# vt-asaplab/vPIN

Hardware: AMD Instinct MI355X
Metric: R1CS constraints/sec, whole Spartan SNARK (sat proof + SPARK evaluation proof; vPIN point-mult + point-add instances) (higher is better)
Workload: dtype u256 (integers mod q and mod p = 2^255-19, 32-bit limbs); 1 GPU; vPIN LeNet trace (layers L1..L7): 12 SNARKs per step; inputs=resident in HBM, parallelism=one trace per rank x 1 rank(s), no collective; 4 stream(s) per rank, table_slot_bytes=128

## Files before the change

vpin_amd/csrc/capi.hip:

```cpp
#include <chrono>
#include <csignal>
#include <execinfo.h>
#include <fcntl.h>
#include <unistd.h>
#include <cstdio>
#include <cstdlib>
#include <cstring>
#include <thread>

#include "ctx.h"

namespace vpin {

static thread_local std::string g_last_error;

void set_last_error(const char* what, hipError_t e) {
  g_last_error = std::string(what) + ": " + hipGetErrorString(e);
}

void set_last_error_text(const char* text) { g_last_error = text; }

static hipEvent_t get_event(vpin_ctx* c) {
  if (!c->free_events.empty()) {
    hipEvent_t e = c->free_events.back();
// ... 209 lines not shown
void ctx_leave_alt(vpin_ctx* c) { if (c && c->stream_alt) ctx_switch_stream(c, c->stream_main, c->cus_main, false); }

ProfScope::ProfScope(vpin_ctx* c, int kclass, double bytes, int also, double units) : ctx(c) {
  if (!c->prof) return;
  ProfRec r;
  r.kclass = kclass;
  r.also = also;
  r.units = units;
  r.bytes = bytes;
  r.start = get_event(c);
  r.stop = get_event(c);
  (void)hipEventRecord(r.start, c->stream);
  c->recs.push_back(r);
  rec = (int)c->recs.size() - 1;
}

ProfScope::~ProfScope() {
  if (rec >= 0) (void)hipEventRecord(ctx->recs[rec].stop, ctx->stream);
}

}

using namespace vpin;

extern "C" {

const char* vpin_strerror(int code) {
  switch (code) {
    case VPIN_OK: return "ok";
    case VPIN_EINVAL: return "invalid argument";
    case VPIN_ENODEV: return "no usable HIP device (this library has no CPU fallback)";
    case VPIN_ENOMEM: return "out of memory";
    case VPIN_EHIP: return "HIP runtime error";
    case VPIN_ESHAPE: return "operand shapes do not match";
    case VPIN_EVERIFY: return "proof rejected by the verifier";
    case VPIN_ECOMM: return "a peer rank failed or timed out";
    default: return "unknown error";
  }
}

const char* vpin_last_error(void) { return g_last_error.c_str(); }

int vpin_abi_version(void) { return 11; }

static int ctx_create(int device, int priority, const uint32_t* cu_mask, uint32_t n_words, vpin_ctx** out);

int vpin_ctx_create(int device, vpin_ctx** out) { return ctx_create(device, 0, nullptr, 0, out); }
int vpin_ctx_create_prio(int device, int priority, vpin_ctx** out) { return ctx_create(device, priority, nullptr, 0, out); }
int vpin_ctx_create_cumask(int device, const uint32_t* cu_mask, uint32_t n_words, vpin_ctx** out) {
  if (!cu_mask || n_words == 0) return VPIN_EINVAL;
  return ctx_create(device, 0, cu_mask, n_words, out);
}

static int ctx_create(int device, int priority, const uint32_t* cu_mask, uint32_t n_words, vpin_ctx** out) {
  if (!out) return VPIN_EINVAL;
  setenv("KMP_BLOCKTIME", "0", 0);
  setenv("OMP_WAIT_POLICY", "PASSIVE", 0);
  setenv("KMP_AFFINITY", "disabled", 0);
  *out = nullptr;
  int n = 0;
  if (hipGetDeviceCount(&n) != hipSuccess || n <= 0) return VPIN_ENODEV;
  if (device < 0 || device >= n) return VPIN_EINVAL;
  VPIN_HIP_TRY(hipSetDevice(device));
  vpin_ctx* c = new (std::nothrow) vpin_ctx();
  if (!c) return VPIN_ENOMEM;
  c->device = device;
  hipDeviceProp_t prop;
  if (hipGetDeviceProperties(&prop, device) == hipSuccess) c->num_cus = prop.multiProcessorCount;
  int lo = 0, hi = 0;
  (void)hipDeviceGetStreamPriorityRange(&lo, &hi);
  int prio = priority < 0 ? hi : priority > 0 ? lo : 0;
  hipError_t e;
  if (cu_mask) {
    int enabled = 0;
    for (uint32_t w = 0; w < n_words; w++) {
      uint32_t bits = cu_mask[w];
      if ((w + 1) * 32 > (uint32_t)c->num_cus) bits &= (w * 32 >= (uint32_t)c->num_cus) ? 0u : ((1u << (c->num_cus - w * 32)) - 1u);
      enabled += __builtin_popcount(bits);
    }
    if (enabled == 0) { delete c; return VPIN_EINVAL; }
    e = hipExtStreamCreateWithCUMask(&c->stream, n_words, cu_mask);
    c->num_cus = enabled;
    c->cu_masked = true;
  } else {
    e = hipStreamCreateWithPriority(&c->stream, hipStreamNonBlocking, prio);
  }
  if (e != hipSuccess) { set_last_error("hipStreamCreate", e); delete c; return VPIN_EHIP; }
  c->stream_main = c->stream;
  c->cus_main = c->num_cus;
  c->partials_cap = (size_t)18 * 4096 * 3;
  if (hipMalloc(&c->d_partials, c->partials_cap * sizeof(fq)) != hipSuccess ||
      hipMalloc(&c->d_out, 8 * sizeof(fq)) != hipSuccess ||
      hipHostMalloc(&c->h_out, 8 * sizeof(fq), hipHostMallocDefault) != hipSuccess) {
    vpin_ctx_destroy(c);
    return VPIN_ENOMEM;
  }
  ctx_register(c);
  *out = c;
  return VPIN_OK;
}

void vpin_ctx_destroy(vpin_ctx* c) {
  if (!c) return;
  (void)hipSetDevice(c->device);
  if (c->stream) (void)hipStreamSynchronize(c->stream);
  ctx_leave_alt(c);
  if (c->prover_cache_free) c->prover_cache_free(c);
  if (c->spark_cache_free) c->spark_cache_free(c);
  if (c->verify_cache_free) c->verify_cache_free(c);
  if (c->h_spark) (void)hipHostFree(c->h_spark);
  if (c->d_spark_cnt) (void)hipFree(c->d_spark_cnt);
  if (c->d_add_count) (void)hipFree(c->d_add_count);
  ctx_unregister(c);
  ctx_wait_unpinned(c);
  dev_pool_release(c);
  if (!c->pool_sizes.empty()) {
    fprintf(stderr, "vpin_ctx_destroy: %zu device block(s) still referenced by live handles are released with the context; "
                    "free tables / instances / decommitments before the context\n", c->pool_sizes.size());
    for (auto& kv : c->pool_sizes) (void)hipFree(kv.first);
    c->pool_sizes.clear();
  }
  for (auto& r : c->recs) { (void)hipEventDestroy(r.start); (void)hipEventDestroy(r.stop); }
  for (auto e : c->free_events) (void)hipEventDestroy(e);
  if (c->d_partials) (void)hipFree(c->d_partials);
  if (c->d_out) (void)hipFree(c->d_out);
  if (c->h_out) (void)hipHostFree(c->h_out);
  if (c->h_bullet) (void)hipHostFree(c->h_bullet);
  if (c->stream_alt) { (void)hipStreamSynchronize(c->stream_alt); (void)hipStreamDestroy(c->stream_alt); }
  if (c->stream_switch_ev) (void)hipEventDestroy(c->stream_switch_ev);
  if (c->stream_main) (void)hipStreamDestroy(c->stream_main);
  delete c;
}

void* vpin_ctx_stream(vpin_ctx* c) { return c ? (void*)c->stream : nullptr; }

int vpin_ctx_set_cumask_after_phase1(vpin_ctx* c, const uint32_t* cu_mask, uint32_t n_words) {
  if (!c || c->cu_masked || c->stream != c->stream_main) return VPIN_EINVAL;
  (void)hipSetDevice(c->device);
  if (c->stream_alt) {
    VPIN_HIP_TRY(hipStreamSynchronize(c->stream_alt));
    (void)hipStreamDestroy(c->stream_alt);
    c->stream_alt = nullptr;
    c->cus_alt = 0;
  }
  if (!cu_mask || n_words == 0) return VPIN_OK;
  int enabled = 0;
  for (uint32_t w = 0; w < n_words; w++) {
    uint32_t bits = cu_mask[w];
    if ((w + 1) * 32 > (uint32_t)c->cus_main) bits &= (w * 32 >= (uint32_t)c->cus_main) ? 0u : ((1u << (c->cus_main - w * 32)) - 1u);
    enabled += __builtin_popcount(bits);
  }
  if (enabled == 0) return VPIN_EINVAL;
  if (!c->stream_switch_ev) VPIN_HIP_TRY(hipEventCreateWithFlags(&c->stream_switch_ev, hipEventDisableTiming));
  VPIN_HIP_TRY(hipExtStreamCreateWithCUMask(&c->stream_alt, n_words, cu_mask));
  c->cus_alt = enabled;
  return VPIN_OK;
}

int vpin_ctx_set_progress_flag(vpin_ctx* c, int* flag) {
  if (!c) return VPIN_EINVAL;
  c->progress_flag = flag;
  return VPIN_OK;
}

unsigned long long vpin_ctx_strip_rows_taken(vpin_ctx* c) { return c ? c->strip_rows_taken : 0ull; }
unsigned long long vpin_ctx_row_table_rows(vpin_ctx* c) { return c ? c->row_table_rows : 0ull; }
// ... 329 lines not shown
```

vpin_amd/csrc/ctx.h:

```cpp
#pragma once
#include <hip/hip_runtime.h>

#include <atomic>
#include <chrono>
#include <cstdio>
#include <cstdlib>
#include <map>
#include <mutex>
#include <string>
#include <unordered_map>
#include <vector>

#include "../../include/vpin_hip.h"
#include "fq_dev.h"

namespace vpin {

void set_last_error(const char* what, hipError_t e);

#define VPIN_HIP_TRY(expr)                         \
  do {                                             \
    hipError_t e_ = (expr);                        \
    if (e_ != hipSuccess) {                        \
      ::vpin::set_last_error(#expr, e_);           \
      return VPIN_EHIP;                            \
    }                                              \
  } while (0)

struct ProfRec {
  int kclass;
  double bytes;
  hipEvent_t start, stop;
  int also = -1;
  double units = 0.0;
};

}

struct vpin_ctx;

struct vpin_table {
  vpin::fq* d = nullptr;
  size_t len = 0;
  size_t cap = 0;
  bool owned = true;
  vpin_ctx* owner = nullptr;
};

struct vpin_gens;

struct vpin_ctx {
  int device = 0;
  hipStream_t stream = nullptr;
  int num_cus = 256;
  bool cu_masked = false;
  hipStream_t stream_main = nullptr, stream_alt = nullptr;
  hipEvent_t stream_switch_ev = nullptr;
  int cus_main = 256, cus_alt = 0;
  vpin::fq* d_partials = nullptr;
  size_t partials_cap = 0;
  vpin::fq* d_out = nullptr;
  vpin::fq* h_out = nullptr;
  bool prof = false;
  bool prof_count_adds = false;
  unsigned long long* d_add_count = nullptr;
  std::vector<vpin::ProfRec> recs;
  std::vector<hipEvent_t> free_events;
  vpin_kstat stats[VPIN_K_COUNT] = {};
  std::mutex pool_mu;
  std::atomic<int> pins{0};
  std::map<size_t, std::vector<void*>> pool_free_lists;
  std::unordered_map<void*, size_t> pool_sizes;
  void* prover_cache = nullptr;
  void (*prover_cache_free)(vpin_ctx*) = nullptr;
  void* spark_cache = nullptr;
  void (*spark_cache_free)(vpin_ctx*) = nullptr;
  void* verify_cache = nullptr;
  void (*verify_cache_free)(vpin_ctx*) = nullptr;
  vpin::fq* h_spark = nullptr;
  uint32_t* d_spark_cnt = nullptr;
  uint32_t spark_seq = 0;
  int round_split = 0, round_split_grid = 0, round_split_ncirc = 0;
  int round_group_ndotp = 0;
  uint32_t tail_seq = 0;
  std::atomic<int> tail_rounds{0};
  vpin::fq tail_sums[3 * 18];
  vpin::fq tail_final[6 * 18];
  unsigned long long pip_row_chunks = 0;
  unsigned long long row_table_rows = 0;
  unsigned long long strip_rows_taken = 0;
  unsigned long long rlc_shared_sums = 0;
  size_t rlc_shared_cap = 0;
  bool pool_poison = false;
  uint32_t pool_poison_word = 0;
  unsigned long long pool_poison_blocks = 0, pool_poison_bytes = 0;
  unsigned long long witness_redo_ops = 0;
  bool low_memory = false;
  bool shared_device = false;
  int expected_proofs = 0;
  double gens_scalars_per_proof = 0.0;
  void* h_bullet = nullptr;
  uint32_t bullet_seq = 0;
  std::atomic<vpin_comm*> comm_pub{nullptr};
  vpin_comm* comm = nullptr;
  volatile int* progress_flag = nullptr;
};

namespace vpin {

struct ProfScope {
  vpin_ctx* ctx;
  int rec = -1;
  ProfScope(vpin_ctx* c, int kclass, double bytes, int also = -1, double units = 0.0);
  ~ProfScope();
};

void ctx_enter_alt(vpin_ctx* c);
void ctx_leave_alt(vpin_ctx* c);
struct AltStreamGuard {
  vpin_ctx* c;
  explicit AltStreamGuard(vpin_ctx* ctx) : c(ctx) {}
  ~AltStreamGuard() { ctx_leave_alt(c); }
};

int dev_alloc(vpin_ctx* c, size_t bytes, void** out);
hipError_t driver_malloc(void** p, size_t bytes);
void note_driver_alloc(size_t bytes);
void dev_free(vpin_ctx* c, void* p);
int live_ctx_count();
double host_cpu_quota();
void dev_free_owned(vpin_ctx* owner, vpin_ctx* fallback, void* p);
void dev_pool_release(vpin_ctx* c);
void dev_release_block(vpin_ctx* c, void* p);

struct DevBuf {
  vpin_ctx* c;
  void* p = nullptr;
  explicit DevBuf(vpin_ctx* ctx) : c(ctx) {}
// ... 87 lines not shown
```

vpin_amd/csrc/host/prover_common.h:

```cpp
#pragma once
#include <omp.h>

#include <chrono>
#include <cstdlib>
#include <cstring>
#include <map>
#include <memory>
#include <mutex>
#include <string>
#include <vector>

#include "../ctx.h"
#include "../comm.h"
#include "curve.h"
#include "transcript.h"

extern "C" {
size_t vpin_gens_msm_parts_count(size_t ncols);
int vpin_gens_msm_parts(vpin_ctx* ctx, const vpin_gens* g, const uint8_t* scalars_mont, size_t rows, size_t ncols,
                        uint8_t* parts_xyzt);
int vpin_poly_bound(vpin_ctx* c, const vpin_table* Z, const uint8_t* Lvec, size_t L_size, uint8_t* out_LZ);
int vpin_gens_map_stream(vpin_ctx* ctx, const uint8_t* stream64, size_t nb, uint8_t* out_xyzt);
void vpin_r1cs_dims(const vpin_r1cs_dev* d, size_t* num_cons, size_t* num_vars, size_t* num_inputs);
}

namespace vpin_prover {

#if defined(__clang__)
#pragma clang diagnostic push
#pragma clang diagnostic ignored "-Wunused-function"
#endif


using namespace vpin_host;
using Clock = std::chrono::steady_clock;
static double secs(Clock::time_point a, Clock::time_point b) { return std::chrono::duration<double>(b - a).count(); }

static int host_threads() {
  static const int fixed = [] {
    setenv("KMP_BLOCKTIME", "0", 0);
    setenv("OMP_WAIT_POLICY", "PASSIVE", 0);
    const char* e = getenv("VPIN_HOST_THREADS");
    int want = e ? atoi(e) : 0;
    const int hw = omp_get_num_procs();
    return want > hw ? hw : want;
  }();
  if (fixed >= 1) return fixed;
  const int ctxs = vpin::live_ctx_count();
  int n = (int)(vpin::host_cpu_quota() / (2.0 * (double)(ctxs > 0 ? ctxs : 1)));
  return n < 1 ? 1 : n > 8 ? 8 : n;
}

static size_t log2z(size_t n) { size_t l = 0; while (((size_t)1 << l) < n) l++; return l; }
static const uint8_t* B(const Fq* p) { return reinterpret_cast<const uint8_t*>(p); }
static uint8_t* B(Fq* p) { return reinterpret_cast<uint8_t*>(p); }

struct CG { uint8_t b[32]; };
static CG compress(const Point& p) { CG c; p.compress(c.b); return c; }


struct Mcg {
  int n;
  const FixedBase* G[4];
  const FixedBase* h;
};

inline void derive_gens(std::vector<Point>& g, size_t nb, const char* label, vpin_ctx* dev = nullptr) {
  static std::mutex mu;
  static std::map<std::string, std::shared_ptr<const std::vector<Point>>> cache;
  std::shared_ptr<const std::vector<Point>> have;
  {
    std::lock_guard<std::mutex> lock(mu);
    auto it = cache.find(label);
    if (it != cache.end()) have = it->second;
  }
  if (have && have->size() >= nb) {
    g.assign(have->begin(), have->begin() + (long)nb);
    return;
  }
  uint8_t bc[32];
  Point::basepoint().compress(bc);
  Shake256 sh;
  sh.absorb(reinterpret_cast<const uint8_t*>(label), strlen(label));
  sh.absorb(bc, 32);
  sh.finalize();
  std::vector<uint8_t> stream(64 * nb);
  sh.squeeze(stream.data(), stream.size());
  auto fresh = std::make_shared<std::vector<Point>>(nb);
// ... 310 lines not shown
  };
  size_t n = R;
  static const bool fine = getenv("VPIN_SPARK_TRACE") && atoi(getenv("VPIN_SPARK_TRACE")) >= 3;
  double tb[6] = {0, 0, 0, 0, 0, 0};
  const bool fused = vpin::bullet_fused(bs);
  auto sum_side = [&](int row, size_t nn) {
    const uint8_t* ptrs[256];
    const size_t cnt = vpin::bullet_part_ptrs(c, bs, nn, row, ptrs);
    Point acc = Point::identity();
    for (size_t k = 0; k < cnt; k++) acc = acc + Point::from_xyzt(ptrs[k]);
    return acc;
  };
  Fq u_prev = Fq::zero(), u_inv_prev = Fq::zero();
  for (size_t round = 0; round < lgR; round++) {
    n /= 2;
    Fq cLR[2];
    auto t0 = Clock::now();
    if (fused) rc = vpin::bullet_step(c, pc.dev, bs, n, round ? B(&u_prev) : nullptr, round ? B(&u_inv_prev) : nullptr, B(cLR));
    else rc = vpin::bullet_round_begin(c, pc.dev, bs, n, parts.data(), B(cLR));
    if (rc) return rc;
    auto t1 = Clock::now();
    Point qh[2] = {Point::identity(), Point::identity()};
    pc.fb_gR.mul_acc(qh[0], cLR[0] * r_); pc.fb_h.mul_acc(qh[0], bv1[round]);
    pc.fb_gR.mul_acc(qh[1], cLR[1] * r_); pc.fb_h.mul_acc(qh[1], bv2[round]);
    auto t2 = Clock::now();
    if ((rc = vpin::bullet_round_end(c))) return rc;
    auto t3 = Clock::now();
    Point lr[2] = {(fused ? sum_side(0, n) : sum_parts(parts.data())) + qh[0],
                   (fused ? sum_side(1, n) : sum_parts(parts.data() + np * 128)) + qh[1]};
    auto t4 = Clock::now();
    out.Lvec[round] = compress(lr[0]);
    out.Rvec[round] = compress(lr[1]);
    tr.append_point("L", out.Lvec[round].b);
    tr.append_point("R", out.Rvec[round].b);
    Fq u = tr.challenge_scalar("u"), u_inv = u.invert();
    auto t5 = Clock::now();
    if (fused) { u_prev = u; u_inv_prev = u_inv; }
    else if ((rc = vpin::bullet_fold(c, bs, n, B(&u), B(&u_inv)))) return rc;
    blind_fin = blind_fin + bv1[round] * u * u + bv2[round] * u_inv * u_inv;
    if (fine) {
      auto t6 = Clock::now();
      tb[0] += secs(t0, t1); tb[1] += secs(t1, t2); tb[2] += secs(t2, t3); tb[3] += secs(t3, t4); tb[4] += secs(t4, t5); tb[5] += secs(t5, t6);
    }
  }
  if (fine)
    fprintf(stderr, "[dplog] R=%zu, %zu rounds, us per round: rows+inner products %.1f | host Q,H terms %.1f | wait for the MSM %.1f | "
            "sum %zu parts x2 %.1f | compress x2 + transcript + invert %.1f | fold launch %.1f\n", R, lgR, tb[0] / lgR * 1e6,
            tb[1] / lgR * 1e6, tb[2] / lgR * 1e6, np, tb[3] / lgR * 1e6, tb[4] / lgR * 1e6, tb[5] / lgR * 1e6);
  Fq xa[2];
  if (fused) rc = vpin::bullet_finish_fused(c, pc.dev, bs, B(&u_prev), B(&u_inv_prev), B(xa));
  else rc = vpin::bullet_finish(c, pc.dev, bs, B(xa), parts.data());
  if (rc) return rc;
  const Fq x_hat = xa[0], a_hat = xa[1], y_hat = x_hat * a_hat;
  Point g_hat = fused ? sum_side(0, 0) : sum_parts(parts.data());
  {
    Point p = g_hat.mul(d_);
    pc.fb_h.mul_acc(p, r_delta);
    out.delta = compress(p);
    tr.append_point("delta", out.delta.b);
    Point q = pc.fb_gR.mul(d_ * r_);
    pc.fb_h.mul_acc(q, r_beta);
    out.beta = compress(q);
    tr.append_point("beta", out.beta.b);
  }
  Fq c_ = tr.challenge_scalar("c");
  out.z1 = d_ + c_ * y_hat;
  out.z2 = a_hat * (c_ * blind_fin + r_beta) + r_delta;
  bs_guard.done = true;
  return VPIN_OK;
}

struct TableGuard {
  vpin_ctx* c;
  std::vector<vpin_table*> t;
  explicit TableGuard(vpin_ctx* c_) : c(c_) {}
  ~TableGuard() { for (auto* p : t) vpin_table_free(c, p); }
  vpin_table* add(vpin_table* p) { t.push_back(p); return p; }
};

#if defined(__clang__)
#pragma clang diagnostic pop
#endif

int sat_prove_core(vpin_ctx* c, const vpin_r1cs_dev* dinst, size_t nv, size_t ncons, size_t ni,
                   const vpin_table* d_para, const vpin_table* d_input, const vpin_table* d_vars, const uint8_t* inputs,
                   const uint8_t seed_commit64[64], const uint8_t seed_proof64[64], uint8_t* proof_out, size_t proof_cap,
                   size_t* proof_len, uint8_t* comm_para_out, uint8_t* comm_input_out, uint8_t inst_evals_out[96],
                   uint8_t* rx_out, uint8_t* ry_out, vpin_host::Transcript* tr_out, vpin_host::Transcript* tape_out);

}
```

vpin_amd/csrc/prover.cpp:

```cpp
#include "host/proof_sizes.h"
#include "host/prover_common.h"

namespace {

using namespace vpin_host;
using namespace vpin_prover;


struct SatGens {
  size_t ell = 0, L = 0, R = 0, nb = 0;
  std::vector<Point> g;
  FixedBase fb[5];
  const vpin_gens* dev = nullptr;
  PcGens pc;
  Mcg gens_1, gens_3, gens_4;
};

struct ProverCache {
  std::map<size_t, std::unique_ptr<SatGens>> by_nv;
};

static void cache_free(vpin_ctx* c) {
  auto* pc = static_cast<ProverCache*>(c->prover_cache);
  if (!pc) return;
// ... 369 lines not shown
  if (rc) return rc;
  struct Guard { vpin_ctx* c; vpin::BulletState* s; ~Guard() { (void)hipStreamSynchronize(c->stream); vpin::bullet_free(c, s); } } guard{c, bs};
  const bool fused = !classic && vpin::bullet_fused(bs);
  if (!classic && !fused) return VPIN_ESHAPE;
  const size_t lgR = log2z(R), np = vpin_gens_msm_parts_count(R);
  auto sum_side = [&](int row, size_t nn) {
    const uint8_t* ptrs[256];
    const size_t cnt = vpin::bullet_part_ptrs(c, bs, nn, row, ptrs);
    Point acc = Point::identity();
    for (size_t k = 0; k < cnt; k++) acc = acc + Point::from_xyzt(ptrs[k]);
    return acc;
  };
  std::vector<uint8_t> parts(2 * np * 128);
  const Fq* u = reinterpret_cast<const Fq*>(u_mont);
  Fq u_prev = Fq::zero(), ui_prev = Fq::zero();
  size_t n = R;
  for (size_t k = 0; k < lgR; k++) {
    n /= 2;
    if (fused) rc = vpin::bullet_step(c, g, bs, n, k ? B(&u_prev) : nullptr, k ? B(&ui_prev) : nullptr, cLR_out + 64 * k);
    else rc = vpin::bullet_round_begin(c, g, bs, n, parts.data(), cLR_out + 64 * k);
    if (rc) return rc;
    if ((rc = vpin::bullet_round_end(c))) return rc;
    for (int row = 0; row < 2; row++) {
      Point acc = Point::identity();
      if (fused) acc = sum_side(row, n);
      else
        for (size_t p = 0; p < np; p++) acc = acc + Point::from_xyzt(parts.data() + ((size_t)row * np + p) * 128);
      acc.compress(LR_out + 64 * k + 32 * row);
    }
    u_prev = u[k];
    ui_prev = u[k].invert();
    if (!fused && (rc = vpin::bullet_fold(c, bs, n, B(&u_prev), B(&ui_prev)))) return rc;
  }
  Point ghat = Point::identity();
  if (fused) {
    if ((rc = vpin::bullet_finish_fused(c, g, bs, B(&u_prev), B(&ui_prev), xhat_ahat_out))) return rc;
    ghat = sum_side(0, 0);
  } else {
    if ((rc = vpin::bullet_finish(c, g, bs, xhat_ahat_out, parts.data()))) return rc;
    for (size_t p = 0; p < np; p++) ghat = ghat + Point::from_xyzt(parts.data() + p * 128);
  }
  ghat.compress(ghat_out);
  return VPIN_OK;
}

void vpin_sat_last_timings(double out[8]) { memcpy(out, g_timings, sizeof g_timings); }

size_t vpin_sat_proof_max_bytes(size_t num_cons, size_t num_vars) { return vpin_sizes::sat_proof_max_bytes(num_cons, num_vars); }

}

namespace vpin_prover {

static int dist_fingerprint_check(vpin_ctx* c, size_t nv, size_t ncons, size_t ni, const uint8_t seed_commit64[64],
                                  const uint8_t seed_proof64[64]) {
  vpin_comm* cm = c->comm;
  auto fnv = [](const uint8_t* p, size_t n) { uint64_t h = 0xcbf29ce484222325ull; for (size_t i = 0; i < n; i++) { h ^= p[i]; h *= 0x100000001b3ull; } return h; };
  auto env_num = [](const char* name, long dflt) { const char* e = getenv(name); return e ? atol(e) : dflt; };
  uint64_t fp[9] = {
      (uint64_t)nv, (uint64_t)ncons, (uint64_t)ni, fnv(seed_commit64, 64), fnv(seed_proof64, 64),
      (uint64_t)(getenv("VPIN_DIST_NO_SAT_SPLIT") != nullptr), (uint64_t)(getenv("VPIN_DIST_BY_CIRCUIT") != nullptr),
      (uint64_t)env_num("VPIN_SPARK_TAIL_PAIRS", 1024), (uint64_t)(getenv("VPIN_BULLET_CLASSIC") != nullptr)};
  std::vector<uint64_t> all((size_t)cm->world * 9);
  int rc = vpin::comm_allgather_ctx(c, fp, all.data(), sizeof fp, "fingerprint");
  if (rc) return rc;
  static const char* what[9] = {"num_vars", "num_cons", "num_inputs", "seed_commit", "seed_proof", "VPIN_DIST_NO_SAT_SPLIT",
                                "VPIN_DIST_BY_CIRCUIT", "VPIN_SPARK_TAIL_PAIRS", "VPIN_BULLET_CLASSIC"};
  for (int r = 0; r < cm->world; r++)
    for (int k = 0; k < 9; k++)
      if (all[(size_t)r * 9 + k] != fp[k]) {
        char msg[200];
        snprintf(msg, sizeof msg, "collective proof: rank %d and rank %d differ in %s (%llu vs %llu)", cm->rank, r, what[k],
                 (unsigned long long)fp[k], (unsigned long long)all[(size_t)r * 9 + k]);
        vpin::set_last_error(msg, hipErrorUnknown);
        return VPIN_ECOMM;
      }
  return VPIN_OK;
}

int sat_prove_core(vpin_ctx* c, const vpin_r1cs_dev* dinst, size_t nv, size_t ncons, size_t ni,
                   const vpin_table* d_para, const vpin_table* d_input, const vpin_table* d_vars, const uint8_t* inputs,
                   const uint8_t seed_commit64[64], const uint8_t seed_proof64[64], uint8_t* proof_out, size_t proof_cap,
                   size_t* proof_len, uint8_t* comm_para_out, uint8_t* comm_input_out, uint8_t inst_evals_out[96],
                   uint8_t* rx_out, uint8_t* ry_out, vpin_host::Transcript* tr_out, vpin_host::Transcript* tape_out) {
  auto t_begin = Clock::now();
  memset(g_timings, 0, sizeof g_timings);
  (void)hipSetDevice(c->device);

  SatGens* sg = nullptr;
  auto t0 = Clock::now();
  int rc = get_gens(c, nv, &sg);
  if (rc) return rc;
  g_timings[5] = secs(t0, Clock::now());
  const size_t L = sg->L, R = sg->R;
  TableGuard tg(c);

  t0 = Clock::now();
  vpin_comm* cm = (c->comm && c->comm->world > 1) ? c->comm : nullptr;
  if (cm && (rc = dist_fingerprint_check(c, nv, ncons, ni, seed_commit64, seed_proof64))) return rc;
  const size_t nrows = cm ? vpin::comm_strided_count(L, cm->rank, cm->world) : L;
  vpin::CommitPairState* cps = nullptr;
  if (nrows && (rc = vpin::commit_pair_begin(c, sg->dev, d_para, d_input, L, &cps, cm ? (size_t)cm->rank : 0, nrows, cm ? (size_t)cm->world : 1)))
    return rc;
  const uint8_t two = 2;
  Transcript tape1 = make_tape(&two, 1, seed_commit64);
  std::vector<Fq> blind_para = tape1.challenge_vector("poly_blinds", L);
  std::vector<Fq> blind_input = tape1.challenge_vector("poly_blinds", L);
  std::vector<Fq> blind_vars(L);
  for (size_t i = 0; i < L; i++) blind_vars[i] = blind_para[i] + blind_input[i];
  std::vector<CG> comm_vars(L);
  if (!cm) {
    rc = vpin::commit_pair_finish(c, sg->dev, cps, B(blind_para.data()), B(blind_input.data()), R + 1, comm_para_out,
                                  comm_input_out, comm_vars[0].b);
    if (rc) return rc;
  } else {
    const size_t pmax = vpin::comm_block_max(L, cm->world);
    std::vector<uint8_t> mine(3 * pmax * 32, 0), all((size_t)cm->world * 3 * pmax * 32);
    if (nrows) {
      std::vector<Fq> bp(nrows), bi(nrows);
      for (size_t k = 0; k < nrows; k++) { bp[k] = blind_para[cm->rank + k * cm->world]; bi[k] = blind_input[cm->rank + k * cm->world]; }
      if ((rc = vpin::commit_pair_finish(c, sg->dev, cps, B(bp.data()), B(bi.data()), R + 1, mine.data(), mine.data() + pmax * 32,
                                         mine.data() + 2 * pmax * 32)))
        return rc;
    }
    if ((rc = vpin::comm_allgather_ctx(c, mine.data(), all.data(), mine.size(), "witness_commit"))) return rc;
    for (int r = 0; r < cm->world; r++) {
      const size_t n = vpin::comm_strided_count(L, r, cm->world);
      const uint8_t* blk = all.data() + (size_t)r * 3 * pmax * 32;
      for (size_t k = 0; k < n; k++) {
        const size_t row = (size_t)r + k * (size_t)cm->world;
        memcpy(comm_para_out + row * 32, blk + k * 32, 32);
        memcpy(comm_input_out + row * 32, blk + pmax * 32 + k * 32, 32);
        memcpy(comm_vars[row].b, blk + 2 * pmax * 32 + k * 32, 32);
      }
    }
  }
  g_timings[0] = secs(t0, Clock::now());

  Transcript tr("snark_example");
  Transcript tape = make_tape(reinterpret_cast<const uint8_t*>("proof"), 5, seed_proof64);
  tr.append_protocol_name("Spartan SNARK proof");
  tr.append_protocol_name("R1CS proof");
  tr.append_message("poly_commitment", "poly_commitment_begin");
  for (size_t i = 0; i < L; i++) tr.append_point("poly_commitment_share", comm_vars[i].b);
  tr.append_message("poly_commitment", "poly_commitment_end");

  t0 = Clock::now();
  const size_t zl = 2 * nv;
  vpin_table* d_z = nullptr;
  if ((rc = vpin_r1cs_build_z(c, dinst, d_vars, inputs, &d_z))) return rc;
  tg.add(d_z);
  const int nrx = (int)log2z(ncons), nry = (int)log2z(zl);
  std::vector<Fq> tau = tr.challenge_vector("challenge_tau", nrx);
  int lw = 0;
  if (cm && (cm->world & (cm->world - 1)) == 0) {
    const int l = (int)log2z((size_t)cm->world);
    static const bool off = getenv("VPIN_DIST_NO_SAT_SPLIT") != nullptr;
    if (!off && nrx - l >= 12 && nry - l >= 12) lw = l;
  }
  const size_t wstep = (size_t)1 << lw, wrank = lw ? (size_t)cm->rank : 0;
  vpin_table* d_pyr = nullptr;
  if ((rc = vpin_eq_suffix_tables(c, B(tau.data()), nrx - lw, &d_pyr))) return rc;
  tg.add(d_pyr);
  const Fq one = Fq::one();
  vpin_table* d_abc[3] = {nullptr, nullptr, nullptr};
  auto t_spmv = Clock::now();
  if (lw) rc = vpin::r1cs_multiply_vec_strided(c, dinst, d_z, wrank, wstep, &d_abc[0], &d_abc[1], &d_abc[2]);
// ... 8 lines not shown
  rc = zk_sumcheck(c, 4, tabs1, Fq::zero(), Fq::zero(), nrx, sg->gens_1, sg->gens_4, tr, tape, sc1, rx, claims1, blind_post1,
                   &tau, d_pyr, lw);
  if (rc) return rc;
  if ((rc = vpin::comm_mark(c, "sat_phase1_rest"))) return rc;
  vpin::ctx_enter_alt(c);
  if (c->progress_flag) *c->progress_flag = 1;
  g_timings[1] = secs(t0, Clock::now());

  const Fq tau_claim = claims1[0], Az_claim = claims1[1], Bz_claim = claims1[2], Cz_claim = claims1[3];
  Fq Az_blind = tape.challenge_scalar("Az_blind"), Bz_blind = tape.challenge_scalar("Bz_blind"),
     Cz_blind = tape.challenge_scalar("Cz_blind"), prod_blind = tape.challenge_scalar("prod_Az_Bz_blind");
  KnowProof pok_Cz;
  CG comm_Cz = knowledge_prove(pok_Cz, sg->gens_1, tr, tape, Cz_claim, Cz_blind);
  ProdProof pprod;
  CG comm_Az, comm_Bz, comm_prod;
  product_prove(pprod, sg->gens_1, tr, tape, Az_claim, Az_blind, Bz_claim, Bz_blind, Az_claim * Bz_claim, prod_blind, comm_Az,
                comm_Bz, comm_prod);
  tr.append_point("comm_Az_claim", comm_Az.b);
  tr.append_point("comm_Bz_claim", comm_Bz.b);
  tr.append_point("comm_Cz_claim", comm_Cz.b);
  tr.append_point("comm_prod_Az_Bz_claims", comm_prod.b);
  Fq blind_expected1 = tau_claim * (prod_blind - Cz_blind);
  Fq claim_post1 = (Az_claim * Bz_claim - Cz_claim) * tau_claim;
  EqProof eq1;
  equality_prove(eq1, sg->gens_1, tr, tape, claim_post1, blind_expected1, claim_post1, blind_post1);

  t0 = Clock::now();
  Fq r_A = tr.challenge_scalar("challenege_Az"), r_B = tr.challenge_scalar("challenege_Bz"),
     r_C = tr.challenge_scalar("challenege_Cz");
  Fq claim2 = r_A * Az_claim + r_B * Bz_claim + r_C * Cz_claim;
  Fq blind_claim2 = r_A * Az_blind + r_B * Bz_blind + r_C * Cz_blind;
  vpin_table *d_eq_rx = nullptr, *d_eabc = nullptr;
  if ((rc = vpin_eq_table(c, B(rx.data()), nrx, &d_eq_rx))) return rc;
  tg.add(d_eq_rx);
  t_spmv = Clock::now();
  {
    Fq rabc[3] = {r_A, r_B, r_C};
    if (lw) rc = vpin::r1cs_eval_table_strided(c, dinst, d_eq_rx, B(rabc), wrank, wstep, &d_eabc);
    else rc = vpin_r1cs_eval_table(c, dinst, d_eq_rx, B(rabc), &d_eabc);
    if (rc) return rc;
    tg.add(d_eabc);
  }
  g_timings[6] += secs(t_spmv, Clock::now());
  Fq claims2[2], blind_post2;
  vpin_table* d_z2 = d_z;
  if (lw) {
    if ((rc = vpin::table_take_strided(c, d_z, wrank, wstep, &d_z2))) return rc;
    tg.add(d_z2);
  }
  vpin_table* tabs2[2] = {d_z2, d_eabc};
  rc = zk_sumcheck(c, 2, tabs2, claim2, blind_claim2, nry, sg->gens_1, sg->gens_3, tr, tape, sc2, ry, claims2, blind_post2, nullptr,
                   nullptr, lw);
  if (rc) return rc;
  if ((rc = vpin::comm_mark(c, "sat_phase2_rest"))) return rc;
  g_timings[2] = secs(t0, Clock::now());

  t0 = Clock::now();
  const size_t left = sg->ell / 2, right = sg->ell - left;
  std::vector<Fq> Lv(L), Rv(R), LZ(R);
  host_eq(ry.data() + 1, left, Lv.data());
  host_eq(ry.data() + 1 + left, right, Rv.data());
  if (cm) rc = vpin::poly_bound_dist(c, d_vars, B(Lv.data()), L, B(LZ.data()));
  else rc = vpin_poly_bound(c, d_vars, B(Lv.data()), L, B(LZ.data()));
  if (rc) return rc;
  Fq eval_vars_at_ry = Fq::zero();
  for (size_t i = 0; i < R; i++) eval_vars_at_ry = eval_vars_at_ry + LZ[i] * Rv[i];
  Fq blind_eval = tape.challenge_scalar("blind_eval");
  tr.append_protocol_name("polynomial evaluation proof");
  Fq LZ_blind = Fq::zero();
  for (size_t i = 0; i < L; i++) LZ_blind = LZ_blind + blind_vars[i] * Lv[i];

  DpLog pe;
  if ((rc = dplog_prove(c, sg->pc, tr, tape, LZ, LZ_blind, Rv, eval_vars_at_ry, blind_eval, pe))) return rc;
  g_timings[3] = secs(t0, Clock::now());

  Fq blind_eval_Z = (one - ry[0]) * blind_eval;
  Fq blind_expected2 = claims2[1] * blind_eval_Z;
  Fq claim_post2 = claims2[0] * claims2[1];
  EqProof eq2;
  equality_prove(eq2, sg->gens_1, tr, tape, claim_post2, blind_expected2, claim_post2, blind_post2);

  t0 = Clock::now();
  Fq ie[3];
  {
    vpin_table* d_eq_ry = nullptr;
    if ((rc = vpin_eq_table(c, B(ry.data()), nry, &d_eq_ry))) return rc;
    tg.add(d_eq_ry);
    if ((rc = vpin_r1cs_evaluate(c, dinst, d_eq_rx, d_eq_ry, B(ie)))) return rc;
  }
  tr.append_scalar("Ar_claim", ie[0]);
  tr.append_scalar("Br_claim", ie[1]);
  tr.append_scalar("Cr_claim", ie[2]);
  memcpy(inst_evals_out, ie, 96);
  g_timings[7] = secs(t0, Clock::now());

  Writer w;
  w.u64(L);
  for (auto& cg : comm_vars) w.point(cg);
  write_zksc(w, sc1);
  w.point(comm_Az); w.point(comm_Bz); w.point(comm_Cz); w.point(comm_prod);
  w.point(pok_Cz.alpha); w.scalar(pok_Cz.z1); w.scalar(pok_Cz.z2);
  w.point(pprod.alpha); w.point(pprod.beta); w.point(pprod.delta);
  for (int i = 0; i < 5; i++) w.scalar(pprod.z[i]);
  w.point(eq1.alpha); w.scalar(eq1.z);
  write_zksc(w, sc2);
  w.point(pe.Cy);
  write_dplog(w, pe);
  w.point(eq2.alpha); w.scalar(eq2.z);
  if (w.buf.size() > proof_cap) return VPIN_ESHAPE;
  memcpy(proof_out, w.buf.data(), w.buf.size());
  *proof_len = w.buf.size();
  if (rx_out) memcpy(rx_out, rx.data(), rx.size() * 32);
  if (ry_out) memcpy(ry_out, ry.data(), ry.size() * 32);
  if ((rc = vpin::comm_mark(c, "sat_replicated"))) return rc;
  if (tr_out) *tr_out = tr;
  if (tape_out) *tape_out = tape;
  g_timings[4] = secs(t_begin, Clock::now());
  static const bool trace_on = getenv("VPIN_SPARK_TRACE") && atoi(getenv("VPIN_SPARK_TRACE")) >= 2;
  if (trace_on)
    fprintf(stderr, "[sat] 2^%d: polycommit %.3f  phase 1 %.3f  phase 2 %.3f  polyeval %.3f  inst.evaluate %.3f  (sparse products %.3f)  total %.3f ms\n",
            nrx, 1e3 * g_timings[0], 1e3 * g_timings[1], 1e3 * g_timings[2], 1e3 * g_timings[3], 1e3 * g_timings[7],
            1e3 * g_timings[6], 1e3 * g_timings[4]);
  return VPIN_OK;
}

}

extern "C" {

int vpin_sat_prepare(vpin_ctx* c, size_t num_vars) {
  if (!c || !vpin::is_pow2(num_vars)) return VPIN_EINVAL;
  SatGens* sg = nullptr;
  return get_gens(c, num_vars, &sg);
}

int vpin_sat_prove_resident(vpin_ctx* c, const vpin_r1cs_dev* dinst, const vpin_table* vars_para, const vpin_table* vars_input,
                            const vpin_table* vars, const uint8_t* inputs, const uint8_t seed_commit64[64],
                            const uint8_t seed_proof64[64], uint8_t* proof_out, size_t proof_cap, size_t* proof_len,
                            uint8_t* comm_para_out, uint8_t* comm_input_out, uint8_t inst_evals_out[96], uint8_t* rx_out,
                            uint8_t* ry_out) {
  if (!c || !dinst || !vars_para || !vars_input || !vars || !seed_commit64 || !seed_proof64 || !proof_out || !proof_len ||
      !comm_para_out || !comm_input_out || !inst_evals_out)
    return VPIN_EINVAL;
  size_t nv, ncons, ni;
  vpin_r1cs_dims(dinst, &ncons, &nv, &ni);
  if (vars_para->len != nv || vars_input->len != nv || vars->len != nv || (ni && !inputs)) return VPIN_ESHAPE;
  vpin::AltStreamGuard alt_guard(c);
  return vpin::comm_leave(c->comm, vpin_prover::sat_prove_core(c, dinst, nv, ncons, ni, vars_para, vars_input, vars, inputs, seed_commit64,
                                                               seed_proof64, proof_out, proof_cap, proof_len, comm_para_out,
                                                               comm_input_out, inst_evals_out, rx_out, ry_out, nullptr, nullptr));
}

int vpin_dense_mlpoly_commit_sum(vpin_ctx* c, const vpin_table* vars, const uint8_t seed_commit64[64], uint8_t* out_compressed) {
  if (!c || !vars || !vars->d || !seed_commit64 || !out_compressed) return VPIN_EINVAL;
  const size_t nv = vars->len;
  if (!vpin::is_pow2(nv) || nv < 2) return VPIN_ESHAPE;
  (void)hipSetDevice(c->device);
  SatGens* sg = nullptr;
  int rc = get_gens(c, nv, &sg);
  if (rc) return rc;
  const size_t L = sg->L, R = sg->R;
  const uint8_t two = 2;
  Transcript tape1 = make_tape(&two, 1, seed_commit64);
  std::vector<Fq> blind_para = tape1.challenge_vector("poly_blinds", L);
  std::vector<Fq> blind_input = tape1.challenge_vector("poly_blinds", L);
  std::vector<Fq> blind_sum(L);
  for (size_t i = 0; i < L; i++) blind_sum[i] = blind_para[i] + blind_input[i];
// ... 33 lines not shown
```

vpin_amd/csrc/sc_dev.h:

```cpp
#pragma once
#include <cstring>
#include <type_traits>

#include "ctx.h"

namespace vpin {

#ifndef VPIN_SC_MIN_WAVES
#define VPIN_SC_MIN_WAVES 3
#endif
constexpr int kBlock = 256;
constexpr int kMinWaves = VPIN_SC_MIN_WAVES;
constexpr int kMaxBlocksCap = 16384;
inline int max_blocks() {
  static const int n = [] { const char* e = getenv("VPIN_SC_BLOCKS"); int v = e ? atoi(e) : 1024; return v < 1 ? 1 : v > kMaxBlocksCap ? kMaxBlocksCap : v; }();
  return n;
}

__host__ __device__ inline size_t pyramid_offset(int ell, int k) { return ((size_t)1 << ell) - ((size_t)2 << (ell - k)); }


template <int K>
struct Acc;

template <>
struct Acc<4> {
  static constexpr int NE = 3;
  fq e[3];
  __device__ __forceinline__ void init() { e[0] = e[1] = e[2] = fq_zero(); }
  __device__ __forceinline__ void stage_bc(fq* u, fq pb, const fq& db, fq pc, const fq& dc) {
    u[0] = fq_mul(pb, pc);
    pb = fq_add(fq_add(pb, db), db); pc = fq_add(fq_add(pc, dc), dc);
    u[1] = fq_mul(pb, pc);
    pb = fq_add(pb, db); pc = fq_add(pc, dc);
    u[2] = fq_mul(pb, pc);
  }
  __device__ __forceinline__ void stage_d(fq* u, fq pd, const fq& dd) {
    u[0] = fq_sub(u[0], pd);
    pd = fq_add(fq_add(pd, dd), dd);
    u[1] = fq_sub(u[1], pd);
    pd = fq_add(pd, dd);
    u[2] = fq_sub(u[2], pd);
  }
  __device__ __forceinline__ void stage_e(const fq* u, const fq& E) {
    e[0] = fq_add(e[0], fq_mul(E, u[0]));
    e[1] = fq_add(e[1], fq_mul(E, u[1]));
    e[2] = fq_add(e[2], fq_mul(E, u[2]));
  }
  __device__ __forceinline__ void lead_bcd(const fq& pb, const fq& db, const fq& pc, const fq& dc, const fq& pd, const fq& E) {
    e[0] = fq_add(e[0], fq_mul(E, fq_sub(fq_mul(pb, pc), pd)));
    e[1] = fq_add(e[1], fq_mul(E, fq_mul(db, dc)));
  }
  __device__ __forceinline__ void lead_one(const fq& pb, const fq& db, const fq& pc, const fq& dc, const fq& pd, const fq& dd,
                                           const fq& E) {
    e[2] = fq_add(e[2], fq_mul(E, fq_sub(fq_mul(fq_add(pb, db), fq_add(pc, dc)), fq_add(pd, dd))));
  }
  __device__ __forceinline__ void stage_a(const fq* u, fq pa, const fq& da) {
    e[0] = fq_add(e[0], fq_mul(pa, u[0]));
    pa = fq_add(fq_add(pa, da), da);
    e[1] = fq_add(e[1], fq_mul(pa, u[1]));
    pa = fq_add(pa, da);
    e[2] = fq_add(e[2], fq_mul(pa, u[2]));
  }
};

struct LeadNow {
  __device__ __forceinline__ void init() {}
  __device__ __forceinline__ void add(fq* e, const fq& E, const fq& X, const fq& Y) {
    e[0] = fq_add(e[0], fq_mul(E, X));
    e[1] = fq_add(e[1], fq_mul(E, Y));
  }
  __device__ __forceinline__ void flush(fq*) {}
};
struct LeadAcc {
  fq_wide w[2];
  int n;
  __device__ __forceinline__ void init() { fqw_zero(w[0]); fqw_zero(w[1]); n = 0; }
  __device__ __forceinline__ void add(fq* e, const fq& E, const fq& X, const fq& Y) {
#ifdef VPIN_NO_LAZY_ACC
    e[0] = fq_add(e[0], fq_mul(E, X));
    e[1] = fq_add(e[1], fq_mul(E, Y));
#else
    fqw_mac(w[0], E, X);
    fqw_mac(w[1], E, Y);
#ifndef VPIN_LAZY_NO_FLUSH
    if (++n == 7) flush(e);
#endif
#endif
  }
  __device__ __forceinline__ void flush(fq* e) {
    if (n == 0) return;
    e[0] = fq_add(e[0], fqw_reduce(w[0]));
    e[1] = fq_add(e[1], fqw_reduce(w[1]));
    fqw_zero(w[0]); fqw_zero(w[1]);
    n = 0;
  }
};

template <>
// ... 213 lines not shown
```

vpin_amd/csrc/spark.cpp:

```cpp
#include <cstdio>

#include "host/proof_sizes.h"
#include "host/prover_common.h"
#include "gadget_dev.h"
#include "sc_dev.h"
#include "spark_dev.h"

namespace {

using namespace vpin_host;
using namespace vpin_prover;

static bool spark_trace() { static const bool on = getenv("VPIN_SPARK_TRACE") != nullptr; return on; }
struct TraceSpan {
  const char* name; Clock::time_point t0;
  explicit TraceSpan(const char* n) : name(n), t0(Clock::now()) {}
  ~TraceSpan() { if (spark_trace()) fprintf(stderr, "[spark] %-28s %8.3f ms\n", name, secs(t0, Clock::now()) * 1e3); }
};


struct SparkGens {
  std::vector<Point> g;
  std::map<size_t, std::unique_ptr<PcGens>> views;
};
// ... 543 lines not shown
        const Fq* res = reinterpret_cast<const Fq*>(c->h_spark);
        for (int t = 0; t < npc; t++) {
          cl[t] = res[4 * t] + rl * (res[4 * t + 1] - res[4 * t]);
          cr[t] = res[4 * t + 2] + rl * (res[4 * t + 3] - res[4 * t + 2]);
        }
        if (with_dotp) {
          const Fq* q = reinterpret_cast<const Fq*>(c->h_spark) + 64;
          for (int i = 0; i < 6; i++)
            for (int t = 0; t < 3; t++) dp[3 * i + t] = q[6 * i + 2 * t] + rl * (q[6 * i + 2 * t + 1] - q[6 * i + 2 * t]);
        }
      }
    }

    for (int t = 0; t < npc; t++) {
      tr.append_scalar("claim_prod_left", cl[t]);
      tr.append_scalar("claim_prod_right", cr[t]);
    }
    if (with_dotp) {
      for (int t = 0; t < 3; t++) out.dotp[t].resize(6);
      for (int i = 0; i < 6; i++) {
        for (int t = 0; t < 3; t++) out.dotp[t][i] = dp[3 * i + t];
        tr.append_scalar("claim_dotp_left", out.dotp[0][i]);
        tr.append_scalar("claim_dotp_right", out.dotp[1][i]);
        tr.append_scalar("claim_dotp_weight", out.dotp[2][i]);
      }
    }
    Fq r_layer = tr.challenge_scalar("challenge_r_layer");
    for (int t = 0; t < npc; t++) claims[t] = cl[t] + r_layer * (cr[t] - cl[t]);
    out.claims_left[o] = cl;
    out.claims_right[o] = cr;
    std::vector<Fq> ext;
    ext.reserve(k + 1);
    ext.push_back(r_layer);
    ext.insert(ext.end(), r.begin(), r.end());
    rand.swap(ext);
    if (fine) { auto t = Clock::now(); t_epi += secs(tl0, t); tl0 = t; }
  }
  if (fine)
    fprintf(stderr, "[spark]   forest of %d x 2^%d: setup %.3f  first result %.3f  later results %.3f  host per-round math %.3f  epilogue %.3f ms\n",
            npc, num_layers, t_setup * 1e3, t_first * 1e3, t_rounds * 1e3, t_host * 1e3, t_epi * 1e3);
  return VPIN_OK;
}

static thread_local double g_spark_timings[8];

static int dist_pick(vpin_ctx* c, const DistPlan& pl, const Fq* mine, size_t cnt, const int* owner, Fq* out, const char* tag) {
  std::vector<Fq> all(cnt * (size_t)pl.world);
  int rc = vpin::comm_allgather_ctx(c, mine, all.data(), cnt * 32, tag);
  if (rc) return rc;
  for (size_t i = 0; i < cnt; i++) out[i] = all[cnt * (size_t)owner[i] + i];
  return VPIN_OK;
}

struct SparkProof {
  vpin_ctx* c;
  const vpin_spark_decomm* d;
  const std::vector<Fq>&rx, &ry;
  const Fq* evals;
  Transcript &tr, &tape;
  const size_t N, M, lgN, lgM;
  const PcGens *g_ops = nullptr, *g_mem = nullptr, *g_derefs = nullptr;
  TableGuard tg;
  DistPlan plan;
  const DistPlan* dz = nullptr;
  bool st = false;
  vpin::SparkLeaves leaves;
  size_t Nf = 0, Mf = 0;
  bool defer_mem = false;
  vpin_table *mem_rx = nullptr, *mem_ry = nullptr, *comb = nullptr;
  vpin_table comb_shape;
  vpin::DevBuf b_cloc, b_crows, b_vloc, b_ops, b_mem, b_scr;
  vpin::fq* comb_rows = nullptr;
  const vpin::fq *derefs = nullptr, *vals = nullptr;
  std::vector<CG> comm_derefs;
  vpin::HashParams hash;
  vpin::SparkForest f_ops, f_mem;
  Fq pl[2][8];
  DotpCtx dotp;
  Fq dotp_left[3], dotp_right[3];
  Batched pf_ops, pf_mem;
  std::vector<Fq> rand_ops, rand_mem;
  Fq ev_derefs[6], ev_ops[15], ev_mem[2];
  DpLog pe_derefs, pe_ops, pe_mem;

  SparkProof(vpin_ctx* c_, const vpin_spark_decomm* d_, const std::vector<Fq>& rx_, const std::vector<Fq>& ry_, const Fq* evals_,
             Transcript& tr_, Transcript& tape_)
      : c(c_), d(d_), rx(rx_), ry(ry_), evals(evals_), tr(tr_), tape(tape_), N(d_->N), M(d_->M), lgN(log2z(d_->N)), lgM(log2z(d_->M)),
        tg(c_), b_cloc(c_), b_crows(c_), b_vloc(c_), b_ops(c_), b_mem(c_), b_scr(c_) {}
  bool by_circuit() const { return dz && !st; }
};

static int split_plan(SparkProof& S) {
  vpin_ctx* c = S.c;
  if (!(c->comm && c->comm->world > 1)) return VPIN_OK;
  if (c->comm->world > 12) return VPIN_EINVAL;
  plan_init(S.plan, c->comm);
  S.dz = &S.plan;
  static const bool by_circuit = getenv("VPIN_DIST_BY_CIRCUIT") != nullptr;
  const size_t Wz = (size_t)S.plan.world;
  if (!by_circuit && (Wz & (Wz - 1)) == 0 && Wz <= 16 && S.N / Wz >= 4096 && S.M / Wz >= 4096 && S.g_derefs->L >= Wz)
    S.plan.lw = (int)log2z(Wz);
  S.st = S.plan.lw > 0;
  if (S.st) { S.leaves.r0 = (size_t)S.plan.rank; S.leaves.step = Wz; }
  return VPIN_OK;
}

static int stage_derefs(SparkProof& S) {
  vpin_ctx* c = S.c;
  const vpin_spark_decomm* d = S.d;
  const DistPlan* dz = S.dz;
  const PcGens* g_derefs = S.g_derefs;
  const size_t N = S.N;
  int rc;
  S.tr.append_protocol_name("Sparse polynomial evaluation proof");
  const size_t nm = std::max(d->nx, d->ny);
  std::vector<Fq> rx_ext(nm, Fq::zero()), ry_ext(nm, Fq::zero());
  std::copy(S.rx.begin(), S.rx.end(), rx_ext.begin() + (nm - d->nx));
  std::copy(S.ry.begin(), S.ry.end(), ry_ext.begin() + (nm - d->ny));
  if ((rc = vpin_eq_table(c, B(rx_ext.data()), (int)nm, &S.mem_rx))) return rc;
  S.tg.add(S.mem_rx);
  if ((rc = vpin_eq_table(c, B(ry_ext.data()), (int)nm, &S.mem_ry))) return rc;
  S.tg.add(S.mem_ry);
  const vpin::fq *mem_rx = S.mem_rx->d, *mem_ry = S.mem_ry->d;
  S.Nf = N / S.leaves.step; S.Mf = S.M / S.leaves.step;
  if (S.st) {
    S.comb_shape.d = nullptr; S.comb_shape.len = S.comb_shape.cap = 8 * N; S.comb_shape.owned = false;
    S.comb = &S.comb_shape;
    const size_t Nl = S.Nf, nrows_loc = vpin::comm_strided_count(g_derefs->L, dz->rank, dz->world);
    if (S.b_cloc.alloc(6 * Nl * 32) || S.b_crows.alloc(std::max<size_t>(1, nrows_loc) * g_derefs->R * 32) || S.b_vloc.alloc(3 * Nl * 32)) return VPIN_ENOMEM;
    S.comb_rows = (vpin::fq*)S.b_crows.p;
    if ((rc = vpin::spark_gather_derefs(c, d, S.leaves, mem_rx, mem_ry, (vpin::fq*)S.b_cloc.p, S.comb_rows, g_derefs->R, nrows_loc))) return rc;
    for (int m = 0; m < 3; m++)
      if ((rc = vpin::spark_take_strided(c, d->vals + (size_t)m * N, Nl, S.leaves.r0, S.leaves.step, (vpin::fq*)S.b_vloc.p + (size_t)m * Nl))) return rc;
    S.derefs = (const vpin::fq*)S.b_cloc.p; S.vals = (const vpin::fq*)S.b_vloc.p;
  } else {
    if ((rc = vpin::table_alloc_uninit(c, 8 * N, &S.comb))) return rc;
    S.tg.add(S.comb);
    if ((rc = vpin::spark_gather_derefs(c, d, S.leaves, mem_rx, mem_ry, S.comb->d))) return rc;
    S.derefs = S.comb->d; S.vals = d->vals;
  }
  if ((rc = vpin::comm_mark(c, "derefs_gather"))) return rc;
  std::vector<CG>& comm_derefs = S.comm_derefs;
  const bool hot = d->hot_col[0] != 0xffffffffu || d->hot_col[1] != 0xffffffffu || d->hot_col[2] != 0xffffffffu;
  const uint32_t* col_idx[3] = {d->idx + 6 * N, d->idx + 7 * N, d->idx + 8 * N};
  if (dz) {
    const size_t L = g_derefs->L, pmax = vpin::comm_block_max(L, dz->world);
    const size_t nrows = vpin::comm_strided_count(L, dz->rank, dz->world);
    std::vector<uint8_t> mine(pmax * 32, 0), all(pmax * 32 * (size_t)dz->world);
    if (nrows) {
      if (hot)
        rc = vpin::hyrax_commit_derefs_hot(c, g_derefs->dev, S.comb, L, N, col_idx, d->hot_col, mem_ry, mine.data(), (size_t)dz->rank,
                                           nrows, (size_t)dz->world, S.comb_rows);
      else
        rc = vpin::hyrax_commit_rows_strided(c, g_derefs->dev, S.comb, L, (size_t)dz->rank, nrows, (size_t)dz->world, mine.data(), S.comb_rows);
      if (rc) return rc;
    }
    if ((rc = vpin::comm_allgather_ctx(c, mine.data(), all.data(), mine.size(), "derefs_commit"))) return rc;
    comm_derefs.resize(L);
    for (int r = 0; r < dz->world; r++) {
      const size_t n = vpin::comm_strided_count(L, r, dz->world);
      for (size_t k = 0; k < n; k++) memcpy(comm_derefs[(size_t)r + k * (size_t)dz->world].b, all.data() + ((size_t)r * pmax + k) * 32, 32);
    }
  } else if (hot) {
    comm_derefs.resize(g_derefs->L);
    if ((rc = vpin::hyrax_commit_derefs_hot(c, g_derefs->dev, S.comb, g_derefs->L, N, col_idx, d->hot_col, mem_ry, comm_derefs[0].b))) return rc;
  } else if ((rc = commit_noblind(c, g_derefs, S.comb, comm_derefs))) {
    return rc;
  }
  S.tr.append_message("derefs_commitment", "begin_derefs_commitment");
  append_polycomm(S.tr, "comm_poly_row_col_ops_val", comm_derefs);
  S.tr.append_message("derefs_commitment", "end_derefs_commitment");
  return VPIN_OK;
}

static vpin::HashParams make_hash(const Fq& r_hash, const Fq& gamma) {
  const Fq r2 = r_hash * r_hash, r2_boost = r2 * Fq::r2();
  vpin::HashParams hp;
  memcpy(hp.r.v, B(&r_hash), 32); memcpy(hp.r2.v, B(&r2), 32); memcpy(hp.r2_boost.v, B(&r2_boost), 32); memcpy(hp.gamma.v, B(&gamma), 32);
  return hp;
}

static int stage_network(SparkProof& S) {
  vpin_ctx* c = S.c;
  const DistPlan* dz = S.dz;
  int rc;
  std::vector<Fq> r_mem_check = S.tr.challenge_vector("challenge_r_hash", 2);
  S.hash = make_hash(r_mem_check[0], r_mem_check[1]);
  vpin::SparkLeaves lv_ops = S.leaves, lv_mem = S.leaves;
  int nl_ops = 12, nl_mem = 4;
  size_t nl_dotp = 6;
  if (S.by_circuit()) {
    const auto &ops = dz->ops_of[dz->rank], &mem = dz->mem_of[dz->rank];
    lv_ops.ncirc = nl_ops = (int)ops.size(); lv_mem.ncirc = nl_mem = (int)mem.size();
    std::copy(ops.begin(), ops.end(), lv_ops.ids);
    std::copy(mem.begin(), mem.end(), lv_mem.ids);
    nl_dotp = dz->dotp_of[dz->rank].size();
  }
  S.defer_mem = !dz && (c->low_memory || getenv("VPIN_MEM_FOREST_LATE") != nullptr);
  if (S.b_ops.alloc((size_t)nl_ops * 2 * S.Nf * 32) || (nl_mem && !S.defer_mem && S.b_mem.alloc((size_t)nl_mem * 2 * S.Mf * 32)) ||
      S.b_scr.alloc(std::max<size_t>(256, 3 * nl_dotp * (S.Nf / 4) * 32)))
    return VPIN_ENOMEM;
  if ((rc = vpin::comm_mark(c, "network_alloc"))) return rc;
  S.f_ops.base = (vpin::fq*)S.b_ops.p; S.f_ops.n = S.Nf; S.f_ops.ncirc = nl_ops;
  S.f_mem.base = (vpin::fq*)S.b_mem.p; S.f_mem.n = S.Mf; S.f_mem.ncirc = nl_mem;
  const vpin::SparkInputs in{S.derefs, S.mem_rx->d, S.mem_ry->d};
  if (!S.by_circuit() && !S.defer_mem) {
    rc = vpin::spark_build_forests(c, S.d, S.hash, S.leaves, in, &S.f_ops, &S.f_mem);
  } else {
    rc = vpin::spark_build_forest(c, S.d, S.hash, lv_ops, in, &S.f_ops, false);
    if (!rc && !S.defer_mem && nl_mem) rc = vpin::spark_build_forest(c, S.d, S.hash, lv_mem, in, &S.f_mem, true);
  }
  if (rc || (rc = vpin::spark_wait(c))) return rc;
  return vpin::comm_mark(c, "network_build");
}

static int product_roots(SparkProof& S) {
  vpin_ctx* c = S.c;
  const DistPlan* dz = S.dz;
  const bool st = S.st;
  const size_t Wz = S.leaves.step;
  auto& pl = S.pl;
  int rc;
  {
    std::vector<Fq> roots(2 * (size_t)vpin::kSparkMaxInst);
    if ((rc = vpin::spark_fetch_tops(c, &S.f_ops, 2))) return rc;
    const Fq* t = reinterpret_cast<const Fq*>(c->h_spark);
    std::vector<Fq> st_roots(2 * 16);
    if (st) {
      std::vector<Fq> mine16(16), all16(16 * Wz);
      for (int i = 0; i < 12; i++) mine16[i] = t[2 * i];
      if ((rc = vpin::spark_fetch_tops(c, &S.f_mem, 2))) return rc;
      for (int i = 0; i < 4; i++) mine16[12 + i] = t[2 * i];
      if ((rc = vpin::comm_allgather_ctx(c, mine16.data(), all16.data(), 16 * 32, "roots"))) return rc;
      for (int i = 0; i < 16; i++) {
        Fq p = Fq::one();
        for (size_t r = 0; r < Wz; r++) p = p * all16[16 * r + i];
        st_roots[2 * i] = p;
      }
      for (int i = 0; i < 12; i++) roots[2 * i] = st_roots[2 * i];
      t = roots.data();
    } else if (dz) {
      if ((rc = dist_exchange(c, *dz, false, false, t, 2, roots.data(), "roots"))) return rc;
      t = roots.data();
    }
    for (int s = 0; s < 2; s++)
      for (int m = 0; m < 3; m++) { pl[s][1 + m] = t[2 * (s * 6 + m)]; pl[s][4 + m] = t[2 * (s * 6 + 3 + m)]; }
    if (st) {
      for (int i = 0; i < 4; i++) roots[2 * i] = st_roots[2 * (12 + i)];
      t = roots.data();
    } else {
      if (S.defer_mem) {
        if ((rc = vpin::spark_mem_roots(c, S.d, S.hash, S.mem_rx->d, S.mem_ry->d))) return rc;
      } else if (S.f_mem.ncirc && (rc = vpin::spark_fetch_tops(c, &S.f_mem, 2))) {
        return rc;
      }
      t = reinterpret_cast<const Fq*>(c->h_spark);
      if (dz) {
        if ((rc = dist_exchange(c, *dz, true, false, t, 2, roots.data(), "roots"))) return rc;
        t = roots.data();
      }
    }
    for (int s = 0; s < 2; s++) { pl[s][0] = t[2 * (2 * s)]; pl[s][7] = t[2 * (2 * s + 1)]; }
  }
  static const char* lab[2][4] = {{"claim_row_eval_init", "claim_row_eval_read", "claim_row_eval_write", "claim_row_eval_audit"},
                                  {"claim_col_eval_init", "claim_col_eval_read", "claim_col_eval_write", "claim_col_eval_audit"}};
  for (int s = 0; s < 2; s++) {
    Fq ws = Fq::one(), rs = Fq::one();
    for (int m = 0; m < 3; m++) { rs = rs * pl[s][1 + m]; ws = ws * pl[s][4 + m]; }
    if (!(pl[s][0] * ws == rs * pl[s][7])) return VPIN_ESHAPE;
    S.tr.append_scalar(lab[s][0], pl[s][0]);
    S.tr.append_scalars(lab[s][1], &pl[s][1], 3);
    S.tr.append_scalars(lab[s][2], &pl[s][4], 3);
    S.tr.append_scalar(lab[s][3], pl[s][7]);
  }
  return VPIN_OK;
}

static int dotp_claims(SparkProof& S) {
  vpin_ctx* c = S.c;
  const DistPlan* dz = S.dz;
  int rc;
  const std::vector<int>* hv = S.by_circuit() ? &dz->dotp_of[dz->rank] : nullptr;
  const size_t nh = hv ? hv->size() : 6;
  if (nh && (rc = vpin::spark_triple_sums(c, S.derefs, S.vals, S.Nf, hv ? hv->data() : nullptr, (int)nh))) return rc;
  Fq mine6[6] = {};
  for (size_t i = 0; i < nh; i++) mine6[hv ? (*hv)[i] : i] = reinterpret_cast<const Fq*>(c->h_spark)[3 * i];
  if (S.st) rc = dist_sum(c, *dz, mine6, 6, S.dotp.claims, "triple_sums");
  else if (dz) rc = dist_pick(c, *dz, mine6, 6, dz->owner_dotp, S.dotp.claims, "triple_sums");
  else std::copy(mine6, mine6 + 6, S.dotp.claims);
  if (rc) return rc;
  for (int m = 0; m < 3; m++) {
    S.dotp_left[m] = S.dotp.claims[2 * m];
    S.dotp_right[m] = S.dotp.claims[2 * m + 1];
    S.tr.append_scalar("claim_eval_dotp_left", S.dotp_left[m]);
    S.tr.append_scalar("claim_eval_dotp_right", S.dotp_right[m]);
    if (!(S.dotp_left[m] + S.dotp_right[m] == S.evals[m])) return VPIN_ESHAPE;
  }
  return VPIN_OK;
}

static int stage_product(SparkProof& S) {
  vpin_ctx* c = S.c;
  int rc;
  S.tr.append_protocol_name("Sparse polynomial evaluation proof");
  S.tr.append_protocol_name("Sparse polynomial product layer proof");
  if ((rc = product_roots(S))) return rc;
  S.dotp = DotpCtx{S.d, S.Nf, S.vals, S.derefs, (vpin::fq*)S.b_scr.p, {}};
  if ((rc = dotp_claims(S))) return rc;
  {
    TraceSpan ts("product: ops forest");
    if ((rc = product_prove(c, S.f_ops, 12, &S.dotp, S.tr, S.pf_ops, S.rand_ops, S.dz))) return rc;
  }
  if (S.defer_mem) {
    TraceSpan ts("network: mem forest (deferred)");
    S.b_ops.release();
    S.b_scr.release();
    if (S.b_mem.alloc((size_t)4 * 2 * S.M * 32)) return VPIN_ENOMEM;
    S.f_mem.base = (vpin::fq*)S.b_mem.p;
    if ((rc = vpin::spark_build_forest(c, S.d, S.hash, S.leaves, {nullptr, S.mem_rx->d, S.mem_ry->d}, &S.f_mem, true))) return rc;
    if ((rc = vpin::spark_wait(c))) return rc;
  }
  TraceSpan ts("product: mem forest");
  return product_prove(c, S.f_mem, 4, nullptr, S.tr, S.pf_mem, S.rand_mem, S.dz);
}

static int hash_slice_evals_dist(SparkProof& S, const vpin_table* comb_ops, const vpin_table* comb_mem, const vpin_table* eq_ops,
                                 const vpin_table* eq_mem) {
  vpin_ctx* c = S.c;
  const DistPlan* dz = S.dz;
  const size_t N = S.N, M = S.M;
  const Fq* hs = reinterpret_cast<const Fq*>(c->h_spark);
  const int cnts[3] = {6, 15, 2};
  const vpin::fq* tabs[3] = {S.derefs, comb_ops->d, comb_mem->d};
  const vpin::fq* eqs[3] = {eq_ops->d, eq_ops->d, eq_mem->d};
  Fq mine23[23] = {}, all23[23];
  int rc, base = 0;
  if (S.st) {
    const size_t rk = S.leaves.r0, Wz = S.leaves.step;
    std::vector<Fq> lo_ops(Wz), lo_mem(Wz);
    host_eq(S.rand_ops.data() + (S.lgN - dz->lw), (size_t)dz->lw, lo_ops.data());
    host_eq(S.rand_mem.data() + (S.lgM - dz->lw), (size_t)dz->lw, lo_mem.data());
    const Fq scale[3] = {lo_ops[rk], lo_ops[rk], lo_mem[rk]};
    for (int g = 0; g < 3; g++) {
      if (g == 0) rc = vpin::spark_slice_evals(c, tabs[g], S.Nf, cnts[g], eqs[g]);
      else rc = vpin::spark_slice_evals(c, tabs[g], g == 1 ? N : M, cnts[g], eqs[g], rk, Wz);
      if (rc) return rc;
      for (int i = 0; i < cnts[g]; i++) mine23[base + i] = hs[3 * i] * scale[g];
      base += cnts[g];
    }
    if ((rc = dist_sum(c, *dz, mine23, 23, all23, "hash_slice_evals"))) return rc;
  } else {
    const size_t cost[3] = {N, N, M};
    size_t total = 0, cum = 0;
    for (int g = 0; g < 3; g++) total += cost[g] * (size_t)cnts[g];
    int owner[23];
    for (int g = 0, sidx = 0; g < 3; g++)
      for (int i = 0; i < cnts[g]; i++, sidx++) {
        owner[sidx] = (int)std::min<size_t>((size_t)dz->world - 1, (cum + cost[g] / 2) * (size_t)dz->world / total);
        cum += cost[g];
      }
    for (int g = 0; g < 3; g++) {
      int first = -1, cnt = 0;
      for (int i = 0; i < cnts[g]; i++)
        if (owner[base + i] == dz->rank) { if (first < 0) first = i; cnt++; }
      if (cnt) {
        if ((rc = vpin::spark_slice_evals(c, tabs[g] + (size_t)first * cost[g], cost[g], cnt, eqs[g]))) return rc;
        for (int i = 0; i < cnt; i++) mine23[base + first + i] = hs[3 * i];
      }
      base += cnts[g];
// ... 29 lines not shown
  const DistPlan* dz = S.dz;
  const size_t N = S.N, M = S.M;
  const std::vector<Fq>&rand_ops = S.rand_ops, &rand_mem = S.rand_mem;
  int rc;
  S.tr.append_protocol_name("Sparse polynomial hash layer proof");
  vpin_table *eq_ops = nullptr, *eq_mem = nullptr;
  const bool one_pass = !dz && SlicePass::fits(*S.g_derefs, 3, rand_ops) && SlicePass::fits(*S.g_ops, 4, rand_ops) &&
                        SlicePass::fits(*S.g_mem, 1, rand_mem);
  SlicePass sp_derefs(c), sp_ops(c), sp_mem(c);
  vpin_table *comb_ops = nullptr, *comb_mem = nullptr;
  if (!one_pass && dz) {
    auto* dm = const_cast<vpin_spark_decomm*>(d);
    dm->comb_unpooled = true;
    if ((rc = vpin::spark_comb_tables(c, dm))) return rc;
    comb_ops = dm->comb_ops; comb_mem = dm->comb_mem;
  } else if (!one_pass) {
    if ((rc = vpin::spark_comb_make(c, d, &comb_ops, &comb_mem))) return rc;
    S.tg.add(comb_ops); S.tg.add(comb_mem);
  }
  if (!one_pass) {
    TraceSpan ts("hash: eq tables");
    const int lwz = S.st ? dz->lw : 0;
    if ((rc = vpin_eq_table(c, B(rand_ops.data()), (int)S.lgN - lwz, &eq_ops))) return rc;
    S.tg.add(eq_ops);
    if ((rc = vpin_eq_table(c, B(rand_mem.data()), (int)S.lgM - lwz, &eq_mem))) return rc;
    S.tg.add(eq_mem);
  }
  if ((rc = vpin::comm_mark(c, "hash_eq_tables"))) return rc;
  const Fq* hs = reinterpret_cast<const Fq*>(c->h_spark);
  if (dz) {
    if ((rc = hash_slice_evals_dist(S, comb_ops, comb_mem, eq_ops, eq_mem))) return rc;
  } else if (one_pass) {
    TraceSpan ts("hash: derefs slices (one pass)");
    if ((rc = sp_derefs.run(c, *S.g_derefs, nullptr, 0, S.derefs, 3, 6, rand_ops, S.ev_derefs))) return rc;
  } else {
    TraceSpan ts("hash: derefs slice evals");
    if ((rc = vpin::spark_slice_evals(c, S.derefs, N, 6, eq_ops->d))) return rc;
    for (int i = 0; i < 6; i++) S.ev_derefs[i] = hs[3 * i];
  }
  S.tr.append_protocol_name("Derefs evaluation proof");
  std::vector<Fq> e8(8, Fq::zero());
  std::copy(S.ev_derefs, S.ev_derefs + 6, e8.begin());
  if ((rc = prove_joint(S, *S.g_derefs, S.comb, sp_derefs, e8, 3, rand_ops,
                        {"evals_ops_val", "challenge_combine_n_to_one", "joint_claim_eval", "hash: polyeval derefs"}, S.comb_rows, S.pe_derefs)))
    return rc;
  if (one_pass) {
    TraceSpan ts("hash: ops+mem slices (one pass)");
    if ((rc = sp_ops.run(c, *S.g_ops, d->idx, 12, d->vals, 4, 15, rand_ops, S.ev_ops))) return rc;
    if ((rc = sp_mem.run(c, *S.g_mem, d->idx + 12 * N, 2, nullptr, 1, 2, rand_mem, S.ev_mem))) return rc;
  } else if (!dz) {
    TraceSpan ts("hash: ops+mem slice evals");
    if ((rc = vpin::spark_slice_evals(c, comb_ops->d, N, 15, eq_ops->d))) return rc;
    for (int i = 0; i < 15; i++) S.ev_ops[i] = hs[3 * i];
    if ((rc = vpin::spark_slice_evals(c, comb_mem->d, M, 2, eq_mem->d))) return rc;
    for (int i = 0; i < 2; i++) S.ev_mem[i] = hs[3 * i];
  }
  std::vector<Fq> e16(16, Fq::zero());
  std::copy(S.ev_ops, S.ev_ops + 15, e16.begin());
  if ((rc = prove_joint(S, *S.g_ops, comb_ops, sp_ops, e16, 4, rand_ops,
                        {"claim_evals_ops", "challenge_combine_n_to_one", "joint_claim_eval_ops", "hash: polyeval ops"}, nullptr, S.pe_ops)))
    return rc;
  return prove_joint(S, *S.g_mem, comb_mem, sp_mem, {S.ev_mem[0], S.ev_mem[1]}, 1, rand_mem,
                     {"claim_evals_mem", "challenge_combine_two_to_one", "joint_claim_eval_mem", "hash: polyeval mem"}, nullptr, S.pe_mem);
}

static void write_proof(const SparkProof& S, Writer& w) {
  const auto& pl = S.pl;
  w.u64(S.comm_derefs.size());
  for (auto& p : S.comm_derefs) w.point(p);
  for (int s = 0; s < 2; s++) { w.scalar(pl[s][0]); w_scalars(w, &pl[s][1], 3); w_scalars(w, &pl[s][4], 3); w.scalar(pl[s][7]); }
  w_scalars(w, S.dotp_left, 3);
  w_scalars(w, S.dotp_right, 3);
  write_batched(w, S.pf_mem);
  write_batched(w, S.pf_ops);
  w_scalars(w, &S.ev_ops[0], 3); w_scalars(w, &S.ev_ops[3], 3); w.scalar(S.ev_mem[0]);
  w_scalars(w, &S.ev_ops[6], 3); w_scalars(w, &S.ev_ops[9], 3); w.scalar(S.ev_mem[1]);
  w_scalars(w, &S.ev_ops[12], 3);
  w_scalars(w, &S.ev_derefs[0], 3); w_scalars(w, &S.ev_derefs[3], 3);
  write_dplog(w, S.pe_ops);
  write_dplog(w, S.pe_mem);
  write_dplog(w, S.pe_derefs);
}

static int spark_prove(vpin_ctx* c, const vpin_spark_decomm* d, const std::vector<Fq>& rx, const std::vector<Fq>& ry,
                       const Fq evals[3], Transcript& tr, Transcript& tape, Writer& w) {
  if (d->N < 4 || d->M < 4 || rx.size() != d->nx || ry.size() != d->ny) return VPIN_ESHAPE;
  int rc;
  SparkProof S(c, d, rx, ry, evals, tr, tape);
  const Shape sh{d->nx, d->ny, S.N, S.M, S.lgN + 4, std::max(d->nx, d->ny) + 1, S.lgN + 3};
  if ((rc = get_view(c, std::max(sh.v_ops, sh.v_mem), &S.g_ops)) || (rc = get_view(c, sh.v_ops, &S.g_ops)) ||
      (rc = get_view(c, sh.v_mem, &S.g_mem)) || (rc = get_view(c, sh.v_derefs, &S.g_derefs)))
    return rc;
  auto t0 = Clock::now();
  auto lap = [&](int slot) { g_spark_timings[slot] = secs(t0, Clock::now()); t0 = Clock::now(); };
  if ((rc = split_plan(S)) || (rc = stage_derefs(S))) return rc;
  lap(1);
  if (c->progress_flag) *c->progress_flag = 2;
  if ((rc = stage_network(S))) return rc;
  lap(2);
  if ((rc = stage_product(S))) return rc;
  lap(3);
  if ((rc = stage_hash(S))) return rc;
  lap(4);
  write_proof(S, w);
  return VPIN_OK;
}

}

extern "C" {

size_t vpin_spark_comm_bytes(const vpin_r1cs* inst) {
  return inst ? vpin_sizes::spark_comm_bytes(inst->num_cons, inst->num_vars, inst->nnz) : 0;
}

size_t vpin_snark_proof_max_bytes(const vpin_r1cs* inst) {
  return inst ? vpin_sizes::snark_proof_max_bytes(inst->num_cons, inst->num_vars, inst->nnz) : 0;
}

int vpin_spark_prepare(vpin_ctx* c, size_t num_cons, size_t num_vars, size_t max_nnz) {
  if (!c || !vpin::is_pow2(num_cons) || !vpin::is_pow2(num_vars) || max_nnz == 0) return VPIN_EINVAL;
  (void)hipSetDevice(c->device);
  const size_t nnz[3] = {max_nnz, max_nnz, max_nnz};
  const Shape s = shape_of(num_cons, num_vars, nnz);
  const PcGens* g = nullptr;
  int rc = get_view(c, std::max(s.v_ops, s.v_mem), &g);
  if (!rc) {
    auto* sg = static_cast<SparkGens*>(c->spark_cache);
    std::vector<size_t> idx;
    for (size_t ell : {s.v_ops, s.v_mem, s.v_derefs}) {
      const size_t R = (size_t)1 << (ell - ell / 2);
      if (R + 1 < sg->g.size()) { idx.push_back(R); idx.push_back(R + 1); }
    }
#pragma omp parallel for schedule(dynamic, 1) num_threads(host_threads())
    for (long k = 0; k < (long)idx.size(); k++) { FixedBase warm(sg->g[idx[(size_t)k]]); (void)warm; }
  }
  if (!rc) rc = get_view(c, s.v_ops, &g);
  if (!rc) rc = get_view(c, s.v_mem, &g);
  if (!rc) rc = get_view(c, s.v_derefs, &g);
  return rc;
}

int vpin_spark_gens_view(vpin_ctx* c, size_t ell, const vpin_gens** out, size_t* L, size_t* R) {
  if (!c || !out || !L || !R || ell < 2 || ell > 40) return VPIN_EINVAL;
  (void)hipSetDevice(c->device);
  const PcGens* g = nullptr;
  int rc = get_view(c, ell, &g);
  if (rc) return rc;
  *out = g->dev; *L = g->L; *R = g->R;
  return VPIN_OK;
}

int vpin_dist_plan(int world, int owner_ops[12], int owner_dotp[6], int owner_mem[4]) {
  if (world < 1 || world > 12 || !owner_ops || !owner_dotp || !owner_mem) return VPIN_EINVAL;
  make_plan(world, owner_ops, owner_dotp, owner_mem);
  return VPIN_OK;
}

void vpin_spark_decomm_hot_cols(const vpin_spark_decomm* d, uint32_t out[3]) {
  for (int m = 0; m < 3; m++) out[m] = d ? d->hot_col[m] : 0xffffffffu;
}

void vpin_spark_decomm_free(vpin_ctx* c, vpin_spark_decomm* d) {
  if (!d) return;
  if (c) {
    (void)hipSetDevice(c->device);
    if (d->idx) vpin::dev_free(c, d->idx);
    if (d->vals) vpin::dev_free(c, d->vals);
    if (d->comb_ops) vpin_table_free(c, d->comb_ops);
    if (d->comb_mem) vpin_table_free(c, d->comb_mem);
  }
  delete d;
}

static int encode_commit(vpin_ctx* c, const Shape& s, std::unique_ptr<vpin_spark_decomm>& d, vpin::TraceLap& lap, size_t num_cons,
                         size_t num_vars, size_t num_inputs, vpin_spark_decomm** out, uint8_t* comm_out, size_t comm_cap,
                         size_t* comm_len, Clock::time_point t0) {
  auto fail = [&](int rc) { vpin_spark_decomm_free(c, d.release()); return rc; };
// ... 108 lines not shown
  if (!g || !g->r1cs) return 0;
  vpin_r1cs r{};
  r.num_cons = g->r1cs->num_cons; r.num_vars = g->r1cs->num_vars; r.num_inputs = g->num_inputs;
  for (int m = 0; m < 3; m++) r.nnz[m] = g->nnz[m];
  return vpin_spark_comm_bytes(&r);
}

size_t vpin_dev_instance_proof_max_bytes(const vpin_dev_instance* g) {
  if (!g || !g->r1cs) return 0;
  vpin_r1cs r{};
  r.num_cons = g->r1cs->num_cons; r.num_vars = g->r1cs->num_vars; r.num_inputs = g->num_inputs;
  for (int m = 0; m < 3; m++) r.nnz[m] = g->nnz[m];
  return vpin_snark_proof_max_bytes(&r);
}

int vpin_poly_slices_bound(vpin_ctx* c, const vpin_table* Z, int nbits, int used, const uint8_t* r, size_t r_len, const uint8_t* ch,
                           uint8_t* evals_out, uint8_t* LZ_out) {
  if (!c || !Z || !Z->d || nbits < 0 || nbits > 4 || used < 1 || used > (1 << nbits) || !r || !evals_out) return VPIN_EINVAL;
  const size_t ell = r_len + (size_t)nbits;
  if (Z->len != ((size_t)1 << ell) || ell / 2 < (size_t)nbits) return VPIN_ESHAPE;
  PcGens pc;
  pc.ell = ell; pc.L = (size_t)1 << (ell / 2); pc.R = (size_t)1 << (ell - ell / 2);
  std::vector<Fq> rand(r_len);
  memcpy(rand.data(), r, r_len * 32);
  SlicePass sp(c);
  std::vector<Fq> ev((size_t)used);
  int rc = sp.run(c, pc, nullptr, 0, Z->d, nbits, used, rand, ev.data());
  if (rc) return rc;
  memcpy(evals_out, ev.data(), (size_t)used * 32);
  if (ch && LZ_out) {
    std::vector<Fq> chv((size_t)nbits), LZ;
    memcpy(chv.data(), ch, (size_t)nbits * 32);
    if ((rc = sp.combine(c, pc, chv, LZ))) return rc;
    memcpy(LZ_out, LZ.data(), pc.R * 32);
  }
  return VPIN_OK;
}

int vpin_poly_slices_bound_u32(vpin_ctx* c, const uint32_t* slices_u32, int n32, const vpin_table* Zfq, int nbits, int used,
                               const uint8_t* r, size_t r_len, const uint8_t* ch, uint8_t* evals_out, uint8_t* LZ_out) {
  if (!c || !slices_u32 || n32 < 1 || nbits < 0 || nbits > 4 || used < n32 || used > (1 << nbits) || !r || !evals_out) return VPIN_EINVAL;
  const size_t ell = r_len + (size_t)nbits, N = (size_t)1 << r_len;
  if (ell / 2 < (size_t)nbits || (used > n32 && (!Zfq || !Zfq->d || Zfq->len < (size_t)(used - n32) * N))) return VPIN_ESHAPE;
  PcGens pc;
  pc.ell = ell; pc.L = (size_t)1 << (ell / 2); pc.R = (size_t)1 << (ell - ell / 2);
  (void)hipSetDevice(c->device);
  vpin::DevBuf b32(c);
  if (b32.alloc((size_t)n32 * N * 4)) return VPIN_ENOMEM;
  if (hipMemcpyAsync(b32.p, slices_u32, (size_t)n32 * N * 4, hipMemcpyHostToDevice, c->stream) != hipSuccess) return VPIN_EHIP;
  std::vector<Fq> rand(r_len);
  memcpy(rand.data(), r, r_len * 32);
  SlicePass sp(c);
  std::vector<Fq> ev((size_t)used);
  int rc = sp.run(c, pc, (const uint32_t*)b32.p, n32, used > n32 ? Zfq->d : nullptr, nbits, used, rand, ev.data());
  if (rc) return rc;
  memcpy(evals_out, ev.data(), (size_t)used * 32);
  if (ch && LZ_out) {
    std::vector<Fq> chv((size_t)nbits), LZ;
    memcpy(chv.data(), ch, (size_t)nbits * 32);
    if ((rc = sp.combine(c, pc, chv, LZ))) return rc;
    memcpy(LZ_out, LZ.data(), pc.R * 32);
  }
  return VPIN_OK;
}

int vpin_snark_prove_resident(vpin_ctx* c, const vpin_r1cs_dev* dinst, const vpin_spark_decomm* decomm,
                              const vpin_table* vars_para, const vpin_table* vars_input, const vpin_table* vars,
                              const uint8_t* inputs, const uint8_t seed_commit64[64], const uint8_t seed_proof64[64],
                              uint8_t* proof_out, size_t proof_cap, size_t* proof_len, uint8_t* comm_para_out,
                              uint8_t* comm_input_out) {
  if (!c || !dinst || !decomm || !vars_para || !vars_input || !vars || !seed_commit64 || !seed_proof64 || !proof_out ||
      !proof_len || !comm_para_out || !comm_input_out)
    return VPIN_EINVAL;
  size_t nv, ncons, ni;
  vpin_r1cs_dims(dinst, &ncons, &nv, &ni);
  if (vars_para->len != nv || vars_input->len != nv || vars->len != nv || (ni && !inputs)) return VPIN_ESHAPE;
  if (decomm->num_cons != ncons || decomm->num_vars != nv || decomm->num_inputs != ni) return VPIN_ESHAPE;
  auto t0 = Clock::now();
  vpin::AltStreamGuard alt_guard(c);
  Transcript tr("snark_example"), tape("snark_example");
  uint8_t ie[96];
  std::vector<Fq> rx(log2z(ncons)), ry(log2z(2 * nv));
  size_t sat_len = 0;
  int rc = sat_prove_core(c, dinst, nv, ncons, ni, vars_para, vars_input, vars, inputs, seed_commit64, seed_proof64, proof_out,
                          proof_cap, &sat_len, comm_para_out, comm_input_out, ie, B(rx.data()), B(ry.data()), &tr, &tape);
  if (rc) return vpin::comm_leave(c->comm, rc);
  if (c->progress_flag) *c->progress_flag = 1;
  g_spark_timings[5] = secs(t0, Clock::now());
  Writer w;
  w.bytes(ie, 96);
  Fq evals[3];
  memcpy(evals, ie, 96);
  if ((rc = spark_prove(c, decomm, rx, ry, evals, tr, tape, w))) return vpin::comm_leave(c->comm, rc);
  if (sat_len + w.buf.size() > proof_cap) return VPIN_ESHAPE;
  memcpy(proof_out + sat_len, w.buf.data(), w.buf.size());
  *proof_len = sat_len + w.buf.size();
  g_spark_timings[6] = secs(t0, Clock::now());
  return VPIN_OK;
}

int vpin_snark_prove(vpin_ctx* c, const vpin_r1cs* inst, const uint8_t* vars_para, const uint8_t* vars_input,
                     const uint8_t* vars, const uint8_t* inputs, const uint8_t seed_commit64[64], const uint8_t seed_proof64[64],
                     uint8_t* proof_out, size_t proof_cap, size_t* proof_len, uint8_t* comm_out, size_t comm_cap, size_t* comm_len,
                     uint8_t* comm_para_out, uint8_t* comm_input_out) {
  if (!c || !inst || !vars_para || !vars_input || !vars) return VPIN_EINVAL;
  const size_t nv = inst->num_vars;
  if (!vpin::is_pow2(nv) || !vpin::is_pow2(inst->num_cons) || inst->num_inputs >= nv) return VPIN_ESHAPE;
  vpin_r1cs_dev* dinst = nullptr;
  vpin_spark_decomm* decomm = nullptr;
  const bool trace = getenv("VPIN_CLI_TRACE") != nullptr;
  auto t0 = std::chrono::steady_clock::now();
  auto lap = [&](const char* what) {
    if (!trace) return;
    (void)hipStreamSynchronize(c->stream);
    auto t1 = std::chrono::steady_clock::now();
    fprintf(stderr, "[vpin_snark_prove] %-18s %9.1f ms\n", what, std::chrono::duration<double, std::milli>(t1 - t0).count());
    t0 = t1;
  };
  int rc = vpin_r1cs_upload(c, inst, &dinst);
  if (rc) return rc;
  lap("r1cs_upload");
  TableGuard tg(c);
  vpin_table *d_para = nullptr, *d_input = nullptr, *d_vars = nullptr;
  rc = vpin_spark_encode(c, inst, &decomm, comm_out, comm_cap, comm_len);
  lap("spark_encode");
  if (!rc) rc = vpin_table_upload(c, vars_para, nv, &d_para);
  if (!rc) { tg.add(d_para); rc = vpin_table_upload(c, vars_input, nv, &d_input); }
  if (!rc) { tg.add(d_input); rc = vpin_table_upload(c, vars, nv, &d_vars); }
  lap("witness_upload");
  if (!rc) {
    tg.add(d_vars);
    rc = vpin_snark_prove_resident(c, dinst, decomm, d_para, d_input, d_vars, inputs, seed_commit64, seed_proof64, proof_out,
                                   proof_cap, proof_len, comm_para_out, comm_input_out);
  }
  lap("prove_resident");
  vpin_spark_decomm_free(c, decomm);
  vpin_r1cs_free(c, dinst);
  return rc;
}

int vpin_snark_prove_dev(vpin_ctx* c, const vpin_dev_instance* g, const uint8_t seed_commit64[64], const uint8_t seed_proof64[64],
                         uint8_t* proof_out, size_t proof_cap, size_t* proof_len, uint8_t* comm_out, size_t comm_cap,
                         size_t* comm_len, uint8_t* comm_para_out, uint8_t* comm_input_out) {
  if (!c || !g || !g->r1cs) return VPIN_EINVAL;
  vpin_spark_decomm* decomm = nullptr;
  vpin::TraceLap lap(c, "vpin_snark_prove_dev");
  int rc = vpin_spark_encode_dev(c, g, &decomm, comm_out, comm_cap, comm_len);
  lap("spark_encode_dev");
  if (!rc)
    rc = vpin_snark_prove_resident(c, g->r1cs, decomm, g->vars_para, g->vars_input, g->vars, g->num_inputs ? g->inputs : nullptr,
                                   seed_commit64, seed_proof64, proof_out, proof_cap, proof_len, comm_para_out, comm_input_out);
  lap("prove_resident");
  vpin_spark_decomm_free(c, decomm);
  return rc;
}

void vpin_spark_last_timings(double out[8]) { memcpy(out, g_spark_timings, sizeof g_spark_timings); }

}
```

vpin_amd/csrc/spark.hip:

```cpp
#include <chrono>
#include <cstdlib>

#include "mailbox_dev.h"
#include "sc_dev.h"
#include "spark_dev.h"

namespace vpin {

__device__ __forceinline__ fq fq_r2() {
  fq r;
  r.v[0] = 0x449c0f01u; r.v[1] = 0xa40611e3u; r.v[2] = 0x68859347u; r.v[3] = 0xd00e1ba7u;
  r.v[4] = 0x17f5be65u; r.v[5] = 0xceec73d2u; r.v[6] = 0x7c309a3du; r.v[7] = 0x0399411bu;
  return r;
}
__device__ __forceinline__ fq fq_raw_u32(uint32_t x) {
  fq r = fq_zero();
  r.v[0] = x;
  return r;
}

__global__ __launch_bounds__(kBlock) void u32_to_fq_kernel(const uint32_t* __restrict__ src, fq* __restrict__ dst, size_t n) {
  const fq r2 = fq_r2();
  for (size_t i = (size_t)blockIdx.x * kBlock + threadIdx.x; i < n; i += (size_t)gridDim.x * kBlock) {
    uint32_t x = src[i];
// ... 74 lines not shown
    const fq h = mem_leaf_init(hp, fq_load(mem + i), i);
    fq_store(init + k, h);
    fq_store(audit + k, mem_leaf_audit(hp, h, ts[i]));
  }
}

__global__ __launch_bounds__(kBlock) void hash_ops_sub_kernel(const uint32_t* __restrict__ idx, const fq* __restrict__ derefs, size_t N,
                                                              HashParams hp, fq* __restrict__ forest, SparkLeaves lv) {
  const int g = lv.ids[blockIdx.y], side = g / 6, kind = (g % 6) / 3, m = g % 3;
  const uint32_t* addr = idx + (size_t)(side * 6 + m) * N;
  const uint32_t* ts = idx + (size_t)(side * 6 + 3 + m) * N;
  const fq* val = derefs + (size_t)(side * 3 + m) * N;
  fq* leaf = forest + (size_t)blockIdx.y * 2 * N;
  for (size_t i = (size_t)blockIdx.x * kBlock + threadIdx.x; i < N; i += (size_t)gridDim.x * kBlock) {
    const fq h = ops_leaf(hp, fq_load(val + i), addr[i], ts[i]);
    fq_store(leaf + i, kind ? ops_leaf_write(hp, h) : h);
  }
}

__global__ __launch_bounds__(kBlock) void hash_mem_sub_kernel(const uint32_t* __restrict__ audit_ts, const fq* __restrict__ mem_rx,
                                                              const fq* __restrict__ mem_ry, size_t M, HashParams hp,
                                                              fq* __restrict__ forest, SparkLeaves lv) {
  const int g = lv.ids[blockIdx.y], side = g / 2, kind = g % 2;
  const fq* mem = side ? mem_ry : mem_rx;
  const uint32_t* ts = audit_ts + (size_t)side * M;
  fq* leaf = forest + (size_t)blockIdx.y * 2 * M;
  for (size_t i = (size_t)blockIdx.x * kBlock + threadIdx.x; i < M; i += (size_t)gridDim.x * kBlock) {
    fq h = mem_leaf_init(hp, fq_load(mem + i), i);
    if (kind) h = mem_leaf_audit(hp, h, ts[i]);
    fq_store(leaf + i, h);
  }
}


__global__ __launch_bounds__(kBlock) void gather_derefs_rows_kernel(const uint32_t* __restrict__ idx, size_t N, size_t R,
                                                                    const fq* __restrict__ mem_rx, const fq* __restrict__ mem_ry,
                                                                    fq* __restrict__ rows_out, size_t r0, size_t step, size_t nrows_loc) {
  const size_t total = nrows_loc * R;
  for (size_t t = (size_t)blockIdx.x * kBlock + threadIdx.x; t < total; t += (size_t)gridDim.x * kBlock) {
    const size_t jl = t / R, cidx = t - jl * R;
    const size_t g = (r0 + jl * step) * R + cidx;
    const size_t sl = g / N, i = g - sl * N;
    fq v = fq_zero();
    if (sl < 3) v = fq_load(mem_rx + idx[sl * N + i]);
    else if (sl < 6) v = fq_load(mem_ry + idx[(3 + sl) * N + i]);
    fq_store(rows_out + t, v);
  }
}

__global__ __launch_bounds__(kBlock) void take_strided_kernel(const fq* __restrict__ src, size_t nloc, size_t r0, size_t step,
                                                              fq* __restrict__ dst) {
  for (size_t k = (size_t)blockIdx.x * kBlock + threadIdx.x; k < nloc; k += (size_t)gridDim.x * kBlock)
    fq_store(dst + k, fq_load(src + r0 + k * step));
}

__global__ __launch_bounds__(kBlock) void tree_level_kernel(fq* __restrict__ forest, size_t stride, size_t src_off, size_t dst_off,
                                                            size_t h) {
  fq* t = forest + (size_t)blockIdx.y * stride;
  const fq* src = t + src_off;
  fq* dst = t + dst_off;
  for (size_t i = (size_t)blockIdx.x * kBlock + threadIdx.x; i < h; i += (size_t)gridDim.x * kBlock)
    fq_store(dst + i, fq_mul(fq_load(src + i), fq_load(src + h + i)));
}

__global__ __launch_bounds__(kBlock) void tree_level3_kernel(fq* __restrict__ forest, size_t stride, size_t src_off, size_t d1_off,
                                                             size_t d2_off, size_t d3_off, size_t h) {
  fq* t = forest + (size_t)blockIdx.y * stride;
  const fq* src = t + src_off;
  fq *d1 = t + d1_off, *d2 = t + d2_off, *d3 = t + d3_off;
  const size_t q = h / 4;
  for (size_t i = (size_t)blockIdx.x * kBlock + threadIdx.x; i < q; i += (size_t)gridDim.x * kBlock) {
    const fq a0 = fq_mul(fq_load(src + i), fq_load(src + h + i));
    const fq a1 = fq_mul(fq_load(src + q + i), fq_load(src + h + q + i));
    const fq a2 = fq_mul(fq_load(src + 2 * q + i), fq_load(src + h + 2 * q + i));
    const fq a3 = fq_mul(fq_load(src + 3 * q + i), fq_load(src + h + 3 * q + i));
    fq_store(d1 + i, a0); fq_store(d1 + q + i, a1); fq_store(d1 + 2 * q + i, a2); fq_store(d1 + 3 * q + i, a3);
    const fq b0 = fq_mul(a0, a2), b1 = fq_mul(a1, a3);
    fq_store(d2 + i, b0); fq_store(d2 + q + i, b1);
    fq_store(d3 + i, fq_mul(b0, b1));
  }
}

constexpr int kTopBlock = 1024;
__global__ __launch_bounds__(kTopBlock) void tree_top_kernel(fq* __restrict__ forest, size_t stride, size_t n2, size_t h0) {
  fq* t = forest + (size_t)blockIdx.x * stride;
  for (size_t h = h0; h >= 1; h >>= 1) {
    const fq* src = t + (n2 - 4 * h);
    fq* dst = t + (n2 - 2 * h);
    if (threadIdx.x < h) fq_store(dst + threadIdx.x, fq_mul(fq_load(src + threadIdx.x), fq_load(src + h + threadIdx.x)));
    __syncthreads();
  }
}


struct Finisher {
  fq* partials;
  uint32_t* counters;
  fq* out;
  uint32_t* flag;
  uint32_t seq;
  int inst0;
  int total_inst;
  int fused;
};

__device__ __forceinline__ void finish_block(fq* e, const Finisher& f) {
  fq t = block_sum<3, kBlock>(e);
  if (!f.fused) {
    if (threadIdx.x < 3) fq_store(&f.partials[((size_t)blockIdx.y * gridDim.x + blockIdx.x) * 3 + threadIdx.x], t);
    return;
  }
  if (gridDim.x > 1) {
    fq* mine = f.partials + (size_t)blockIdx.y * gridDim.x * 3;
    if (threadIdx.x < 3) fq_store(&mine[(size_t)blockIdx.x * 3 + threadIdx.x], t);
    __shared__ bool is_last;
    __threadfence();
    __syncthreads();
    if (threadIdx.x == 0) is_last = (atomicAdd(&f.counters[f.inst0 + blockIdx.y], 1u) == gridDim.x - 1);
    __syncthreads();
    if (!is_last) return;
    __threadfence();
    fq s[3];
    sum_partial_rows<3>(mine, (int)gridDim.x, threadIdx.x, kBlock, s);
    t = block_sum<3, kBlock>(s);
  }
  if (threadIdx.x < 3) {
    fq_store(&f.out[3 * (size_t)(f.inst0 + blockIdx.y) + threadIdx.x], t);
    __threadfence_system();
  }
  __syncthreads();
  if (threadIdx.x == 0) {
    if (gridDim.x > 1) f.counters[f.inst0 + blockIdx.y] = 0;
    if (atomicAdd(&f.counters[kSparkMaxInst], 1u) == (uint32_t)f.total_inst - 1) {
      f.counters[kSparkMaxInst] = 0;
      __threadfence_system();
      *(volatile uint32_t*)f.flag = f.seq;
    }
  }
}


template <bool BIND, bool LEAD, bool BIG = false>
__global__ __launch_bounds__(kBlock, kMinWaves) void prod_round_kernel(fq* __restrict__ forest, size_t stride, size_t off, size_t h,
                                                                       const fq* __restrict__ E, size_t pairs, fq r, fq_const rc,
                                                                       Finisher fin) {
  constexpr PdMode M = !BIND ? PD_LOAD : LEAD ? PD_FOLD_C : PD_FOLD;
  FoldR fr{r, nullptr};
  if constexpr (M == PD_FOLD_C) fr.tt = stage_fq_const(rc);
  fq* A = forest + (size_t)blockIdx.y * stride + off;
  fq* B = A + h;
  Acc<4> acc;
  acc.init();
  LeadAcc lacc;
  if (LEAD) lacc.init();
  for (size_t i = (size_t)blockIdx.x * kBlock + threadIdx.x; i < pairs; i += (size_t)gridDim.x * kBlock)
    pair_prod<M, LEAD>(acc, lacc, A, B, E, i, pairs, fr);
  if (LEAD) lacc.flush(acc.e);
  finish_block(acc.e, fin);
}

struct DotpPtrs { const fq* src[3]; fq* dst[3]; size_t src_stride[3]; };
struct CircIds { int v[12]; };

template <bool BIND>
__global__ __launch_bounds__(kBlock, kMinWaves) void dotp_round_kernel(const fq* __restrict__ derefs, const fq* __restrict__ vals,
                                                                       size_t N, fq* __restrict__ scratch, bool from_scratch,
                                                                       size_t pairs, fq r, Finisher fin, CircIds kmap) {
  const int k = kmap.v[blockIdx.y], m = k >> 1, half = k & 1;
  const size_t hN = N / 2, q4 = N / 4;
  const fq* src[3];
  fq* dst[3];
#pragma unroll
// ... 222 lines not shown

__global__ __launch_bounds__(kBlock) void count_cols_kernel(const uint32_t* __restrict__ idx, size_t N, uint32_t v0, uint32_t v1,
                                                            unsigned long long* __restrict__ cnt) {
  const int m = blockIdx.y;
  const uint32_t* a = idx + (size_t)(6 + m) * N;
  unsigned n0 = 0, n1 = 0;
  for (size_t i = (size_t)blockIdx.x * kBlock + threadIdx.x; i < N; i += (size_t)gridDim.x * kBlock) {
    const uint32_t x = a[i];
    n0 += x == v0;
    n1 += x == v1;
  }
  __shared__ unsigned sh[2][kBlock];
  sh[0][threadIdx.x] = n0;
  sh[1][threadIdx.x] = n1;
  __syncthreads();
  for (int st = kBlock / 2; st >= 1; st >>= 1) {
    if ((int)threadIdx.x < st) { sh[0][threadIdx.x] += sh[0][threadIdx.x + st]; sh[1][threadIdx.x] += sh[1][threadIdx.x + st]; }
    __syncthreads();
  }
  if (threadIdx.x == 0) {
    if (sh[0][0]) atomicAdd(&cnt[2 * m], (unsigned long long)sh[0][0]);
    if (sh[1][0]) atomicAdd(&cnt[2 * m + 1], (unsigned long long)sh[1][0]);
  }
}

int spark_find_hot_cols(vpin_ctx* c, vpin_spark_decomm* d) {
  if (!c || !d || !d->idx || d->N == 0) return VPIN_EINVAL;
  for (int m = 0; m < 3; m++) d->hot_col[m] = 0xffffffffu;
  if (d->N < ((size_t)1 << 20)) return VPIN_OK;
  (void)hipSetDevice(c->device);
  DevBuf cnt(c);
  if (cnt.alloc(6 * sizeof(unsigned long long))) return VPIN_ENOMEM;
  VPIN_HIP_TRY(hipMemsetAsync(cnt.p, 0, 6 * sizeof(unsigned long long), c->stream));
  const uint32_t v0 = (uint32_t)d->num_vars, v1 = (uint32_t)d->num_vars + 1;
  hipLaunchKernelGGL(count_cols_kernel, dim3(grid_for(d->N), 3), dim3(kBlock), 0, c->stream, (const uint32_t*)d->idx, d->N, v0, v1,
                     (unsigned long long*)cnt.p);
  VPIN_HIP_TRY(hipGetLastError());
  unsigned long long h[6];
  VPIN_HIP_TRY(hipMemcpyAsync(h, cnt.p, sizeof h, hipMemcpyDeviceToHost, c->stream));
  VPIN_HIP_TRY(hipStreamSynchronize(c->stream));
  for (int m = 0; m < 3; m++) {
    const int k = h[2 * m + 1] > h[2 * m] ? 1 : 0;
    if (h[2 * m + k] >= d->N / 64) d->hot_col[m] = k ? v1 : v0;
  }
  return VPIN_OK;
}

int spark_gather_derefs(vpin_ctx* c, const vpin_spark_decomm* d, const SparkLeaves& lv, const fq* mem_rx, const fq* mem_ry, fq* comb,
                        fq* comb_rows, size_t R, size_t nrows_loc) {
  const bool strided = lv.step > 1;
  if (!c || !d || !mem_rx || !mem_ry || !comb || lv.ncirc || lv.step == 0 || lv.r0 >= lv.step || d->N % lv.step) return VPIN_EINVAL;
  if (strided && (!comb_rows || R == 0 || d->N % R)) return VPIN_EINVAL;
  (void)hipSetDevice(c->device);
  ProfScope ps(c, VPIN_K_SPARK_BUILD, strided ? (double)d->N * 6 * 68.0 + (double)nrows_loc * R * 68.0 : (double)d->N * (6 * 68.0 + 2 * 32.0));
  const dim3 grid(grid_for(d->N / lv.step), strided ? 6 : 8);
  if (strided)
    hipLaunchKernelGGL(gather_derefs_kernel<true>, grid, dim3(kBlock), 0, c->stream, (const uint32_t*)d->idx, d->N, mem_rx, mem_ry, comb, lv);
  else
    hipLaunchKernelGGL(gather_derefs_kernel<false>, grid, dim3(kBlock), 0, c->stream, (const uint32_t*)d->idx, d->N, mem_rx, mem_ry, comb, lv);
  if (strided && nrows_loc)
    hipLaunchKernelGGL(gather_derefs_rows_kernel, dim3(grid_for(nrows_loc * R)), dim3(kBlock), 0, c->stream, (const uint32_t*)d->idx, d->N,
                       R, mem_rx, mem_ry, comb_rows, lv.r0, lv.step, nrows_loc);
  VPIN_HIP_TRY(hipGetLastError());
  return VPIN_OK;
}

static int build_levels(vpin_ctx* c, SparkForest* f) {
  const size_t n2 = 2 * f->n;
  size_t h = f->n / 2;
  int l = 0;
  while (h > (size_t)kTopBlock) {
    if (h / 4 > (size_t)kTopBlock) {
      hipLaunchKernelGGL(tree_level3_kernel, dim3(grid_for(h / 4), f->ncirc), dim3(kBlock), 0, c->stream, f->base, f->stride(),
                         f->level_off(l), f->level_off(l + 1), f->level_off(l + 2), f->level_off(l + 3), h);
      h >>= 3;
      l += 3;
      continue;
    }
    hipLaunchKernelGGL(tree_level_kernel, dim3(grid_for(h), f->ncirc), dim3(kBlock), 0, c->stream, f->base, f->stride(),
                       f->level_off(l), f->level_off(l + 1), h);
    h >>= 1;
    l++;
  }
  if (h >= 1) hipLaunchKernelGGL(tree_top_kernel, dim3(f->ncirc), dim3(kTopBlock), 0, c->stream, f->base, f->stride(), n2, h);
  VPIN_HIP_TRY(hipGetLastError());
  return VPIN_OK;
}

static int check_forest(const vpin_ctx* c, const vpin_spark_decomm* d, const SparkLeaves& lv, const SparkInputs& in, const SparkForest* f,
                        bool is_mem) {
  const int all = is_mem ? 4 : 12;
  if (!c || !d || !f || !f->base || lv.step == 0 || lv.r0 >= lv.step || (lv.ncirc && lv.step > 1)) return VPIN_EINVAL;
  if (is_mem ? (!in.mem_rx || !in.mem_ry) : !in.derefs) return VPIN_EINVAL;
  if (lv.ncirc < 0 || lv.ncirc > all) return VPIN_EINVAL;
  for (int j = 0; j < lv.ncirc; j++)
    if (lv.ids[j] < 0 || lv.ids[j] >= all) return VPIN_EINVAL;
  if (f->n * lv.step != (is_mem ? d->M : d->N) || f->ncirc != (lv.ncirc ? lv.ncirc : all) || f->n < 2) return VPIN_ESHAPE;
  return VPIN_OK;
}

static double forest_bytes(const SparkLeaves& lv, const SparkForest* f, bool is_mem) {
  if (lv.ncirc) return (double)f->n * f->ncirc * (is_mem ? (36.0 + 32.0 + 64.0) : (8.0 + 32.0 + 32.0 + 64.0));
  return (double)f->n * (is_mem ? (2 * 36.0 + 4 * 32.0 + 4 * 64.0) : (6 * (8.0 + 32.0) + 12 * 32.0 + 12 * 64.0));
}

static void launch_leaves(vpin_ctx* c, const vpin_spark_decomm* d, const HashParams& hp, const SparkLeaves& lv, const SparkInputs& in,
                          SparkForest* f, bool is_mem) {
  const uint32_t* idx = d->idx;
  const uint32_t* audit_ts = d->idx + 12 * d->N;
  const dim3 paired(grid_for(f->n), is_mem ? 2 : 6), each(grid_for(f->n), f->ncirc), block(kBlock);
  if (is_mem) {
    if (lv.ncirc) hipLaunchKernelGGL(hash_mem_sub_kernel, each, block, 0, c->stream, audit_ts, in.mem_rx, in.mem_ry, d->M, hp, f->base, lv);
    else if (lv.step > 1) hipLaunchKernelGGL(hash_mem_kernel<true>, paired, block, 0, c->stream, audit_ts, in.mem_rx, in.mem_ry, d->M, hp, f->base, lv);
    else hipLaunchKernelGGL(hash_mem_kernel<false>, paired, block, 0, c->stream, audit_ts, in.mem_rx, in.mem_ry, d->M, hp, f->base, lv);
  } else {
    if (lv.ncirc) hipLaunchKernelGGL(hash_ops_sub_kernel, each, block, 0, c->stream, idx, in.derefs, d->N, hp, f->base, lv);
    else if (lv.step > 1) hipLaunchKernelGGL(hash_ops_kernel<true>, paired, block, 0, c->stream, idx, in.derefs, d->N, hp, f->base, lv);
    else hipLaunchKernelGGL(hash_ops_kernel<false>, paired, block, 0, c->stream, idx, in.derefs, d->N, hp, f->base, lv);
  }
}

int spark_build_forest(vpin_ctx* c, const vpin_spark_decomm* d, const HashParams& hp, const SparkLeaves& lv, const SparkInputs& in,
                       SparkForest* f, bool is_mem) {
  int rc = check_forest(c, d, lv, in, f, is_mem);
  if (rc) return rc;
  (void)hipSetDevice(c->device);
  ProfScope ps(c, VPIN_K_SPARK_BUILD, forest_bytes(lv, f, is_mem));
  launch_leaves(c, d, hp, lv, in, f, is_mem);
  VPIN_HIP_TRY(hipGetLastError());
  return build_levels(c, f);
}

int spark_build_forests(vpin_ctx* c, const vpin_spark_decomm* d, const HashParams& hp, const SparkLeaves& lv, const SparkInputs& in,
                        SparkForest* ops, SparkForest* mem) {
  int rc = check_forest(c, d, lv, in, ops, false);
  if (!rc) rc = check_forest(c, d, lv, in, mem, true);
  if (rc) return rc;
  (void)hipSetDevice(c->device);
  ProfScope ps(c, VPIN_K_SPARK_BUILD, forest_bytes(lv, ops, false) + forest_bytes(lv, mem, true));
  launch_leaves(c, d, hp, lv, in, ops, false);
  launch_leaves(c, d, hp, lv, in, mem, true);
  VPIN_HIP_TRY(hipGetLastError());
  rc = build_levels(c, ops);
  if (!rc) rc = build_levels(c, mem);
  return rc;
}

__device__ __forceinline__ fq fq_wave_prod(fq a) {
#pragma unroll
  for (int off = 32; off >= 1; off >>= 1) a = fq_mul(a, fq_shfl_xor(a, off));
  return a;
}
__global__ __launch_bounds__(kBlock) void hash_mem_roots_kernel(const uint32_t* __restrict__ audit_ts, const fq* __restrict__ mem_rx,
                                                                const fq* __restrict__ mem_ry, size_t M, HashParams hp,
                                                                fq* __restrict__ parts) {
  const int side = blockIdx.y;
  const fq* mem = side ? mem_ry : mem_rx;
  const uint32_t* ts = audit_ts + (size_t)side * M;
  fq pi = fq_one(), pa = fq_one();
  for (size_t i = (size_t)blockIdx.x * kBlock + threadIdx.x; i < M; i += (size_t)gridDim.x * kBlock) {
    const fq h = mem_leaf_init(hp, fq_load(mem + i), i);
    pi = fq_mul(pi, h);
    pa = fq_mul(pa, mem_leaf_audit(hp, h, ts[i]));
  }
  pi = fq_wave_prod(pi);
  pa = fq_wave_prod(pa);
  __shared__ fq sh[kBlock / 64][2];
// ... 170 lines not shown
      hipLaunchKernelGGL((dotp_round_kernel<decltype(B)::value>), dim3(grid, ndotp), dim3(kBlock), 0, c->stream, comb_derefs, vals, N,
                         scratch, from_scratch, pairs, rr, fin, kmap);
    }, r != nullptr);
  }
  VPIN_HIP_TRY(hipGetLastError());
  if (!fin.fused) return round_finish_launch(c, partials, c->round_split_ncirc, c->round_split_grid, ndotp, grid);
  return VPIN_OK;
}

int spark_collect(vpin_ctx* c, const SparkForest* f, int level, const vpin_spark_decomm* d, const fq* comb_derefs,
                  const fq* scratch, bool with_dotp, bool folded) {
  if (!c || !f || !f->base || f->ncirc > 12 || (with_dotp && (!d || !comb_derefs || !scratch))) return VPIN_EINVAL;
  int rc = spark_pinned(c);
  if (rc) return rc;
  const size_t h = f->n >> (level + 1);
  if (h < 2) return VPIN_ESHAPE;
  c->spark_seq++;
  hipLaunchKernelGGL(collect_kernel, dim3(1), dim3(128), 0, c->stream, (const fq*)f->base, f->stride(), f->level_off(level), h,
                     f->ncirc, comb_derefs, with_dotp ? (const fq*)d->vals : (const fq*)nullptr,
                     with_dotp ? d->N : (size_t)0, scratch, with_dotp, folded, c->h_spark, flag_ptr(c), c->spark_seq);
  VPIN_HIP_TRY(hipGetLastError());
  return spark_wait_flag(c);
}

int spark_triple_sums(vpin_ctx* c, const fq* comb_derefs, const fq* vals, size_t N, const int* halves, int nh) {
  if (!c || !comb_derefs || !vals || N < 2 || nh < 1 || nh > 6) return VPIN_EINVAL;
  CircIds kmap{};
  for (int i = 0; i < nh; i++) kmap.v[i] = halves ? halves[i] : i;
  int rc = spark_pinned(c);
  if (rc) return rc;
  (void)hipSetDevice(c->device);
  fq* partials = nullptr;
  if ((rc = round_partials(c, &partials))) return rc;
  const int grid = round_grid(N / 2, 6, c->shared_device);
  {
    ProfScope ps(c, VPIN_K_SPARK_BUILD, 1.5 * nh * 32.0 * (double)N);
    hipLaunchKernelGGL(triple_sum_kernel, dim3(grid, nh), dim3(kBlock), 0, c->stream, comb_derefs, vals, N, partials, kmap);
  }
  hipLaunchKernelGGL(sc_finish_kernel<3>, dim3(nh), dim3(kBlock), 0, c->stream, (const fq*)partials, grid, c->h_spark);
  VPIN_HIP_TRY(hipGetLastError());
  return spark_wait(c);
}

int spark_slice_evals(vpin_ctx* c, const fq* table, size_t len, int nslices, const fq* eq, size_t r0, size_t step) {
  if (!c || !table || !eq || nslices < 1 || nslices > kSparkMaxInst || step == 0 || r0 >= step || len % step) return VPIN_EINVAL;
  int rc = spark_pinned(c);
  if (rc) return rc;
  (void)hipSetDevice(c->device);
  fq* partials = nullptr;
  if ((rc = round_partials(c, &partials))) return rc;
  const int grid = (int)std::min<size_t>(2048, std::max<size_t>(1, (len / step + kBlock * 8 - 1) / (kBlock * 8)));
  const int groups = (nslices + 2) / 3;
  {
    ProfScope ps(c, VPIN_K_SPARK_BUILD, ((double)nslices * 32.0 * (double)len + 32.0 * (double)len) / (double)step);
    hipLaunchKernelGGL(slice_dot3_kernel, dim3(grid, groups), dim3(kBlock), 0, c->stream, table, len, nslices, eq, partials, r0, step);
  }
  hipLaunchKernelGGL(sc_finish_kernel<3>, dim3(groups), dim3(kBlock), 0, c->stream, (const fq*)partials, grid, c->h_spark);
  VPIN_HIP_TRY(hipGetLastError());
  if ((rc = spark_wait(c))) return rc;
  fq tmp[kSparkMaxInst];
  for (int i = 0; i < nslices; i++) tmp[i] = c->h_spark[i];
  for (int i = 0; i < nslices; i++) c->h_spark[3 * i] = tmp[i];
  return VPIN_OK;
}


struct TailArgs {
  fq* forest; size_t stride, off, h; int ncirc;
  const fq* pyr; int k;
  int j0; size_t len0;
  fq r_prev;
  const fq* derefs; const fq* vals; fq* scratch; size_t N;
  CircIds kmap;
  uint32_t* up;
  const uint32_t* down;
  const uint32_t* abort_flag;
  uint32_t seq0;
  unsigned long long* trace;
};

constexpr int kTailBlock = 512;
constexpr int kTailUpChunks = 32;
constexpr long kTailSpinLimit = 4000000;
constexpr size_t kTailQuadPairs = kTailBlock / 4;

__device__ __forceinline__ fq fq_shfl_from(const fq& a, int src) {
  fq r;
#pragma unroll
  for (int i = 0; i < 8; i++) r.v[i] = __shfl(a.v[i], src, 64);
  return r;
}

__global__ __launch_bounds__(kTailBlock) void spark_tail_kernel(TailArgs a) {
  const int inst = (int)blockIdx.x;
  const bool is_dotp = inst >= a.ncirc;
  __shared__ fq sh_r;
  __shared__ int sh_stop;
  fq r = a.r_prev;
  size_t len = a.len0;
  fq* A = nullptr;
  fq* Bt = nullptr;
  const fq* src[3] = {nullptr, nullptr, nullptr};
  fq* dst[3] = {nullptr, nullptr, nullptr};
  if (!is_dotp) {
    A = a.forest + (size_t)inst * a.stride + a.off;
    Bt = A + a.h;
  } else {
    const int kl = inst - a.ncirc, kk = a.kmap.v[kl], m = kk >> 1, half = kk & 1;
    const size_t hN = a.N / 2, q4 = a.N / 4;
    src[0] = a.derefs + (size_t)m * a.N + (size_t)half * hN;
    src[1] = a.derefs + (size_t)(3 + m) * a.N + (size_t)half * hN;
    src[2] = a.vals + (size_t)m * a.N + (size_t)half * hN;
#pragma unroll
    for (int t = 0; t < 3; t++) dst[t] = a.scratch + (size_t)(3 * kl + t) * q4;
  }
  uint32_t* up = a.up + (size_t)inst * kTailUpChunks * 4;
  for (int j = a.j0; j < a.k; j++) {
    const bool bind = j > 0, last = j == a.k - 1;
    const size_t pairs = bind ? len / 4 : len / 2;
    const uint32_t seq = a.seq0 + (uint32_t)(j - a.j0) + 1u;
    const fq* E = a.pyr + pyramid_offset(a.k, j + 1);
    const FoldR fr{r, nullptr};
    if (a.trace && inst == 0 && threadIdx.x == 0) a.trace[4 * (j - a.j0)] = wall_clock64();
    Acc<4> acc;
    acc.init();
    int nw = kTailBlock / 64, lo_off = 1;
    fq mine = fq_zero();
    if (!is_dotp && pairs <= kTailQuadPairs) {
      const int role = threadIdx.x & 3;
      const size_t pi = threadIdx.x >> 2;
      if (pi < pairs) {
        fq* T = (role & 2) ? Bt : A;
        const size_t idx = (role & 1) ? pairs + pi : pi;
        if (bind) {
          const fq x0 = fq_load(T + idx), x1 = fq_load(T + 2 * pairs + idx);
          mine = fq_add(x0, fq_mul(r, fq_sub(x1, x0)));
          fq_store(T + idx, mine);
        } else {
          mine = fq_load(T + idx);
        }
      }
      const int lbase = (threadIdx.x & 63) & ~3;
      const fq pA = fq_shfl_from(mine, lbase), hA = fq_shfl_from(mine, lbase + 1), pB = fq_shfl_from(mine, lbase + 2),
               hB = fq_shfl_from(mine, lbase + 3);
      if (pi < pairs && role < 2) {
        const fq u = role ? fq_mul(fq_sub(hA, pA), fq_sub(hB, pB)) : fq_mul(pA, pB);
        acc.e[role] = fq_mul(fq_load(E + pi), u);
      }
      nw = (int)((4 * pairs + 63) / 64);
      lo_off = 4;
    } else if (!is_dotp) {
      LeadNow now;
      for (size_t i = threadIdx.x; i < pairs; i += kTailBlock) {
        if (bind) pair_prod<PD_FOLD, true>(acc, now, A, Bt, E, i, pairs, fr);
        else pair_prod<PD_LOAD, true>(acc, now, A, Bt, E, i, pairs, fr);
      }
      if (pairs < (size_t)kTailBlock) nw = (int)((pairs + 63) / 64);
    } else {
      const bool from_src = j <= 1;
      for (size_t i = threadIdx.x; i < pairs; i += kTailBlock) {
        const fq* const from[3] = {from_src ? src[0] : dst[0], from_src ? src[1] : dst[1], from_src ? src[2] : dst[2]};
        if (bind) pair_dotp<true>(acc, from, dst, i, pairs, fr);
        else pair_dotp<false>(acc, from, dst, i, pairs, fr);
      }
      if (pairs < (size_t)kTailBlock) nw = (int)((pairs + 63) / 64);
    }
    if (bind) len /= 2;
    fq t;
    if (lo_off == 4) {
      fq v = (threadIdx.x & 1) ? acc.e[1] : acc.e[0];
      __shared__ fq shq[kTailBlock / 64][2];
      const int lane = threadIdx.x & 63, wave = threadIdx.x >> 6;
      if (wave < nw) {
        for (int off = 32; off >= 4; off >>= 1) v = fq_add(v, fq_shfl_xor(v, off));
        if (lane < 2) shq[wave][lane] = v;
      }
      __syncthreads();
      t = fq_zero();
      if (threadIdx.x < 2) {
        t = shq[0][threadIdx.x];
        for (int w = 1; w < nw; w++) t = fq_add(t, shq[w][threadIdx.x]);
      }
    } else {
      t = block_sum<3, kTailBlock>(acc.e, nw);
    }
    if ((int)threadIdx.x < (is_dotp ? 3 : 2)) publish_scalar(up + 12 * threadIdx.x, t, seq);
    if (last) {
      if (!is_dotp && lo_off == 4) {
        if (threadIdx.x < 4) publish_scalar(up + 36 + 12 * threadIdx.x, mine, seq);
      } else {
        const int ne = is_dotp ? 6 : 4;
        if ((int)threadIdx.x < ne) {
          const int tt = threadIdx.x >> 1, e = threadIdx.x & 1;
          const fq* tab;
          if (!is_dotp) tab = tt ? Bt : A;
          else tab = (a.k >= 2) ? dst[tt] : src[tt];
          publish_scalar(up + 36 + 12 * threadIdx.x, fq_load(tab + e), seq);
        }
      }
    }
    if (a.trace && inst == 0 && threadIdx.x == 0) a.trace[4 * (j - a.j0) + 1] = wall_clock64();
    if (last) break;
    if (threadIdx.x == 0) {
      int stop = 1;
      for (long spin = 0; spin < kTailSpinLimit; spin++) {
        u32x4 c0 = load16_system(a.down), c1, c2;
        if (c0.x != seq) {
          if ((spin & 15) == 15 && __hip_atomic_load(a.abort_flag, __ATOMIC_RELAXED, __HIP_MEMORY_SCOPE_SYSTEM) != 0u) break;
          continue;
        }
        load48_system(a.down, c0, c1, c2);
        fq rr;
        if (take_reply(c0, c1, c2, seq, rr)) {
          sh_r = rr;
          stop = 0;
          break;
        }
        if (__hip_atomic_load(a.abort_flag, __ATOMIC_RELAXED, __HIP_MEMORY_SCOPE_SYSTEM) != 0u) break;
      }
      sh_stop = stop;
      if (a.trace && inst == 0) a.trace[4 * (j - a.j0) + 2] = wall_clock64();
    }
    __syncthreads();
    if (sh_stop) return;
    r = sh_r;
  }
}

constexpr size_t kTailUp = 4096;
constexpr size_t kTailWords = 4096 + 320;
constexpr size_t kTailTrace = 4096 + 384;
static inline uint32_t* tail_words(vpin_ctx* c) { return reinterpret_cast<uint32_t*>(c->h_spark + kTailWords); }
static inline uint32_t* tail_up(vpin_ctx* c) { return reinterpret_cast<uint32_t*>(c->h_spark + kTailUp); }

size_t spark_tail_pairs() {
  static const size_t n = [] { const char* e = getenv("VPIN_SPARK_TAIL_PAIRS"); long v = e ? atol(e) : 1024; return (size_t)(v < 0 ? 0 : v); }();
  return n;
}

int spark_tail_launch(vpin_ctx* c, const SparkForest* f, int level, int k, int j0, size_t len0, const fq* pyr, const uint8_t* r_prev,
                      size_t N, const fq* vals, const fq* comb_derefs, fq* scratch, const int* halves, int ndotp) {
  if (!c || !f || !f->base || !pyr || k < 1 || j0 < 0 || j0 >= k || (j0 > 0 && !r_prev) || f->ncirc > 12 || f->ncirc < 1) return VPIN_EINVAL;
  const bool with_dotp = vals != nullptr && ndotp > 0;
  if (with_dotp && (!comb_derefs || !scratch || ndotp > 6 || level != 0 || N != f->n)) return VPIN_EINVAL;
  const size_t h = f->n >> (level + 1);
  if (h != ((size_t)1 << k) || len0 != (j0 == 0 ? h : (h >> (j0 - 1)))) return VPIN_ESHAPE;
  int rc = spark_pinned(c);
  if (rc) return rc;
  (void)hipSetDevice(c->device);
  TailArgs a{};
  a.forest = f->base; a.stride = f->stride(); a.off = f->level_off(level); a.h = h; a.ncirc = f->ncirc;
  a.pyr = pyr; a.k = k; a.j0 = j0; a.len0 = len0;
  if (r_prev) a.r_prev = load_host_fq(r_prev);
  a.derefs = comb_derefs; a.vals = vals; a.scratch = scratch; a.N = N;
  for (int i = 0; i < 6; i++) a.kmap.v[i] = (with_dotp && halves && i < ndotp) ? halves[i] : i;
  a.up = tail_up(c);
  uint32_t* w = tail_words(c);
  a.abort_flag = w; a.down = w + 16;
  w[0] = 0;
  a.seq0 = c->tail_seq;
  static const bool trace_on = getenv("VPIN_TAIL_TRACE") != nullptr;
  a.trace = trace_on ? reinterpret_cast<unsigned long long*>(c->h_spark + kTailTrace) : nullptr;
  if (trace_on) memset(c->h_spark + kTailTrace, 0, 64 * 32);
  const int ninst = f->ncirc + (with_dotp ? ndotp : 0);
  c->tail_rounds = k - j0;
  {
    ProfScope ps(c, VPIN_K_SPARK_TAIL, 0.0);
    hipLaunchKernelGGL(spark_tail_kernel, dim3((unsigned)ninst), dim3(kTailBlock), 0, c->stream, a);
  }
  if (hipGetLastError() != hipSuccess) { c->tail_rounds = 0; return VPIN_EHIP; }
  return VPIN_OK;
}

int spark_tail_wait(vpin_ctx* c, int idx, int ninst, int ncirc) {
  const uint32_t want = c->tail_seq + (uint32_t)idx + 1u;
  const bool last = idx == c->tail_rounds - 1;
  const uint32_t* up = tail_up(c);
  const auto t0 = std::chrono::steady_clock::now();
  unsigned done_mask = 0;
  const unsigned all = (1u << ninst) - 1u;
  double next_nudge = 1.0;
  for (long spins = 0;; spins++) {
    for (int i = 0; i < ninst; i++) {
      if (done_mask >> i & 1u) continue;
      const uint32_t* u = up + (size_t)i * kTailUpChunks * 4;
      bool ok = true;
      const int nsum = i < ncirc ? 2 : 3;
      for (int k = 0; k < nsum && ok; k++) ok = tail_take(u + 12 * k, want, &c->tail_sums[3 * i + k]);
      if (nsum == 2) c->tail_sums[3 * i + 2] = fq_zero_host();
      const int ne = i < ncirc ? 4 : 6;
      for (int e = 0; last && e < ne && ok; e++) ok = tail_take(u + 36 + 12 * e, want, &c->tail_final[6 * i + e]);
      if (ok) done_mask |= 1u << i;
    }
    if (done_mask == all) return VPIN_OK;
    __builtin_ia32_pause();
    if ((spins & 0xfff) == 0xfff) {
      const double waited = std::chrono::duration<double>(std::chrono::steady_clock::now() - t0).count();
      static const double limit_s = [] { const char* e = getenv("VPIN_TAIL_TIMEOUT_S"); double v = e ? atof(e) : 0.0; return v > 0.0 ? v : 20.0; }();
      if (waited > next_nudge) {
        const double tq = std::chrono::duration<double>(std::chrono::steady_clock::now() - t0).count();
        const hipError_t q = hipStreamQuery(c->stream);
        const double tq1 = std::chrono::duration<double>(std::chrono::steady_clock::now() - t0).count();
        fprintf(stderr, "[tail] ctx %p waits %.2f s for round %d of %d (instances done %#x of %#x, seq %u, stream %s, query took %.3f s, "
                        "masked %d)\n", (void*)c, waited, idx, c->tail_rounds.load(), done_mask, all, want,
                q == hipSuccess ? "IDLE: the kernel has left" : q == hipErrorNotReady ? "busy" : hipGetErrorName(q), tq1 - tq, (int)c->cu_masked);
        next_nudge += 1.0;
      }
      if (waited > limit_s) {
        for (int i = 0; i < ninst; i++)
          if (!(done_mask >> i & 1u)) {
            const uint32_t* u = up + (size_t)i * kTailUpChunks * 4;
            fprintf(stderr, "[tail]   instance %d: sequence words of its first sum %u %u %u (want %u); reply slot holds %u\n", i, u[0], u[4], u[8],
                    want, tail_words(c)[16]);
          }
        tail_words(c)[0] = 1;
        (void)hipStreamSynchronize(c->stream);
        c->tail_seq += (uint32_t)c->tail_rounds + 1u;
        c->tail_rounds = 0;
        set_last_error("spark_tail_wait: the persistent round kernel did not answer", hipErrorUnknown);
        return VPIN_EHIP;
      }
    }
  }
}

void spark_tail_reply(vpin_ctx* c, int idx, const uint8_t r[32]) {
  host_reply(tail_words(c) + 16, c->tail_seq + (uint32_t)idx + 1u, r);
  __atomic_thread_fence(__ATOMIC_SEQ_CST);
}

void spark_tail_abort(vpin_ctx* c) {
  if (!c || c->tail_rounds == 0) return;
  tail_words(c)[0] = 1;
  (void)hipStreamSynchronize(c->stream);
  c->tail_seq += (uint32_t)c->tail_rounds + 1u;
  c->tail_rounds = 0;
}

void spark_tail_end(vpin_ctx* c) {
  static const bool trace_on = getenv("VPIN_TAIL_TRACE") != nullptr;
  if (trace_on) {
    (void)hipStreamSynchronize(c->stream);
    const unsigned long long* t = reinterpret_cast<const unsigned long long*>(c->h_spark + kTailTrace);
    fprintf(stderr, "[tail] %d rounds:", c->tail_rounds.load());
    for (int i = 0; i < c->tail_rounds && i < 64; i++) {
      const double comp = (double)(t[4 * i + 1] - t[4 * i]) * 0.01, wait = t[4 * i + 2] ? (double)(t[4 * i + 2] - t[4 * i + 1]) * 0.01 : 0.0;
      fprintf(stderr, " %.1f+%.1f", comp, wait);
    }
    fprintf(stderr, " us (compute+publish, wait for reply)\n");
  }
  c->tail_seq += (uint32_t)c->tail_rounds + 1u;
// ... 53 lines not shown
```

vpin_amd/csrc/sumcheck.hip:

```cpp
#include <cstring>

#include "ctx.h"
#include "host/field.h"
#include "sc_dev.h"

namespace vpin {

fq_const make_fq_const(const uint8_t* p) {
  vpin_host::Fq r;
  memcpy(r.l, p, 32);
  fq_const out;
  for (int i = 0; i < 8; i++) {
    vpin_host::Fq pw = vpin_host::Fq::zero();
    pw.l[i / 2] = (uint64_t)1 << (32 * (i & 1));
    const vpin_host::Fq t = r * pw;
    uint32_t limbs[8];
    memcpy(limbs, t.l, 32);
    for (int k = 0; k < 8; k++) out.tt[k][i] = limbs[k];
  }
  return out;
}

template <int K>
__global__ __launch_bounds__(kBlock, kMinWaves) void sc_eval_kernel(Tabs<K> tabs, size_t half,
                                                         fq* __restrict__ partials) {
  Acc<K> acc;
  acc.init();
  for (size_t i = (size_t)blockIdx.x * kBlock + threadIdx.x; i < half; i += (size_t)gridDim.x * kBlock)
    pair_ktab<K, PD_LOAD>(acc, tabs, i, half, FoldR{});
  block_reduce_store<Acc<K>::NE>(acc.e, partials);
}

template <int K>
__global__ __launch_bounds__(kBlock, kMinWaves) void sc_bind_eval_kernel(Tabs<K> tabs, size_t quarter, fq r,
                                                              fq* __restrict__ partials) {
  const FoldR fr{r, nullptr};
  Acc<K> acc;
  acc.init();
  for (size_t i = (size_t)blockIdx.x * kBlock + threadIdx.x; i < quarter; i += (size_t)gridDim.x * kBlock)
    pair_ktab<K, PD_FOLD>(acc, tabs, i, quarter, fr);
  block_reduce_store<Acc<K>::NE>(acc.e, partials);
}

template <bool BIND, bool LEAD>
__global__ __launch_bounds__(kBlock, kMinWaves) void sc_cubic3_kernel(Tabs<3> tabs, const fq* __restrict__ E, size_t pairs,
                                                                      fq r, fq_const rc, fq* __restrict__ partials) {
  constexpr PdMode M = !BIND ? PD_LOAD : LEAD ? PD_FOLD_C : PD_FOLD;
  FoldR fr{r, nullptr};
  if constexpr (M == PD_FOLD_C) fr.tt = stage_fq_const(rc);
  Acc<4> acc;
  acc.init();
  for (size_t i = (size_t)blockIdx.x * kBlock + threadIdx.x; i < pairs; i += (size_t)gridDim.x * kBlock)
    pair_phase1<M, LEAD>(acc, tabs, E, i, pairs, fr);
  block_reduce_store<3>(acc.e, partials);
}

constexpr int kSmallBlock = 512;
constexpr size_t kSmallPairs = 512;

template <int NE>
__device__ __forceinline__ void tail_store(const fq* e, fq* __restrict__ out) {
  const fq s = block_sum<NE, kSmallBlock>(e);
  if (threadIdx.x < NE) fq_store(&out[threadIdx.x], s);
}

template <int K, bool BIND>
__global__ __launch_bounds__(kSmallBlock) void sc_tail_kernel(Tabs<K> tabs, size_t pairs, fq r, fq* __restrict__ out) {
  Acc<K> acc;
  acc.init();
  if (threadIdx.x < pairs) pair_ktab<K, BIND ? PD_FOLD : PD_LOAD>(acc, tabs, threadIdx.x, pairs, FoldR{r, nullptr});
  tail_store<Acc<K>::NE>(acc.e, out);
}

template <bool BIND, bool LEAD>
__global__ __launch_bounds__(kSmallBlock) void sc_tail3_kernel(Tabs<3> tabs, const fq* __restrict__ E, size_t pairs, fq r,
                                                               fq* __restrict__ out) {
  Acc<4> acc;
  acc.init();
  if (threadIdx.x < pairs) pair_phase1<BIND ? PD_FOLD : PD_LOAD, LEAD>(acc, tabs, E, threadIdx.x, pairs, FoldR{r, nullptr});
  tail_store<3>(acc.e, out);
}

__global__ __launch_bounds__(kBlock) void eq_pyramid_step_kernel(const fq* __restrict__ src, fq* __restrict__ dst, size_t m,
                                                                 fq tau_k) {
  for (size_t i = (size_t)blockIdx.x * kBlock + threadIdx.x; i < m; i += (size_t)gridDim.x * kBlock) {
    fq v = fq_load(src + i);
    fq hi = fq_mul(v, tau_k);
    fq_store(dst + i, fq_sub(v, hi));
    fq_store(dst + m + i, hi);
  }
}

struct TauPack { fq t[10]; };
__global__ __launch_bounds__(512) void eq_pyramid_top_kernel(fq* __restrict__ base, int ell, int k_lo, TauPack taus) {
  const size_t n = (size_t)1 << ell;
  if (threadIdx.x == 0) fq_store(base + (n - 2), fq_one());
  __syncthreads();
  for (int k = ell - 1; k >= k_lo; k--) {
    const size_t m = (size_t)1 << (ell - k - 1);
    const fq* src = base + (n - ((size_t)2 << (ell - k - 1)));
    fq* dst = base + (n - ((size_t)2 << (ell - k)));
    if (threadIdx.x < m) {
      fq v = fq_load(src + threadIdx.x);
      fq hi = fq_mul(v, taus.t[k - k_lo]);
      fq_store(dst + threadIdx.x, fq_sub(v, hi));
      fq_store(dst + m + threadIdx.x, hi);
    }
    __syncthreads();
  }
}

__global__ __launch_bounds__(64) void sc_final_kernel(Tabs<4> tabs, int k, fq r, fq* __restrict__ out) {
  const int i = threadIdx.x;
  if (i >= k) return;
  const fq a0 = fq_load(tabs.t[i]), a1 = fq_load(tabs.t[i] + 1);
  const fq v = fq_add(a0, fq_mul(r, fq_sub(a1, a0)));
  fq_store(tabs.t[i], v);
  fq_store(out + i, v);
}

template <int K>
__global__ __launch_bounds__(kBlock) void sc_bind_kernel(Tabs<K> tabs, size_t half, fq r) {
  for (size_t i = (size_t)blockIdx.x * kBlock + threadIdx.x; i < half; i += (size_t)gridDim.x * kBlock) {
#pragma unroll
    for (int k = 0; k < K; k++) {
      fq a0 = fq_load(tabs.t[k] + i);
      fq a1 = fq_load(tabs.t[k] + half + i);
      fq_store(tabs.t[k] + i, fq_add(a0, fq_mul(r, fq_sub(a1, a0))));
    }
  }
}

__global__ __launch_bounds__(kBlock) void eq_step_kernel(const fq* __restrict__ src, fq* __restrict__ dst,
                                                         size_t prev, fq rj) {
  for (size_t i = (size_t)blockIdx.x * kBlock + threadIdx.x; i < prev; i += (size_t)gridDim.x * kBlock) {
    fq s = fq_load(src + i);
    fq hi = fq_mul(s, rj);
    fq_store(dst + 2 * i + 1, hi);
    fq_store(dst + 2 * i, fq_sub(s, hi));
  }
}

struct EqHead { fq r[9]; };
__global__ __launch_bounds__(512) void eq_head_kernel(fq* __restrict__ out, int k0, EqHead rs) {
  __shared__ fq buf[2][512];
  if (threadIdx.x == 0) buf[0][0] = fq_one();
  __syncthreads();
  int cur = 0;
  for (int j = 0; j < k0; j++) {
    const size_t prev = (size_t)1 << j;
    if (threadIdx.x < prev) {
      const fq s = buf[cur][threadIdx.x];
      const fq hi = fq_mul(s, rs.r[j]);
      buf[cur ^ 1][2 * threadIdx.x + 1] = hi;
      buf[cur ^ 1][2 * threadIdx.x] = fq_sub(s, hi);
    }
    cur ^= 1;
    __syncthreads();
  }
  if (threadIdx.x < ((size_t)1 << k0)) fq_store(out + threadIdx.x, buf[cur][threadIdx.x]);
}

struct TauAll { fq t[32]; };
constexpr int kEqLoVars = 9, kEqChunk = 1 << kEqLoVars;

__device__ __forceinline__ int eq_lo_build_lsb(fq (*buf)[kEqChunk], const TauAll& ts, int first) {
  if (threadIdx.x == 0) buf[0][0] = fq_one();
  __syncthreads();
  int cur = 0;
  for (int j = 0; j < kEqLoVars; j++) {
    const int prev = 1 << j;
    if ((int)threadIdx.x < prev) {
      const fq s = buf[cur][threadIdx.x];
      const fq hi = fq_mul(s, ts.t[first + j]);
      buf[cur ^ 1][2 * threadIdx.x + 1] = hi;
      buf[cur ^ 1][2 * threadIdx.x] = fq_sub(s, hi);
    }
    cur ^= 1;
    __syncthreads();
  }
  return cur;
}

constexpr int kEqMidVars = 5, kEqMid = 1 << kEqMidVars;
__global__ __launch_bounds__(kEqChunk) void eq_table_fused_kernel(fq* __restrict__ out, int ell, int nmid, TauAll rs) {
  __shared__ fq buf[2][kEqChunk];
  __shared__ fq hm[kEqMid];
  const int cur = eq_lo_build_lsb(buf, rs, ell - kEqLoVars);
  const int nhi = ell - kEqLoVars - nmid;
  const fq one = fq_one();
  if ((int)threadIdx.x < (1 << nmid)) {
    fq run = one;
    const size_t bidx = blockIdx.x;
    for (int j = 0; j < nhi; j++) run = fq_mul(run, ((bidx >> (nhi - 1 - j)) & 1) ? rs.t[j] : fq_sub(one, rs.t[j]));
    const int m = threadIdx.x;
    for (int j = 0; j < nmid; j++) run = fq_mul(run, ((m >> (nmid - 1 - j)) & 1) ? rs.t[nhi + j] : fq_sub(one, rs.t[nhi + j]));
    hm[m] = run;
  }
  __syncthreads();
  const fq lo = buf[cur][threadIdx.x];
  fq* dst = out + ((size_t)blockIdx.x << (nmid + kEqLoVars)) + threadIdx.x;
  for (int m = 0; m < (1 << nmid); m++) fq_store(dst + (size_t)m * kEqChunk, fq_mul(hm[m], lo));
}

__global__ __launch_bounds__(kEqChunk) void eq_pyramid_fused_kernel(fq* __restrict__ base, int ell, int nlow, TauAll ts) {
  __shared__ fq buf[2][kEqChunk];
  __shared__ fq pm[kEqMid][kEqMidVars];
  __shared__ fq pb[32];
  const size_t n = (size_t)1 << ell;
  if (threadIdx.x == 0) {
    buf[0][0] = fq_one();
    if (blockIdx.x == 0) fq_store(base + (n - 2), fq_one());
  }
  __syncthreads();
  int cur = 0;
  for (int s = 1; s <= kEqLoVars; s++) {
    const int k = ell - s, m = 1 << (s - 1);
    if ((int)threadIdx.x < m) {
      const fq v = buf[cur][threadIdx.x];
      const fq hi = fq_mul(v, ts.t[k]);
      buf[cur ^ 1][threadIdx.x] = fq_sub(v, hi);
      buf[cur ^ 1][m + threadIdx.x] = hi;
    }
    cur ^= 1;
    __syncthreads();
    if (blockIdx.x == 0 && (int)threadIdx.x < 2 * m)
      fq_store(base + (n - ((size_t)2 << (ell - k))) + threadIdx.x, buf[cur][threadIdx.x]);
  }
  const int nbits = ell - kEqLoVars - 1;
  const fq one = fq_one();
  if ((int)threadIdx.x < (1 << nlow)) {
    fq run = one;
    for (int j = 0; j < nlow; j++) {
      const fq& t = ts.t[ell - kEqLoVars - 1 - j];
      run = fq_mul(run, ((threadIdx.x >> j) & 1) ? t : fq_sub(one, t));
      pm[threadIdx.x][j] = run;
    }
  } else if (threadIdx.x == 64) {
    fq run = one;
    const size_t bidx = blockIdx.x;
    for (int j = nlow; j < nbits; j++) {
      const fq& t = ts.t[ell - kEqLoVars - 1 - j];
      run = fq_mul(run, ((bidx >> (j - nlow)) & 1) ? t : fq_sub(one, t));
      pb[j] = run;
    }
  }
  __syncthreads();
  const fq lo = buf[cur][threadIdx.x];
  for (int k = 1; k <= ell - kEqLoVars - 1; k++) {
    const int nb = ell - k - kEqLoVars;
    fq* lvl = base + (n - ((size_t)2 << (ell - k))) + threadIdx.x;
    if (nb <= nlow) {
      if (blockIdx.x != 0) continue;
      for (int m = 0; m < (1 << nb); m++) fq_store(lvl + (size_t)m * kEqChunk, fq_mul(pm[m][nb - 1], lo));
    } else {
      if (((size_t)blockIdx.x >> (nb - nlow)) != 0) continue;
      const fq hb = fq_mul(pb[nb - 1], lo);
      if (nlow == 0) { fq_store(lvl + (size_t)blockIdx.x * kEqChunk, hb); continue; }
      for (int m = 0; m < (1 << nlow); m++)
        fq_store(lvl + (((size_t)blockIdx.x << nlow) + m) * kEqChunk, fq_mul(pm[m][nlow - 1], hb));
    }
  }
}

template <int K>
static int check_tabs(vpin_ctx* c, const vpin_table* const* t, size_t min_len) {
  if (!c) return VPIN_EINVAL;
  for (int k = 0; k < K; k++)
    if (!t[k] || !t[k]->d) return VPIN_EINVAL;
  for (int k = 1; k < K; k++)
    if (t[k]->len != t[0]->len) return VPIN_ESHAPE;
  if (!is_pow2(t[0]->len) || t[0]->len < min_len) return VPIN_ESHAPE;
  return VPIN_OK;
}

template <int NE>
static int finish_launch(vpin_ctx* c, int nblocks) {
  hipLaunchKernelGGL((sc_finish_kernel<NE>), dim3(1), dim3(kBlock), 0, c->stream, c->d_partials, nblocks, c->h_out);
  VPIN_HIP_TRY(hipGetLastError());
  return VPIN_OK;
}

template <int K>
static int launch_eval(vpin_ctx* c, const vpin_table* const* t, int kclass) {
  int rc = check_tabs<K>(c, t, 2);
  if (rc) return rc;
  (void)hipSetDevice(c->device);
  Tabs<K> tabs;
  for (int k = 0; k < K; k++) tabs.t[k] = t[k]->d;
  size_t half = t[0]->len / 2;
  if (half <= kSmallPairs) {
    ProfScope ps(c, VPIN_K_SC_TAIL, (double)K * 32.0 * (double)t[0]->len);
    hipLaunchKernelGGL((sc_tail_kernel<K, false>), dim3(1), dim3(kSmallBlock), 0, c->stream, tabs, half, fq{}, c->h_out);
    VPIN_HIP_TRY(hipGetLastError());
    return VPIN_OK;
  }
  int grid = grid_for(half);
  {
    ProfScope ps(c, kclass, (double)K * 32.0 * (double)t[0]->len);
    hipLaunchKernelGGL((sc_eval_kernel<K>), dim3(grid), dim3(kBlock), 0, c->stream, tabs, half, c->d_partials);
  }
  VPIN_HIP_TRY(hipGetLastError());
  return finish_launch<Acc<K>::NE>(c, grid);
}

template <int K>
static int launch_bind_eval(vpin_ctx* c, vpin_table* const* t, const uint8_t* r, int kclass) {
  int rc = check_tabs<K>(c, t, 4);
  if (rc) return rc;
  if (!r) return VPIN_EINVAL;
  (void)hipSetDevice(c->device);
  Tabs<K> tabs;
  for (int k = 0; k < K; k++) tabs.t[k] = t[k]->d;
  size_t len = t[0]->len, quarter = len / 4;
  if (quarter <= kSmallPairs) {
    {
      ProfScope ps(c, VPIN_K_SC_TAIL, (double)K * 32.0 * ((double)len + (double)len / 2));
      hipLaunchKernelGGL((sc_tail_kernel<K, true>), dim3(1), dim3(kSmallBlock), 0, c->stream, tabs, quarter, load_host_fq(r),
                         c->h_out);
    }
    VPIN_HIP_TRY(hipGetLastError());
    for (int k = 0; k < K; k++) t[k]->len = len / 2;
    return VPIN_OK;
  }
  int grid = grid_for(quarter);
  {
    ProfScope ps(c, kclass, (double)K * 32.0 * ((double)len + (double)len / 2));
    hipLaunchKernelGGL((sc_bind_eval_kernel<K>), dim3(grid), dim3(kBlock), 0, c->stream, tabs, quarter,
                       load_host_fq(r), c->d_partials);
  }
  VPIN_HIP_TRY(hipGetLastError());
  for (int k = 0; k < K; k++) t[k]->len = len / 2;
  return finish_launch<Acc<K>::NE>(c, grid);
}

static int fetch(vpin_ctx* c, int ne, uint8_t* out) {
  for (long spins = 0;; spins++) {
    const hipError_t q = hipStreamQuery(c->stream);
    if (q == hipSuccess) break;
    if (q != hipErrorNotReady) { set_last_error("sum-check round: hipStreamQuery", q); return VPIN_EHIP; }
    if (spins > 4000000) { VPIN_HIP_TRY(hipStreamSynchronize(c->stream)); break; }
  }
  memcpy(out, c->h_out, (size_t)ne * sizeof(fq));
  return VPIN_OK;
}

template <int K>
static int run_eval(vpin_ctx* c, const vpin_table* const* t, uint8_t* out, int kclass) {
  int rc = launch_eval<K>(c, t, kclass);
  return rc ? rc : fetch(c, Acc<K>::NE, out);
}

template <int K>
static int run_bind_eval(vpin_ctx* c, vpin_table* const* t, const uint8_t* r, uint8_t* out, int kclass) {
  if (!out) return VPIN_EINVAL;
  int rc = launch_bind_eval<K>(c, t, r, kclass);
  return rc ? rc : fetch(c, Acc<K>::NE, out);
}

int sc_round_launch(vpin_ctx* c, int K, vpin_table* const* tabs, const uint8_t* r) {
  if (K == 4) return r ? launch_bind_eval<4>(c, tabs, r, VPIN_K_SC_CUBIC_FUSED) : launch_eval<4>(c, tabs, VPIN_K_SC_CUBIC);
  if (K == 2) return r ? launch_bind_eval<2>(c, tabs, r, VPIN_K_SC_QUAD_FUSED) : launch_eval<2>(c, tabs, VPIN_K_SC_QUAD);
  return VPIN_EINVAL;
}
int sc_round_wait(vpin_ctx* c, int K, uint8_t* out) { return fetch(c, K == 4 ? 3 : 2, out); }

int sc_cubic3_launch(vpin_ctx* c, vpin_table* const* t, const vpin_table* pyramid, int ell, int level, const uint8_t* r, bool lead) {
  int rc = check_tabs<3>(c, t, r ? 4 : 2);
  if (rc) return rc;
  if (!pyramid || level < 1 || level > ell || pyramid->len != ((size_t)1 << ell)) return VPIN_ESHAPE;
  (void)hipSetDevice(c->device);
  Tabs<3> tabs;
  for (int k = 0; k < 3; k++) tabs.t[k] = t[k]->d;
  const size_t len = t[0]->len, pairs = r ? len / 4 : len / 2;
  if (pairs != ((size_t)1 << (ell - level))) return VPIN_ESHAPE;
  const fq* E = pyramid->d + pyramid_offset(ell, level);
  const fq rr = r ? load_host_fq(r) : fq{};
  const fq_const rconst = (r && lead) ? make_fq_const(r) : fq_const{};
  const double bytes = r ? 4 * 32.0 * ((double)len + (double)len / 2) : 4 * 32.0 * (double)len;
  if (pairs <= kSmallPairs) {
    {
      ProfScope ps(c, VPIN_K_SC_TAIL, bytes);
      dispatch_bools([&](auto B, auto L) {
        hipLaunchKernelGGL((sc_tail3_kernel<decltype(B)::value, decltype(L)::value>), dim3(1), dim3(kSmallBlock), 0, c->stream, tabs, E,
                           pairs, rr, c->h_out);
      }, r != nullptr, lead);
    }
    VPIN_HIP_TRY(hipGetLastError());
  } else {
    int grid = grid_for(pairs);
    {
      ProfScope ps(c, r ? VPIN_K_SC_CUBIC_FUSED : VPIN_K_SC_CUBIC, bytes);
      dispatch_bools([&](auto B, auto L) {
        hipLaunchKernelGGL((sc_cubic3_kernel<decltype(B)::value, decltype(L)::value>), dim3(grid), dim3(kBlock), 0, c->stream, tabs, E,
                           pairs, rr, rconst, c->d_partials);
      }, r != nullptr, lead);
    }
    VPIN_HIP_TRY(hipGetLastError());
    rc = finish_launch<3>(c, grid);
    if (rc) return rc;
  }
  if (r)
    for (int k = 0; k < 3; k++) t[k]->len = len / 2;
  return VPIN_OK;
}


int sc_final_claims(vpin_ctx* c, vpin_table* const* tables, int k, const uint8_t r[32], uint8_t* out) {
  if (!c || !tables || !r || !out || k < 1 || k > 4) return VPIN_EINVAL;
  Tabs<4> t4{};
  for (int i = 0; i < k; i++) {
    if (!tables[i] || !tables[i]->d || tables[i]->len != 2) return VPIN_ESHAPE;
    t4.t[i] = tables[i]->d;
  }
  (void)hipSetDevice(c->device);
  {
    ProfScope ps(c, VPIN_K_SC_BIND, (double)k * 96.0);
    hipLaunchKernelGGL(sc_final_kernel, dim3(1), dim3(64), 0, c->stream, t4, k, load_host_fq(r), c->h_out);
  }
  VPIN_HIP_TRY(hipGetLastError());
  for (int i = 0; i < k; i++) tables[i]->len = 1;
  return fetch(c, k, out);
}

}

using namespace vpin;

extern "C" {

int vpin_sc_cubic_round(vpin_ctx* c, const vpin_table* tau, const vpin_table* Az, const vpin_table* Bz,
                        const vpin_table* Cz, uint8_t out[96]) {
  if (!out) return VPIN_EINVAL;
  const vpin_table* t[4] = {tau, Az, Bz, Cz};
  return run_eval<4>(c, t, out, VPIN_K_SC_CUBIC);
}

int vpin_sc_quad_round(vpin_ctx* c, const vpin_table* A, const vpin_table* B, uint8_t out[64]) {
  if (!out) return VPIN_EINVAL;
  const vpin_table* t[2] = {A, B};
  return run_eval<2>(c, t, out, VPIN_K_SC_QUAD);
}

int vpin_sc_bind(vpin_ctx* c, vpin_table* const* tables, int k, const uint8_t r[32]) {
  if (!c || !tables || !r || k < 1 || k > 4) return VPIN_EINVAL;
  for (int i = 0; i < k; i++)
    if (!tables[i] || !tables[i]->d) return VPIN_EINVAL;
  for (int i = 1; i < k; i++)
    if (tables[i]->len != tables[0]->len) return VPIN_ESHAPE;
  size_t len = tables[0]->len;
  if (!is_pow2(len) || len < 2) return VPIN_ESHAPE;
  (void)hipSetDevice(c->device);
  size_t half = len / 2;
  int grid = grid_for(half);
  fq rr = load_host_fq(r);
  {
    ProfScope ps(c, VPIN_K_SC_BIND, (double)k * 32.0 * ((double)len + (double)half));
    Tabs<4> t4;
    Tabs<2> t2;
    Tabs<1> t1;
    switch (k) {
      case 4:
        for (int i = 0; i < 4; i++) t4.t[i] = tables[i]->d;
        hipLaunchKernelGGL((sc_bind_kernel<4>), dim3(grid), dim3(kBlock), 0, c->stream, t4, half, rr);
        break;
      case 3:
        for (int i = 0; i < 2; i++) t2.t[i] = tables[i]->d;
        hipLaunchKernelGGL((sc_bind_kernel<2>), dim3(grid), dim3(kBlock), 0, c->stream, t2, half, rr);
        t1.t[0] = tables[2]->d;
        hipLaunchKernelGGL((sc_bind_kernel<1>), dim3(grid), dim3(kBlock), 0, c->stream, t1, half, rr);
        break;
      case 2:
        for (int i = 0; i < 2; i++) t2.t[i] = tables[i]->d;
        hipLaunchKernelGGL((sc_bind_kernel<2>), dim3(grid), dim3(kBlock), 0, c->stream, t2, half, rr);
        break;
      default:
        t1.t[0] = tables[0]->d;
        hipLaunchKernelGGL((sc_bind_kernel<1>), dim3(grid), dim3(kBlock), 0, c->stream, t1, half, rr);
    }
  }
  VPIN_HIP_TRY(hipGetLastError());
  for (int i = 0; i < k; i++) tables[i]->len = half;
  VPIN_HIP_TRY(hipStreamSynchronize(c->stream));
  return VPIN_OK;
}

int vpin_sc_cubic_bind_round(vpin_ctx* c, vpin_table* tau, vpin_table* Az, vpin_table* Bz, vpin_table* Cz,
                             const uint8_t r[32], uint8_t out[96]) {
  vpin_table* t[4] = {tau, Az, Bz, Cz};
  return run_bind_eval<4>(c, t, r, out, VPIN_K_SC_CUBIC_FUSED);
}

int vpin_sc_quad_bind_round(vpin_ctx* c, vpin_table* A, vpin_table* B, const uint8_t r[32], uint8_t out[64]) {
  vpin_table* t[2] = {A, B};
  return run_bind_eval<2>(c, t, r, out, VPIN_K_SC_QUAD_FUSED);
}

int vpin_eq_suffix_tables(vpin_ctx* c, const uint8_t* tau, int ell, vpin_table** out) {
  if (!c || !out || !tau || ell < 1 || ell > 40) return VPIN_EINVAL;
  (void)hipSetDevice(c->device);
  vpin_table* t = nullptr;
  int rc = table_alloc_uninit(c, (size_t)1 << ell, &t);
  if (rc) return rc;
  hipError_t e = hipSuccess;
  {
    ProfScope ps(c, VPIN_K_EQ, 32.0 * 3.0 * (double)(((size_t)1 << (ell - 1)) - 1));
    if (ell >= kEqLoVars + 2 && ell <= 32) {
      TauAll ta;
      for (int k = 0; k < ell; k++) ta.t[k] = load_host_fq(tau + 32 * (size_t)k);
      const int nbits = ell - kEqLoVars - 1, nlow = std::min(kEqMidVars, std::max(0, nbits - 8));
      hipLaunchKernelGGL(eq_pyramid_fused_kernel, dim3((unsigned)((size_t)1 << (nbits - nlow))), dim3(kEqChunk), 0, c->stream, t->d, ell, nlow, ta);
    } else {
      const int k_lo = ell - 9 > 1 ? ell - 9 : 1;
      TauPack tp;
      for (int k = k_lo; k <= ell - 1; k++) tp.t[k - k_lo] = load_host_fq(tau + 32 * (size_t)k);
      hipLaunchKernelGGL(eq_pyramid_top_kernel, dim3(1), dim3(512), 0, c->stream, t->d, ell, k_lo, tp);
      for (int k = k_lo - 1; k >= 1; k--) {
        size_t m = (size_t)1 << (ell - k - 1);
        hipLaunchKernelGGL(eq_pyramid_step_kernel, dim3(grid_for(m)), dim3(kBlock), 0, c->stream,
                           (const fq*)(t->d + pyramid_offset(ell, k + 1)), t->d + pyramid_offset(ell, k), m,
                           load_host_fq(tau + 32 * (size_t)k));
      }
    }
    e = hipGetLastError();
  }
  if (e != hipSuccess) { set_last_error("vpin_eq_suffix_tables", e); vpin_table_free(c, t); return VPIN_EHIP; }
  *out = t;
  return VPIN_OK;
}

int vpin_sc_cubic3_round(vpin_ctx* c, const vpin_table* pyramid, int ell, int level, vpin_table* Az, vpin_table* Bz,
                         vpin_table* Cz, uint8_t out[96]) {
  if (!out) return VPIN_EINVAL;
  vpin_table* t[3] = {Az, Bz, Cz};
  int rc = sc_cubic3_launch(c, t, pyramid, ell, level, nullptr, false);
  return rc ? rc : sc_round_wait(c, 4, out);
}
int vpin_sc_cubic3_bind_round(vpin_ctx* c, const vpin_table* pyramid, int ell, int level, vpin_table* Az, vpin_table* Bz,
                              vpin_table* Cz, const uint8_t r[32], uint8_t out[96]) {
  if (!out || !r) return VPIN_EINVAL;
  vpin_table* t[3] = {Az, Bz, Cz};
  int rc = sc_cubic3_launch(c, t, pyramid, ell, level, r, false);
  return rc ? rc : sc_round_wait(c, 4, out);
}

int vpin_sc_cubic3_lead_round(vpin_ctx* c, const vpin_table* pyramid, int ell, int level, vpin_table* Az, vpin_table* Bz,
                              vpin_table* Cz, const uint8_t* r, uint8_t out[96]) {
  if (!out) return VPIN_EINVAL;
  vpin_table* t[3] = {Az, Bz, Cz};
  int rc = sc_cubic3_launch(c, t, pyramid, ell, level, r, true);
  return rc ? rc : sc_round_wait(c, 4, out);
}

int vpin_eq_table(vpin_ctx* c, const uint8_t* r, int ell, vpin_table** out) {
  if (!c || !out || ell < 0 || ell > 40 || (ell > 0 && !r)) return VPIN_EINVAL;
  (void)hipSetDevice(c->device);
  size_t n = (size_t)1 << ell;
  if (ell >= kEqLoVars + 1 && ell <= 32) {
    vpin_table* t = nullptr;
    int rc1 = table_alloc_uninit(c, n, &t);
    if (rc1) return rc1;
    TauAll ra;
    for (int j = 0; j < ell; j++) ra.t[j] = load_host_fq(r + 32 * (size_t)j);
    {
      ProfScope ps(c, VPIN_K_EQ, 32.0 * (double)n);
      const int nmid = std::min(kEqMidVars, std::max(0, ell - kEqLoVars - 8));
      hipLaunchKernelGGL(eq_table_fused_kernel, dim3((unsigned)(n >> (kEqLoVars + nmid))), dim3(kEqChunk), 0, c->stream, t->d, ell, nmid, ra);
    }
    hipError_t e1 = hipGetLastError();
    if (e1 != hipSuccess) { set_last_error("eq_table", e1); vpin_table_free(c, t); return VPIN_EHIP; }
    *out = t;
    return VPIN_OK;
  }
  vpin_table *a = nullptr, *b = nullptr;
  int rc = table_alloc_uninit(c, n, &a);
  if (rc) return rc;
  if (ell > 0) {
    rc = table_alloc_uninit(c, n, &b);
    if (rc) { vpin_table_free(c, a); return rc; }
  }
  const int k0 = ell < 9 ? ell : 9;
  vpin_table* src = ((ell - k0) % 2 == 0) ? a : b;
  hipError_t e = hipSuccess;
  {
    ProfScope ps(c, VPIN_K_EQ, 32.0 * 3.0 * (double)(n - 1));
    EqHead rs;
    for (int j = 0; j < k0; j++) rs.r[j] = load_host_fq(r + 32 * (size_t)j);
    hipLaunchKernelGGL(eq_head_kernel, dim3(1), dim3(512), 0, c->stream, src->d, k0, rs);
    vpin_table* dst = (src == a) ? b : a;
    size_t prev = (size_t)1 << k0;
    for (int j = k0; j < ell; j++) {
      hipLaunchKernelGGL(eq_step_kernel, dim3(grid_for(prev)), dim3(kBlock), 0, c->stream, src->d, dst->d, prev,
                         load_host_fq(r + 32 * (size_t)j));
      prev *= 2;
      vpin_table* tmp = src; src = dst; dst = tmp;
    }
  }
  e = hipGetLastError();
  if (e == hipSuccess) e = hipStreamSynchronize(c->stream);
  if (b) vpin_table_free(c, b);
  if (e != hipSuccess) { set_last_error("eq_table", e); vpin_table_free(c, a); return VPIN_EHIP; }
  *out = a;
  return VPIN_OK;
}

}
```

Measured before the change: 79.80 million constraints/s.

## Derive instance evals from SPARK derefs and cap block size on CU-masked streams

In the single-rank case, the sat prover no longer builds eq tables and evaluates the R1CS matrices to get the instance evaluations. It obtains them from the SPARK deref tables and triple sums instead, and those results are cached and reused by the later SPARK stages, which removes duplicated work. Separately, CU-masked contexts now launch the tail, tree-top and eq kernels templated on 256-thread blocks with strided loops. This is meant to fit stream slots better, at the cost of more template instantiations and more loop iterations per thread.

```diff
diff --git a/vpin_amd/csrc/capi.hip b/vpin_amd/csrc/capi.hip
--- a/vpin_amd/csrc/capi.hip
+++ b/vpin_amd/csrc/capi.hip
@@ -315,6 +315,7 @@
     e = hipExtStreamCreateWithCUMask(&c->stream, n_words, cu_mask);
     c->num_cus = enabled;
     c->cu_masked = true;
+    c->slot_blocks = true;
   } else {
     e = hipStreamCreateWithPriority(&c->stream, hipStreamNonBlocking, prio);
   }
diff --git a/vpin_amd/csrc/ctx.h b/vpin_amd/csrc/ctx.h
--- a/vpin_amd/csrc/ctx.h
+++ b/vpin_amd/csrc/ctx.h
@@ -54,6 +54,7 @@
   hipStream_t stream = nullptr;
   int num_cus = 256;
   bool cu_masked = false;
+  bool slot_blocks = false;
   hipStream_t stream_main = nullptr, stream_alt = nullptr;
   hipEvent_t stream_switch_ev = nullptr;
   int cus_main = 256, cus_alt = 0;
diff --git a/vpin_amd/csrc/host/prover_common.h b/vpin_amd/csrc/host/prover_common.h
--- a/vpin_amd/csrc/host/prover_common.h
+++ b/vpin_amd/csrc/host/prover_common.h
@@ -4,6 +4,7 @@
 #include <chrono>
 #include <cstdlib>
 #include <cstring>
+#include <functional>
 #include <map>
 #include <memory>
 #include <mutex>
@@ -480,10 +481,12 @@
 #pragma clang diagnostic pop
 #endif
 
+using InstEvalsFn = std::function<int(const Fq* rx, size_t nrx, const Fq* ry, size_t nry, Fq ie[3])>;
 int sat_prove_core(vpin_ctx* c, const vpin_r1cs_dev* dinst, size_t nv, size_t ncons, size_t ni,
                    const vpin_table* d_para, const vpin_table* d_input, const vpin_table* d_vars, const uint8_t* inputs,
                    const uint8_t seed_commit64[64], const uint8_t seed_proof64[64], uint8_t* proof_out, size_t proof_cap,
                    size_t* proof_len, uint8_t* comm_para_out, uint8_t* comm_input_out, uint8_t inst_evals_out[96],
-                   uint8_t* rx_out, uint8_t* ry_out, vpin_host::Transcript* tr_out, vpin_host::Transcript* tape_out);
-
-}
+                   uint8_t* rx_out, uint8_t* ry_out, vpin_host::Transcript* tr_out, vpin_host::Transcript* tape_out,
+                   const InstEvalsFn* evals_from = nullptr);
+
+}
diff --git a/vpin_amd/csrc/prover.cpp b/vpin_amd/csrc/prover.cpp
--- a/vpin_amd/csrc/prover.cpp
+++ b/vpin_amd/csrc/prover.cpp
@@ -475,7 +475,8 @@
                    const vpin_table* d_para, const vpin_table* d_input, const vpin_table* d_vars, const uint8_t* inputs,
                    const uint8_t seed_commit64[64], const uint8_t seed_proof64[64], uint8_t* proof_out, size_t proof_cap,
                    size_t* proof_len, uint8_t* comm_para_out, uint8_t* comm_input_out, uint8_t inst_evals_out[96],
-                   uint8_t* rx_out, uint8_t* ry_out, vpin_host::Transcript* tr_out, vpin_host::Transcript* tape_out) {
+                   uint8_t* rx_out, uint8_t* ry_out, vpin_host::Transcript* tr_out, vpin_host::Transcript* tape_out,
+                   const InstEvalsFn* evals_from) {
   auto t_begin = Clock::now();
   memset(g_timings, 0, sizeof g_timings);
   (void)hipSetDevice(c->device);
@@ -650,7 +651,9 @@
 
   t0 = Clock::now();
   Fq ie[3];
-  {
+  if (evals_from) {
+    if ((rc = (*evals_from)(rx.data(), rx.size(), ry.data(), ry.size(), ie))) return rc;
+  } else {
     vpin_table* d_eq_ry = nullptr;
     if ((rc = vpin_eq_table(c, B(ry.data()), nry, &d_eq_ry))) return rc;
     tg.add(d_eq_ry);
diff --git a/vpin_amd/csrc/sc_dev.h b/vpin_amd/csrc/sc_dev.h
--- a/vpin_amd/csrc/sc_dev.h
+++ b/vpin_amd/csrc/sc_dev.h
@@ -15,6 +15,14 @@
 inline int max_blocks() {
   static const int n = [] { const char* e = getenv("VPIN_SC_BLOCKS"); int v = e ? atoi(e) : 1024; return v < 1 ? 1 : v > kMaxBlocksCap ? kMaxBlocksCap : v; }();
   return n;
+}
+
+constexpr int kSlotBlock = 256;
+constexpr int tb_min_waves(int tb) { return tb <= kSlotBlock ? kMinWaves : 1; }
+template <int FULL, class F>
+inline void dispatch_block(const vpin_ctx* c, F&& f) {
+  if (c->slot_blocks) f(std::integral_constant<int, kSlotBlock>{});
+  else f(std::integral_constant<int, FULL>{});
 }
 
 __host__ __device__ inline size_t pyramid_offset(int ell, int k) { return ((size_t)1 << ell) - ((size_t)2 << (ell - k)); }
diff --git a/vpin_amd/csrc/spark.cpp b/vpin_amd/csrc/spark.cpp
--- a/vpin_amd/csrc/spark.cpp
+++ b/vpin_amd/csrc/spark.cpp
@@ -649,6 +649,8 @@
   std::vector<Fq> rand_ops, rand_mem;
   Fq ev_derefs[6], ev_ops[15], ev_mem[2];
   DpLog pe_derefs, pe_ops, pe_mem;
+  bool have_derefs = false, have_sums = false;
+  Fq sums6[6];
 
   SparkProof(vpin_ctx* c_, const vpin_spark_decomm* d_, const std::vector<Fq>& rx_, const std::vector<Fq>& ry_, const Fq* evals_,
              Transcript& tr_, Transcript& tape_)
@@ -672,14 +674,13 @@
   return VPIN_OK;
 }
 
-static int stage_derefs(SparkProof& S) {
+static int derefs_tables(SparkProof& S) {
   vpin_ctx* c = S.c;
   const vpin_spark_decomm* d = S.d;
   const DistPlan* dz = S.dz;
   const PcGens* g_derefs = S.g_derefs;
   const size_t N = S.N;
   int rc;
-  S.tr.append_protocol_name("Sparse polynomial evaluation proof");
   const size_t nm = std::max(d->nx, d->ny);
   std::vector<Fq> rx_ext(nm, Fq::zero()), ry_ext(nm, Fq::zero());
   std::copy(S.rx.begin(), S.rx.end(), rx_ext.begin() + (nm - d->nx));
@@ -706,6 +707,20 @@
     if ((rc = vpin::spark_gather_derefs(c, d, S.leaves, mem_rx, mem_ry, S.comb->d))) return rc;
     S.derefs = S.comb->d; S.vals = d->vals;
   }
+  S.have_derefs = true;
+  return VPIN_OK;
+}
+
+static int stage_derefs(SparkProof& S) {
+  vpin_ctx* c = S.c;
+  const vpin_spark_decomm* d = S.d;
+  const DistPlan* dz = S.dz;
+  const PcGens* g_derefs = S.g_derefs;
+  const size_t N = S.N;
+  int rc;
+  S.tr.append_protocol_name("Sparse polynomial evaluation proof");
+  if (!S.have_derefs && (rc = derefs_tables(S))) return rc;
+  const vpin::fq* mem_ry = S.mem_ry->d;
   if ((rc = vpin::comm_mark(c, "derefs_gather"))) return rc;
   std::vector<CG>& comm_derefs = S.comm_derefs;
   const bool hot = d->hot_col[0] != 0xffffffffu || d->hot_col[1] != 0xffffffffu || d->hot_col[2] != 0xffffffffu;
@@ -849,9 +864,13 @@
   int rc;
   const std::vector<int>* hv = S.by_circuit() ? &dz->dotp_of[dz->rank] : nullptr;
   const size_t nh = hv ? hv->size() : 6;
-  if (nh && (rc = vpin::spark_triple_sums(c, S.derefs, S.vals, S.Nf, hv ? hv->data() : nullptr, (int)nh))) return rc;
   Fq mine6[6] = {};
-  for (size_t i = 0; i < nh; i++) mine6[hv ? (*hv)[i] : i] = reinterpret_cast<const Fq*>(c->h_spark)[3 * i];
+  if (S.have_sums) {
+    std::copy(S.sums6, S.sums6 + 6, mine6);
+  } else {
+    if (nh && (rc = vpin::spark_triple_sums(c, S.derefs, S.vals, S.Nf, hv ? hv->data() : nullptr, (int)nh))) return rc;
+    for (size_t i = 0; i < nh; i++) mine6[hv ? (*hv)[i] : i] = reinterpret_cast<const Fq*>(c->h_spark)[3 * i];
+  }
   if (S.st) rc = dist_sum(c, *dz, mine6, 6, S.dotp.claims, "triple_sums");
   else if (dz) rc = dist_pick(c, *dz, mine6, 6, dz->owner_dotp, S.dotp.claims, "triple_sums");
   else std::copy(mine6, mine6 + 6, S.dotp.claims);
@@ -1047,18 +1066,36 @@
   write_dplog(w, S.pe_derefs);
 }
 
-static int spark_prove(vpin_ctx* c, const vpin_spark_decomm* d, const std::vector<Fq>& rx, const std::vector<Fq>& ry,
-                       const Fq evals[3], Transcript& tr, Transcript& tape, Writer& w) {
-  if (d->N < 4 || d->M < 4 || rx.size() != d->nx || ry.size() != d->ny) return VPIN_ESHAPE;
-  int rc;
-  SparkProof S(c, d, rx, ry, evals, tr, tape);
+static int spark_begin(SparkProof& S) {
+  vpin_ctx* c = S.c;
+  const vpin_spark_decomm* d = S.d;
+  if (d->N < 4 || d->M < 4 || S.rx.size() != d->nx || S.ry.size() != d->ny) return VPIN_ESHAPE;
+  int rc;
   const Shape sh{d->nx, d->ny, S.N, S.M, S.lgN + 4, std::max(d->nx, d->ny) + 1, S.lgN + 3};
   if ((rc = get_view(c, std::max(sh.v_ops, sh.v_mem), &S.g_ops)) || (rc = get_view(c, sh.v_ops, &S.g_ops)) ||
       (rc = get_view(c, sh.v_mem, &S.g_mem)) || (rc = get_view(c, sh.v_derefs, &S.g_derefs)))
     return rc;
+  return split_plan(S);
+}
+
+static int spark_inst_evals(SparkProof& S, Fq ie[3]) {
+  vpin_ctx* c = S.c;
+  int rc;
+  if (S.dz) return VPIN_EINVAL;
+  if ((rc = derefs_tables(S))) return rc;
+  if ((rc = vpin::spark_triple_sums(c, S.derefs, S.vals, S.Nf, nullptr, 6))) return rc;
+  for (int i = 0; i < 6; i++) S.sums6[i] = reinterpret_cast<const Fq*>(c->h_spark)[3 * i];
+  S.have_sums = true;
+  for (int m = 0; m < 3; m++) ie[m] = S.sums6[2 * m] + S.sums6[2 * m + 1];
+  return VPIN_OK;
+}
+
+static int spark_finish(SparkProof& S, Writer& w) {
+  vpin_ctx* c = S.c;
+  int rc;
   auto t0 = Clock::now();
   auto lap = [&](int slot) { g_spark_timings[slot] = secs(t0, Clock::now()); t0 = Clock::now(); };
-  if ((rc = split_plan(S)) || (rc = stage_derefs(S))) return rc;
+  if ((rc = stage_derefs(S))) return rc;
   lap(1);
   if (c->progress_flag) *c->progress_flag = 2;
   if ((rc = stage_network(S))) return rc;
@@ -1333,16 +1370,27 @@
   uint8_t ie[96];
   std::vector<Fq> rx(log2z(ncons)), ry(log2z(2 * nv));
   size_t sat_len = 0;
+  Fq evals[3];
+  const bool fused = !(c->comm && c->comm->world > 1);
+  SparkProof S(c, decomm, rx, ry, evals, tr, tape);
+  const vpin_prover::InstEvalsFn from_derefs = [&](const Fq* rx_, size_t nrx, const Fq* ry_, size_t nry, Fq out[3]) -> int {
+    if (nrx != rx.size() || nry != ry.size()) return VPIN_ESHAPE;
+    std::copy(rx_, rx_ + nrx, rx.begin());
+    std::copy(ry_, ry_ + nry, ry.begin());
+    int rc_ = spark_begin(S);
+    return rc_ ? rc_ : spark_inst_evals(S, out);
+  };
   int rc = sat_prove_core(c, dinst, nv, ncons, ni, vars_para, vars_input, vars, inputs, seed_commit64, seed_proof64, proof_out,
-                          proof_cap, &sat_len, comm_para_out, comm_input_out, ie, B(rx.data()), B(ry.data()), &tr, &tape);
+                          proof_cap, &sat_len, comm_para_out, comm_input_out, ie, B(rx.data()), B(ry.data()), &tr, &tape,
+                          fused ? &from_derefs : nullptr);
   if (rc) return vpin::comm_leave(c->comm, rc);
   if (c->progress_flag) *c->progress_flag = 1;
   g_spark_timings[5] = secs(t0, Clock::now());
   Writer w;
   w.bytes(ie, 96);
-  Fq evals[3];
   memcpy(evals, ie, 96);
-  if ((rc = spark_prove(c, decomm, rx, ry, evals, tr, tape, w))) return vpin::comm_leave(c->comm, rc);
+  if (!fused) rc = spark_begin(S);
+  if (rc || (rc = spark_finish(S, w))) return vpin::comm_leave(c->comm, rc);
   if (sat_len + w.buf.size() > proof_cap) return VPIN_ESHAPE;
   memcpy(proof_out + sat_len, w.buf.data(), w.buf.size());
   *proof_len = sat_len + w.buf.size();
diff --git a/vpin_amd/csrc/spark.hip b/vpin_amd/csrc/spark.hip
--- a/vpin_amd/csrc/spark.hip
+++ b/vpin_amd/csrc/spark.hip
@@ -180,12 +180,17 @@
 }
 
 constexpr int kTopBlock = 1024;
-__global__ __launch_bounds__(kTopBlock) void tree_top_kernel(fq* __restrict__ forest, size_t stride, size_t n2, size_t h0) {
+template <int TB>
+__global__ __launch_bounds__(TB, tb_min_waves(TB)) void tree_top_kernel(fq* __restrict__ forest, size_t stride, size_t n2, size_t h0) {
   fq* t = forest + (size_t)blockIdx.x * stride;
   for (size_t h = h0; h >= 1; h >>= 1) {
     const fq* src = t + (n2 - 4 * h);
     fq* dst = t + (n2 - 2 * h);
-    if (threadIdx.x < h) fq_store(dst + threadIdx.x, fq_mul(fq_load(src + threadIdx.x), fq_load(src + h + threadIdx.x)));
+    if constexpr (TB >= kTopBlock) {
+      if (threadIdx.x < h) fq_store(dst + threadIdx.x, fq_mul(fq_load(src + threadIdx.x), fq_load(src + h + threadIdx.x)));
+    } else {
+      for (size_t i = threadIdx.x; i < h; i += TB) fq_store(dst + i, fq_mul(fq_load(src + i), fq_load(src + h + i)));
+    }
     __syncthreads();
   }
 }
@@ -574,7 +579,10 @@
     h >>= 1;
     l++;
   }
-  if (h >= 1) hipLaunchKernelGGL(tree_top_kernel, dim3(f->ncirc), dim3(kTopBlock), 0, c->stream, f->base, f->stride(), n2, h);
+  if (h >= 1)
+    dispatch_block<kTopBlock>(c, [&](auto TB) {
+      hipLaunchKernelGGL(tree_top_kernel<TB()>, dim3(f->ncirc), dim3(TB()), 0, c->stream, f->base, f->stride(), n2, h);
+    });
   VPIN_HIP_TRY(hipGetLastError());
   return VPIN_OK;
 }
@@ -911,7 +919,8 @@
 constexpr int kTailBlock = 512;
 constexpr int kTailUpChunks = 32;
 constexpr long kTailSpinLimit = 4000000;
-constexpr size_t kTailQuadPairs = kTailBlock / 4;
+template <int TB>
+constexpr size_t kTailQuadPairs = TB / 4;
 
 __device__ __forceinline__ fq fq_shfl_from(const fq& a, int src) {
   fq r;
@@ -920,7 +929,8 @@
   return r;
 }
 
-__global__ __launch_bounds__(kTailBlock) void spark_tail_kernel(TailArgs a) {
+template <int TB>
+__global__ __launch_bounds__(TB, tb_min_waves(TB)) void spark_tail_kernel(TailArgs a) {
   const int inst = (int)blockIdx.x;
   const bool is_dotp = inst >= a.ncirc;
   __shared__ fq sh_r;
@@ -953,9 +963,9 @@
     if (a.trace && inst == 0 && threadIdx.x == 0) a.trace[4 * (j - a.j0)] = wall_clock64();
     Acc<4> acc;
     acc.init();
-    int nw = kTailBlock / 64, lo_off = 1;
+    int nw = TB / 64, lo_off = 1;
     fq mine = fq_zero();
-    if (!is_dotp && pairs <= kTailQuadPairs) {
+    if (!is_dotp && pairs <= kTailQuadPairs<TB>) {
       const int role = threadIdx.x & 3;
       const size_t pi = threadIdx.x >> 2;
       if (pi < pairs) {
@@ -980,25 +990,25 @@
       lo_off = 4;
     } else if (!is_dotp) {
       LeadNow now;
-      for (size_t i = threadIdx.x; i < pairs; i += kTailBlock) {
+      for (size_t i = threadIdx.x; i < pairs; i += TB) {
         if (bind) pair_prod<PD_FOLD, true>(acc, now, A, Bt, E, i, pairs, fr);
         else pair_prod<PD_LOAD, true>(acc, now, A, Bt, E, i, pairs, fr);
       }
-      if (pairs < (size_t)kTailBlock) nw = (int)((pairs + 63) / 64);
+      if (pairs < (size_t)TB) nw = (int)((pairs + 63) / 64);
     } else {
       const bool from_src = j <= 1;
-      for (size_t i = threadIdx.x; i < pairs; i += kTailBlock) {
+      for (size_t i = threadIdx.x; i < pairs; i += TB) {
         const fq* const from[3] = {from_src ? src[0] : dst[0], from_src ? src[1] : dst[1], from_src ? src[2] : dst[2]};
         if (bind) pair_dotp<true>(acc, from, dst, i, pairs, fr);
         else pair_dotp<false>(acc, from, dst, i, pairs, fr);
       }
-      if (pairs < (size_t)kTailBlock) nw = (int)((pairs + 63) / 64);
+      if (pairs < (size_t)TB) nw = (int)((pairs + 63) / 64);
     }
     if (bind) len /= 2;
     fq t;
     if (lo_off == 4) {
       fq v = (threadIdx.x & 1) ? acc.e[1] : acc.e[0];
-      __shared__ fq shq[kTailBlock / 64][2];
+      __shared__ fq shq[TB / 64][2];
       const int lane = threadIdx.x & 63, wave = threadIdx.x >> 6;
       if (wave < nw) {
         for (int off = 32; off >= 4; off >>= 1) v = fq_add(v, fq_shfl_xor(v, off));
@@ -1011,7 +1021,7 @@
         for (int w = 1; w < nw; w++) t = fq_add(t, shq[w][threadIdx.x]);
       }
     } else {
-      t = block_sum<3, kTailBlock>(acc.e, nw);
+      t = block_sum<3, TB>(acc.e, nw);
     }
     if ((int)threadIdx.x < (is_dotp ? 3 : 2)) publish_scalar(up + 12 * threadIdx.x, t, seq);
     if (last) {
@@ -1095,7 +1105,9 @@
   c->tail_rounds = k - j0;
   {
     ProfScope ps(c, VPIN_K_SPARK_TAIL, 0.0);
-    hipLaunchKernelGGL(spark_tail_kernel, dim3((unsigned)ninst), dim3(kTailBlock), 0, c->stream, a);
+    dispatch_block<kTailBlock>(c, [&](auto TB) {
+      hipLaunchKernelGGL(spark_tail_kernel<TB()>, dim3((unsigned)ninst), dim3(TB()), 0, c->stream, a);
+    });
   }
   if (hipGetLastError() != hipSuccess) { c->tail_rounds = 0; return VPIN_EHIP; }
   return VPIN_OK;
diff --git a/vpin_amd/csrc/sumcheck.hip b/vpin_amd/csrc/sumcheck.hip
--- a/vpin_amd/csrc/sumcheck.hip
+++ b/vpin_amd/csrc/sumcheck.hip
@@ -58,27 +58,35 @@
 constexpr int kSmallBlock = 512;
 constexpr size_t kSmallPairs = 512;
 
-template <int NE>
+template <int NE, int TB>
 __device__ __forceinline__ void tail_store(const fq* e, fq* __restrict__ out) {
-  const fq s = block_sum<NE, kSmallBlock>(e);
+  const fq s = block_sum<NE, TB>(e);
   if (threadIdx.x < NE) fq_store(&out[threadIdx.x], s);
 }
 
-template <int K, bool BIND>
-__global__ __launch_bounds__(kSmallBlock) void sc_tail_kernel(Tabs<K> tabs, size_t pairs, fq r, fq* __restrict__ out) {
+template <int K, bool BIND, int TB>
+__global__ __launch_bounds__(TB, tb_min_waves(TB)) void sc_tail_kernel(Tabs<K> tabs, size_t pairs, fq r, fq* __restrict__ out) {
   Acc<K> acc;
   acc.init();
-  if (threadIdx.x < pairs) pair_ktab<K, BIND ? PD_FOLD : PD_LOAD>(acc, tabs, threadIdx.x, pairs, FoldR{r, nullptr});
-  tail_store<Acc<K>::NE>(acc.e, out);
-}
-
-template <bool BIND, bool LEAD>
-__global__ __launch_bounds__(kSmallBlock) void sc_tail3_kernel(Tabs<3> tabs, const fq* __restrict__ E, size_t pairs, fq r,
-                                                               fq* __restrict__ out) {
+  if constexpr ((size_t)TB >= kSmallPairs) {
+    if (threadIdx.x < pairs) pair_ktab<K, BIND ? PD_FOLD : PD_LOAD>(acc, tabs, threadIdx.x, pairs, FoldR{r, nullptr});
+  } else {
+    for (size_t i = threadIdx.x; i < pairs; i += TB) pair_ktab<K, BIND ? PD_FOLD : PD_LOAD>(acc, tabs, i, pairs, FoldR{r, nullptr});
+  }
+  tail_store<Acc<K>::NE, TB>(acc.e, out);
+}
+
+template <bool BIND, bool LEAD, int TB>
+__global__ __launch_bounds__(TB, tb_min_waves(TB)) void sc_tail3_kernel(Tabs<3> tabs, const fq* __restrict__ E, size_t pairs, fq r,
+                                                                        fq* __restrict__ out) {
   Acc<4> acc;
   acc.init();
-  if (threadIdx.x < pairs) pair_phase1<BIND ? PD_FOLD : PD_LOAD, LEAD>(acc, tabs, E, threadIdx.x, pairs, FoldR{r, nullptr});
-  tail_store<3>(acc.e, out);
+  if constexpr ((size_t)TB >= kSmallPairs) {
+    if (threadIdx.x < pairs) pair_phase1<BIND ? PD_FOLD : PD_LOAD, LEAD>(acc, tabs, E, threadIdx.x, pairs, FoldR{r, nullptr});
+  } else {
+    for (size_t i = threadIdx.x; i < pairs; i += TB) pair_phase1<BIND ? PD_FOLD : PD_LOAD, LEAD>(acc, tabs, E, i, pairs, FoldR{r, nullptr});
+  }
+  tail_store<3, TB>(acc.e, out);
 }
 
 __global__ __launch_bounds__(kBlock) void eq_pyramid_step_kernel(const fq* __restrict__ src, fq* __restrict__ dst, size_t m,
@@ -92,7 +100,9 @@
 }
 
 struct TauPack { fq t[10]; };
-__global__ __launch_bounds__(512) void eq_pyramid_top_kernel(fq* __restrict__ base, int ell, int k_lo, TauPack taus) {
+template <int TB>
+__global__ __launch_bounds__(TB, tb_min_waves(TB)) void eq_pyramid_top_kernel(fq* __restrict__ base, int ell, int k_lo, TauPack taus) {
+  static_assert(TB >= 256, "a thread per entry of the widest source level");
   const size_t n = (size_t)1 << ell;
   if (threadIdx.x == 0) fq_store(base + (n - 2), fq_one());
   __syncthreads();
@@ -142,7 +152,9 @@
 }
 
 struct EqHead { fq r[9]; };
-__global__ __launch_bounds__(512) void eq_head_kernel(fq* __restrict__ out, int k0, EqHead rs) {
+template <int TB>
+__global__ __launch_bounds__(TB, tb_min_waves(TB)) void eq_head_kernel(fq* __restrict__ out, int k0, EqHead rs) {
+  static_assert(TB >= 256, "a thread per entry of the widest doubling step");
   __shared__ fq buf[2][512];
   if (threadIdx.x == 0) buf[0][0] = fq_one();
   __syncthreads();
@@ -158,7 +170,9 @@
     cur ^= 1;
     __syncthreads();
   }
-  if (threadIdx.x < ((size_t)1 << k0)) fq_store(out + threadIdx.x, buf[cur][threadIdx.x]);
+#pragma unroll
+  for (int i = threadIdx.x; i < 512; i += TB)
+    if (i < (1 << k0)) fq_store(out + i, buf[cur][i]);
 }
 
 struct TauAll { fq t[32]; };
@@ -183,7 +197,9 @@
 }
 
 constexpr int kEqMidVars = 5, kEqMid = 1 << kEqMidVars;
-__global__ __launch_bounds__(kEqChunk) void eq_table_fused_kernel(fq* __restrict__ out, int ell, int nmid, TauAll rs) {
+template <int TB>
+__global__ __launch_bounds__(TB, tb_min_waves(TB)) void eq_table_fused_kernel(fq* __restrict__ out, int ell, int nmid, TauAll rs) {
+  static_assert(TB >= kEqChunk / 2 && kEqChunk % TB == 0, "eq_lo_build_lsb: a thread per entry of the widest doubling step");
   __shared__ fq buf[2][kEqChunk];
   __shared__ fq hm[kEqMid];
   const int cur = eq_lo_build_lsb(buf, rs, ell - kEqLoVars);
@@ -198,12 +214,18 @@
     hm[m] = run;
   }
   __syncthreads();
-  const fq lo = buf[cur][threadIdx.x];
-  fq* dst = out + ((size_t)blockIdx.x << (nmid + kEqLoVars)) + threadIdx.x;
-  for (int m = 0; m < (1 << nmid); m++) fq_store(dst + (size_t)m * kEqChunk, fq_mul(hm[m], lo));
-}
-
-__global__ __launch_bounds__(kEqChunk) void eq_pyramid_fused_kernel(fq* __restrict__ base, int ell, int nlow, TauAll ts) {
+#pragma unroll
+  for (int s = 0; s < kEqChunk / TB; s++) {
+    const int i = threadIdx.x + s * TB;
+    const fq lo = buf[cur][i];
+    fq* dst = out + ((size_t)blockIdx.x << (nmid + kEqLoVars)) + i;
+    for (int m = 0; m < (1 << nmid); m++) fq_store(dst + (size_t)m * kEqChunk, fq_mul(hm[m], lo));
+  }
+}
+
+template <int TB>
+__global__ __launch_bounds__(TB, tb_min_waves(TB)) void eq_pyramid_fused_kernel(fq* __restrict__ base, int ell, int nlow, TauAll ts) {
+  static_assert(TB >= kEqChunk / 2 && kEqChunk % TB == 0, "a thread per entry of the widest doubling step");
   __shared__ fq buf[2][kEqChunk];
   __shared__ fq pm[kEqMid][kEqMidVars];
   __shared__ fq pb[32];
@@ -224,8 +246,11 @@
     }
     cur ^= 1;
     __syncthreads();
-    if (blockIdx.x == 0 && (int)threadIdx.x < 2 * m)
-      fq_store(base + (n - ((size_t)2 << (ell - k))) + threadIdx.x, buf[cur][threadIdx.x]);
+    if (blockIdx.x == 0) {
+#pragma unroll
+      for (int i = threadIdx.x; i < kEqChunk; i += TB)
+        if (i < 2 * m) fq_store(base + (n - ((size_t)2 << (ell - k))) + i, buf[cur][i]);
+    }
   }
   const int nbits = ell - kEqLoVars - 1;
   const fq one = fq_one();
@@ -246,19 +271,23 @@
     }
   }
   __syncthreads();
-  const fq lo = buf[cur][threadIdx.x];
-  for (int k = 1; k <= ell - kEqLoVars - 1; k++) {
-    const int nb = ell - k - kEqLoVars;
-    fq* lvl = base + (n - ((size_t)2 << (ell - k))) + threadIdx.x;
-    if (nb <= nlow) {
-      if (blockIdx.x != 0) continue;
-      for (int m = 0; m < (1 << nb); m++) fq_store(lvl + (size_t)m * kEqChunk, fq_mul(pm[m][nb - 1], lo));
-    } else {
-      if (((size_t)blockIdx.x >> (nb - nlow)) != 0) continue;
-      const fq hb = fq_mul(pb[nb - 1], lo);
-      if (nlow == 0) { fq_store(lvl + (size_t)blockIdx.x * kEqChunk, hb); continue; }
-      for (int m = 0; m < (1 << nlow); m++)
-        fq_store(lvl + (((size_t)blockIdx.x << nlow) + m) * kEqChunk, fq_mul(pm[m][nlow - 1], hb));
+#pragma unroll
+  for (int s = 0; s < kEqChunk / TB; s++) {
+    const int i = threadIdx.x + s * TB;
+    const fq lo = buf[cur][i];
+    for (int k = 1; k <= ell - kEqLoVars - 1; k++) {
+      const int nb = ell - k - kEqLoVars;
+      fq* lvl = base + (n - ((size_t)2 << (ell - k))) + i;
+      if (nb <= nlow) {
+        if (blockIdx.x != 0) continue;
+        for (int m = 0; m < (1 << nb); m++) fq_store(lvl + (size_t)m * kEqChunk, fq_mul(pm[m][nb - 1], lo));
+      } else {
+        if (((size_t)blockIdx.x >> (nb - nlow)) != 0) continue;
+        const fq hb = fq_mul(pb[nb - 1], lo);
+        if (nlow == 0) { fq_store(lvl + (size_t)blockIdx.x * kEqChunk, hb); continue; }
+        for (int m = 0; m < (1 << nlow); m++)
+          fq_store(lvl + (((size_t)blockIdx.x << nlow) + m) * kEqChunk, fq_mul(pm[m][nlow - 1], hb));
+      }
     }
   }
 }
@@ -291,7 +320,9 @@
   size_t half = t[0]->len / 2;
   if (half <= kSmallPairs) {
     ProfScope ps(c, VPIN_K_SC_TAIL, (double)K * 32.0 * (double)t[0]->len);
-    hipLaunchKernelGGL((sc_tail_kernel<K, false>), dim3(1), dim3(kSmallBlock), 0, c->stream, tabs, half, fq{}, c->h_out);
+    dispatch_block<kSmallBlock>(c, [&](auto TB) {
+      hipLaunchKernelGGL((sc_tail_kernel<K, false, TB()>), dim3(1), dim3(TB()), 0, c->stream, tabs, half, fq{}, c->h_out);
+    });
     VPIN_HIP_TRY(hipGetLastError());
     return VPIN_OK;
   }
@@ -316,8 +347,9 @@
   if (quarter <= kSmallPairs) {
     {
       ProfScope ps(c, VPIN_K_SC_TAIL, (double)K * 32.0 * ((double)len + (double)len / 2));
-      hipLaunchKernelGGL((sc_tail_kernel<K, true>), dim3(1), dim3(kSmallBlock), 0, c->stream, tabs, quarter, load_host_fq(r),
-                         c->h_out);
+      dispatch_block<kSmallBlock>(c, [&](auto TB) {
+        hipLaunchKernelGGL((sc_tail_kernel<K, true, TB()>), dim3(1), dim3(TB()), 0, c->stream, tabs, quarter, load_host_fq(r), c->h_out);
+      });
     }
     VPIN_HIP_TRY(hipGetLastError());
     for (int k = 0; k < K; k++) t[k]->len = len / 2;
@@ -382,8 +414,10 @@
     {
       ProfScope ps(c, VPIN_K_SC_TAIL, bytes);
       dispatch_bools([&](auto B, auto L) {
-        hipLaunchKernelGGL((sc_tail3_kernel<decltype(B)::value, decltype(L)::value>), dim3(1), dim3(kSmallBlock), 0, c->stream, tabs, E,
-                           pairs, rr, c->h_out);
+        dispatch_block<kSmallBlock>(c, [&](auto TB) {
+          hipLaunchKernelGGL((sc_tail3_kernel<decltype(B)::value, decltype(L)::value, TB()>), dim3(1), dim3(TB()), 0, c->stream, tabs, E,
+                             pairs, rr, c->h_out);
+        });
       }, r != nullptr, lead);
     }
     VPIN_HIP_TRY(hipGetLastError());
@@ -509,12 +543,16 @@
       TauAll ta;
       for (int k = 0; k < ell; k++) ta.t[k] = load_host_fq(tau + 32 * (size_t)k);
       const int nbits = ell - kEqLoVars - 1, nlow = std::min(kEqMidVars, std::max(0, nbits - 8));
-      hipLaunchKernelGGL(eq_pyramid_fused_kernel, dim3((unsigned)((size_t)1 << (nbits - nlow))), dim3(kEqChunk), 0, c->stream, t->d, ell, nlow, ta);
+      dispatch_block<kEqChunk>(c, [&](auto TB) {
+        hipLaunchKernelGGL(eq_pyramid_fused_kernel<TB()>, dim3((unsigned)((size_t)1 << (nbits - nlow))), dim3(TB()), 0, c->stream, t->d, ell, nlow, ta);
+      });
     } else {
       const int k_lo = ell - 9 > 1 ? ell - 9 : 1;
       TauPack tp;
       for (int k = k_lo; k <= ell - 1; k++) tp.t[k - k_lo] = load_host_fq(tau + 32 * (size_t)k);
-      hipLaunchKernelGGL(eq_pyramid_top_kernel, dim3(1), dim3(512), 0, c->stream, t->d, ell, k_lo, tp);
+      dispatch_block<512>(c, [&](auto TB) {
+        hipLaunchKernelGGL(eq_pyramid_top_kernel<TB()>, dim3(1), dim3(TB()), 0, c->stream, t->d, ell, k_lo, tp);
+      });
       for (int k = k_lo - 1; k >= 1; k--) {
         size_t m = (size_t)1 << (ell - k - 1);
         hipLaunchKernelGGL(eq_pyramid_step_kernel, dim3(grid_for(m)), dim3(kBlock), 0, c->stream,
@@ -565,7 +603,9 @@
     {
       ProfScope ps(c, VPIN_K_EQ, 32.0 * (double)n);
       const int nmid = std::min(kEqMidVars, std::max(0, ell - kEqLoVars - 8));
-      hipLaunchKernelGGL(eq_table_fused_kernel, dim3((unsigned)(n >> (kEqLoVars + nmid))), dim3(kEqChunk), 0, c->stream, t->d, ell, nmid, ra);
+      dispatch_block<kEqChunk>(c, [&](auto TB) {
+        hipLaunchKernelGGL(eq_table_fused_kernel<TB()>, dim3((unsigned)(n >> (kEqLoVars + nmid))), dim3(TB()), 0, c->stream, t->d, ell, nmid, ra);
+      });
     }
     hipError_t e1 = hipGetLastError();
     if (e1 != hipSuccess) { set_last_error("eq_table", e1); vpin_table_free(c, t); return VPIN_EHIP; }
@@ -586,7 +626,9 @@
     ProfScope ps(c, VPIN_K_EQ, 32.0 * 3.0 * (double)(n - 1));
     EqHead rs;
     for (int j = 0; j < k0; j++) rs.r[j] = load_host_fq(r + 32 * (size_t)j);
-    hipLaunchKernelGGL(eq_head_kernel, dim3(1), dim3(512), 0, c->stream, src->d, k0, rs);
+    dispatch_block<512>(c, [&](auto TB) {
+      hipLaunchKernelGGL(eq_head_kernel<TB()>, dim3(1), dim3(TB()), 0, c->stream, src->d, k0, rs);
+    });
     vpin_table* dst = (src == a) ? b : a;
     size_t prev = (size_t)1 << k0;
     for (int j = k0; j < ell; j++) {
```

Result: faster. 81.43 million constraints/s, median of 6 (+2.0%).
